# jackhwalters/DCS-Net

Measured on AMD Instinct MI355X. Metric: STFT frames/sec (train fwd+bwd+Adam), higher is better.
Workload: dtype f32

## Files before the change

dcs-net_amd/csrc/attention.hip:

```cpp
#include "conv_common.h"
#include "cbn_geom.h"

namespace {

constexpr int kThreads = 256;
#ifndef DCS_ATT_APP_IT
#define DCS_ATT_APP_IT 2
#endif
#ifndef DCS_ATT_GRID_CAP
#define DCS_ATT_GRID_CAP 8192
#endif
constexpr int kMaxChunks = DCS_ATT_MAX_CHUNKS;

inline bool att_geom(int C, int* G) { return att::geom(C, G); }
inline int ca_chunks(long HW, int G) { return att::ca_chunks(HW, G); }

__device__ __forceinline__ void ca_pool_kernel_body(const act_t* __restrict__ x, double* __restrict__ part,
                                                            long HW, int C, int G, int bx, int by, int gx) {
    __shared__ double red[kThreads * 4];
    const int t = threadIdx.x, g = t % G, r0 = t / G, rpi = kThreads / G;
    const int b = by;
    const ActIn4<act_t> x4 = act_in4(x) + (long)b * HW * G;
    float s0 = 0.f, s1 = 0.f, s2 = 0.f, s3 = 0.f;
    for (long r = (long)bx * rpi + r0; r < HW; r += (long)gx * rpi) {
// ... 75 lines not shown
    const int t = threadIdx.x, g = t % G, r0 = t / G, rpi = kThreads / G;
    const int b = by;
    const ActIn4<act_t> x4 = act_in4(x) + (long)b * HW * G;
    float4 a = make_float4(1.f, 0.f, 1.f, 0.f);
    if (ca) a = reinterpret_cast<const float4*>(ca)[(long)b * G + g];
    const float invC = 1.f / (float)C;
    const long iters = (HW + (long)gx * rpi - 1) / ((long)gx * rpi);
    for (long k = 0; k < iters; ++k) {
        const long r = (k * gx + bx) * rpi + r0;
        const bool ok = r < HW;
        float4 v = make_float4(0.f, 0.f, 0.f, 0.f);
        if (ok) v = x4[r * G + g];
        const float z0r = a.x * v.x - a.y * v.y, z0i = a.x * v.y + a.y * v.x;
        const float z1r = a.z * v.z - a.w * v.w, z1i = a.z * v.w + a.w * v.z;
        const float sr = group_sum(z0r + z1r, G), si = group_sum(z0i + z1i, G);
        const float mr = group_max(fmaxf(z0r, z1r), G), mi = group_max(fmaxf(z0i, z1i), G);
        if (ok && g == 0) pooled[(long)b * HW + r] = make_float4(sr * invC, si * invC, mr, mi);
    }
}

template <bool DROP>
__device__ __forceinline__ void attention_apply_kernel_body(const act_t* __restrict__ x,
                                                                    const float* __restrict__ ca,
                                                                    const float2* __restrict__ sa, act_t* __restrict__ y,
                                                                    long HW, int C, int G, float drop_p, uint64_t seed, const uint64_t* __restrict__ seed_dev, int bx, int by, int gx) {
    if (seed_dev) seed += seed_dev[0];
    const int t = threadIdx.x, g = t % G, r0 = t / G, rpi = kThreads / G;
    const int b = by;
    const long base = (long)b * HW * G;
    const ActIn4<act_t> x4 = act_in4(x) + base;
    const ActOut4<act_t> y4 = act_out4(y) + base;
    float4 a = make_float4(1.f, 0.f, 1.f, 0.f);
    if (ca) a = reinterpret_cast<const float4*>(ca)[(long)b * G + g];
    const float inv_keep = DROP ? 1.f / (1.f - drop_p) : 1.f;
    for (long r = (long)bx * rpi + r0; r < HW; r += (long)gx * rpi) {
        const float4 v = x4[r * G + g];
        float2 s = make_float2(1.f, 0.f);
        if (sa) s = sa[(long)b * HW + r];
        const float z0r = fmaf(a.x, v.x, -(a.y * v.y)), z0i = fmaf(a.x, v.y, a.y * v.x);
        const float z1r = fmaf(a.z, v.z, -(a.w * v.w)), z1i = fmaf(a.z, v.w, a.w * v.z);
        float4 o;
        o.x = fmaf(s.x, z0r, -(s.y * z0i)); o.y = fmaf(s.x, z0i, s.y * z0r);
        o.z = fmaf(s.x, z1r, -(s.y * z1i)); o.w = fmaf(s.x, z1i, s.y * z1r);
        if (DROP) {
            const uint64_t e = (uint64_t)(base + r * G + g) * 4;
            o.x *= dcs_keep_scale(seed, e, drop_p, inv_keep);
            o.y *= dcs_keep_scale(seed, e + 1, drop_p, inv_keep);
            o.z *= dcs_keep_scale(seed, e + 2, drop_p, inv_keep);
            o.w *= dcs_keep_scale(seed, e + 3, drop_p, inv_keep);
        }
        y4[r * G + g] = o;
    }
}

constexpr int kMaxBatch = 8;
template <class P> struct Tbl { P p[kMaxBatch]; int x0[kMaxBatch + 1]; };
template <class P> __device__ __forceinline__ int tbl_find(const Tbl<P>& t, int bx) {
    int z = 0;
#pragma unroll
    for (int k = 1; k < kMaxBatch; ++k) z += bx >= t.x0[k] ? 1 : 0;
    return z;
}

struct CaPoolP { const act_t* x; double* part; long HW; int C, G, nx; };
struct CaFcP { const double* part; int nchunks; const float2* w1; const float2* w2; float2* ca; float2* pooled; float2* hidden;
               long HW; int C, Ch; };
struct SpPoolP { const act_t* x; const float* ca; float4* pooled; long HW; int C, G, nx; };
struct ApplyP { const act_t* x; const float* ca; const float2* sa; act_t* y; long HW; int C, G, nx; };

__global__ __launch_bounds__(kThreads) void ca_pool_kernel(CaPoolP p) {
    ca_pool_kernel_body(p.x, p.part, p.HW, p.C, p.G, blockIdx.x, blockIdx.y, gridDim.x);
}
__global__ __launch_bounds__(kThreads) void ca_pool_multi_kernel(Tbl<CaPoolP> t) {
    const int z = tbl_find(t, blockIdx.x);
    const CaPoolP& p = t.p[z];
    ca_pool_kernel_body(p.x, p.part, p.HW, p.C, p.G, blockIdx.x - t.x0[z], blockIdx.y, p.nx);
}
__global__ __launch_bounds__(kThreads) void ca_fc_kernel(CaFcP p) {
    ca_fc_kernel_body(p.part, p.nchunks, p.w1, p.w2, p.ca, p.pooled, p.hidden, p.HW, p.C, p.Ch, blockIdx.x, 0, 0);
}
__global__ __launch_bounds__(kThreads) void ca_fc_multi_kernel(Tbl<CaFcP> t) {
    const CaFcP& p = t.p[blockIdx.z];
    ca_fc_kernel_body(p.part, p.nchunks, p.w1, p.w2, p.ca, p.pooled, p.hidden, p.HW, p.C, p.Ch, blockIdx.x, 0, 0);
}
__global__ __launch_bounds__(kThreads) void spatial_pool_kernel(SpPoolP p) {
    spatial_pool_kernel_body(p.x, p.ca, p.pooled, p.HW, p.C, p.G, blockIdx.x, blockIdx.y, gridDim.x);
}
__global__ __launch_bounds__(kThreads) void spatial_pool_multi_kernel(Tbl<SpPoolP> t) {
    const int z = tbl_find(t, blockIdx.x);
    const SpPoolP& p = t.p[z];
    spatial_pool_kernel_body(p.x, p.ca, p.pooled, p.HW, p.C, p.G, blockIdx.x - t.x0[z], blockIdx.y, p.nx);
}
template <bool DROP>
__global__ __launch_bounds__(kThreads) void attention_apply_kernel(ApplyP p, float drop_p, uint64_t seed, const uint64_t* seed_dev) {
    attention_apply_kernel_body<DROP>(p.x, p.ca, p.sa, p.y, p.HW, p.C, p.G, drop_p, seed, seed_dev, blockIdx.x, blockIdx.y, gridDim.x);
}
__global__ __launch_bounds__(kThreads) void attention_apply_multi_kernel(Tbl<ApplyP> t) {
    const int z = tbl_find(t, blockIdx.x);
    const ApplyP& p = t.p[z];
    attention_apply_kernel_body<false>(p.x, p.ca, p.sa, p.y, p.HW, p.C, p.G, 0.f, 0, nullptr, blockIdx.x - t.x0[z], blockIdx.y, p.nx);
}

#ifndef DCS_ACT_BF16
__global__ __launch_bounds__(kThreads) void dropout_kernel(const float* __restrict__ x, float* __restrict__ y, long n,
                                                            float drop_p, uint64_t seed, const uint64_t* __restrict__ seed_dev) {
    if (seed_dev) seed += seed_dev[0];
    const float inv_keep = 1.f / (1.f - drop_p);
    for (long i = (long)blockIdx.x * kThreads + threadIdx.x; i < n; i += (long)gridDim.x * kThreads)
        y[i] = x[i] * (drop_p > 0.f ? dcs_keep_scale(seed, (uint64_t)i, drop_p, inv_keep) : 1.f);
}
#endif

inline int stream_grid(long HW, int G, int B) {
    const int rpi = kThreads / G;
    long it = (HW + rpi - 1) / rpi;
    long nb = it <= DCS_ATT_SMALL_IT ? (it + DCS_ATT_APP_IT - 1) / DCS_ATT_APP_IT : (it + 3) / 4;
    long cap = (it <= DCS_ATT_SMALL_IT ? DCS_ATT_GRID_CAP : 2048) / (B > 0 ? B : 1);
    if (cap < 1) cap = 1;
    return (int)(nb < 1 ? 1 : (nb > cap ? cap : nb));
}

}

#ifndef DCS_ACT_BF16
extern "C" long dcs_ca_workspace_bytes(int B, long HW, int C) {
    int G;
    if (B <= 0 || HW <= 0 || !att_geom(C, &G)) return -1;
    return (long)B * ca_chunks(HW, G) * C * 2 * (long)sizeof(double);
}
#endif

extern "C" int DCS_SYM(dcs_channel_attention_fwd)(const act_t* x, const float* w1, const float* w2, float* ca_out,
                                         float* pooled_out, float* hidden_out, void* workspace, long workspace_bytes,
                                         int B, long HW, int C, int Ch, dcs_stream_t stream) {
    int G;
    if (!x || !w1 || !w2 || !ca_out || !pooled_out || !hidden_out || !workspace) return DCS_ERR_BADARG;
    if (B <= 0 || B > 65535 || HW <= 0 || !att_geom(C, &G) || Ch <= 0 || Ch > 64) return DCS_ERR_BADARG;
    const int nch = ca_chunks(HW, G);
    if (workspace_bytes < (long)B * nch * C * 2 * (long)sizeof(double)) return DCS_ERR_WORKSPACE;
    hipStream_t s = dcs_stream(stream);
    const CaPoolP pp{x, (double*)workspace, HW, C, G, nch};
    DCS_LAUNCH(ca_pool_kernel, dim3(nch, B), dim3(kThreads), 0, s, pp);
    DCS_CHECK_LAUNCH();
    const CaFcP fp{(const double*)workspace, nch, (const float2*)w1, (const float2*)w2, (float2*)ca_out, (float2*)pooled_out,
                   (float2*)hidden_out, HW, C, Ch};
    DCS_LAUNCH(ca_fc_kernel, dim3(B), dim3(kThreads), 0, s, fp);
    DCS_CHECK_LAUNCH();
    return DCS_OK;
}

#ifndef DCS_ACT_BF16
extern "C" int dcs_ca_pool_chunks(long HW, int C) {
    int G;
    if (HW <= 0 || !att_geom(C, &G)) return -1;
    return ca_chunks(HW, G);
}

extern "C" int dcs_channel_attention_fc_fwd(const void* part, const float* w1, const float* w2, float* ca_out,
                                            float* pooled_out, float* hidden_out, int B, long HW, int C, int Ch,
                                            dcs_stream_t stream) {
    int G;
    if (!part || !w1 || !w2 || !ca_out || !pooled_out || !hidden_out) return DCS_ERR_BADARG;
    if (B <= 0 || B > 65535 || HW <= 0 || !att_geom(C, &G) || Ch <= 0 || Ch > 64) return DCS_ERR_BADARG;
    const CaFcP fp{(const double*)part, ca_chunks(HW, G), (const float2*)w1, (const float2*)w2, (float2*)ca_out,
                   (float2*)pooled_out, (float2*)hidden_out, HW, C, Ch};
    DCS_LAUNCH(ca_fc_kernel, dim3(B), dim3(kThreads), 0, dcs_stream(stream), fp);
    DCS_CHECK_LAUNCH();
    return DCS_OK;
}
#endif

extern "C" int DCS_SYM(dcs_spatial_pool_fwd)(const act_t* x, const float* ca, float* pooled, int B, long HW, int C,
                                    dcs_stream_t stream) {
    int G;
    if (!x || !pooled || B <= 0 || B > 65535 || HW <= 0 || !att_geom(C, &G)) return DCS_ERR_BADARG;
    const int nx = stream_grid(HW, G, B);
    const SpPoolP sp{x, ca, (float4*)pooled, HW, C, G, nx};
    DCS_LAUNCH(spatial_pool_kernel, dim3(nx, B), dim3(kThreads), 0, dcs_stream(stream), sp);
    DCS_CHECK_LAUNCH();
    return DCS_OK;
}

extern "C" int DCS_SYM(dcs_attention_apply_fwd)(const act_t* x, const float* ca, const float* sa, act_t* y, int B, long HW,
                                       int C, float drop_p, unsigned long long seed, const unsigned long long* seed_dev, dcs_stream_t stream) {
    int G;
    if (!x || !y || B <= 0 || B > 65535 || HW <= 0 || !att_geom(C, &G)) return DCS_ERR_BADARG;
    if (!(drop_p >= 0.f && drop_p < 1.f)) return DCS_ERR_BADARG;
    const int nx = stream_grid(HW, G, B);
    dim3 grid(nx, B);
    const ApplyP ap{x, ca, (const float2*)sa, y, HW, C, G, nx};
    if (drop_p > 0.f)
        DCS_LAUNCH(attention_apply_kernel<true>, grid, dim3(kThreads), 0, dcs_stream(stream), ap, drop_p,
                           (uint64_t)seed, (const uint64_t*)seed_dev);
    else
        DCS_LAUNCH(attention_apply_kernel<false>, grid, dim3(kThreads), 0, dcs_stream(stream), ap, drop_p,
                           (uint64_t)seed, (const uint64_t*)seed_dev);
    DCS_CHECK_LAUNCH();
    return DCS_OK;
}

static long fwd_batched_workspace_bytes(int n, const dcs_attention_item* items, int B) {
    if (n < 1 || n > kMaxBatch || !items || B <= 0) return -1;
    long total = 0;
    for (int i = 0; i < n; ++i) {
        int G;
        if (!att_geom(items[i].C, &G)) return -1;
        const long b = (long)B * ca_chunks((long)items[i].H * items[i].W, G) * items[i].C * 2 * (long)sizeof(double);
        total += (b + 255) / 256 * 256;
    }
    return total;
}

#ifndef DCS_ACT_BF16
extern "C" long dcs_attention_fwd_batched_workspace_bytes(int n, const dcs_attention_item* items, int B) {
    return fwd_batched_workspace_bytes(n, items, B);
}
#endif

extern "C" int DCS_SYM(dcs_attention_fwd_batched)(int n, const dcs_attention_item* items, void* workspace, long workspace_bytes, int B,
                                         dcs_stream_t stream) {
    if (n < 1 || n > kMaxBatch || !items || !workspace || B <= 0 || B > 65535) return DCS_ERR_BADARG;
    if (workspace_bytes < fwd_batched_workspace_bytes(n, items, B)) return DCS_ERR_WORKSPACE;
    Tbl<CaPoolP> tp; Tbl<CaFcP> tf; Tbl<SpPoolP> ts; Tbl<ApplyP> ta;
    conv::Args ca_[kMaxBatch];
    int nx_pool = 1, nx_stream = 1;
    char* ws = (char*)workspace;
    for (int i = 0; i < n; ++i) {
        const dcs_attention_item& it = items[i];
        int G;
        if (!it.x || !it.w1 || !it.w2 || !it.wsa || !it.sa_bias || !it.ca || !it.pooled || !it.hidden || !it.sp || !it.sa ||
            !it.y || it.H <= 0 || it.W <= 0 || it.Ch <= 0 || it.Ch > 64 || !att_geom(it.C, &G))
            return DCS_ERR_BADARG;
        const long HW = (long)it.H * it.W;
        const int nch = ca_chunks(HW, G), nxs = stream_grid(HW, G, B);
        tp.p[i] = CaPoolP{(const act_t*)it.x, (double*)ws, HW, it.C, G, nch};
        tf.p[i] = CaFcP{(const double*)ws, nch, (const float2*)it.w1, (const float2*)it.w2, (float2*)it.ca, (float2*)it.pooled,
                        (float2*)it.hidden, HW, it.C, it.Ch};
        ts.p[i] = SpPoolP{(const act_t*)it.x, it.ca, (float4*)it.sp, HW, it.C, G, nxs};
        ta.p[i] = ApplyP{(const act_t*)it.x, it.ca, (const float2*)it.sa, (act_t*)it.y, HW, it.C, G, nxs};
        ws += ((long)B * nch * it.C * 2 * (long)sizeof(double) + 255) / 256 * 256;
        nx_pool = nch > nx_pool ? nch : nx_pool;
        nx_stream = nxs > nx_stream ? nxs : nx_stream;
        conv::Args& a = ca_[i];
        a = conv::Args{};
        a.x1 = (const act2_t*)it.sp;     a.x2 = nullptr; a.wp = (const float2*)it.wsa; a.bias = (const float2*)it.sa_bias;
        a.y = (act2_t*)it.sa;
        a.B = B; a.Hin = it.H; a.Win = it.W; a.C1 = 2; a.C2 = 0; a.up_f = 1; a.up_t = 1; a.zero_ins = 0; a.Cout = 1;
        a.kh = 7; a.kw = 7; a.sf = 1; a.st = 1; a.pad_f = 3; a.pad_t = 3; a.act = DCS_ACT_SIGMOID;
        a.Hv = it.H; a.Wv = it.W; a.Hout = it.H; a.Wout = it.W;
    }
    hipStream_t s = dcs_stream(stream);
    {
        int ap = 0, as_ = 0;
        for (int k = 0; k <= kMaxBatch; ++k) {
            tp.x0[k] = k < n ? ap : 0x7fffffff; ts.x0[k] = ta.x0[k] = k < n ? as_ : 0x7fffffff;
            if (k < n) { ap += tp.p[k].nx; as_ += ts.p[k].nx; }
        }
        tp.x0[n] = ap; ts.x0[n] = ta.x0[n] = as_;
        nx_pool = ap; nx_stream = as_;
    }
    DCS_LAUNCH(ca_pool_multi_kernel, dim3(nx_pool, B, 1), dim3(kThreads), 0, s, tp);
    DCS_CHECK_LAUNCH();
    DCS_LAUNCH(ca_fc_multi_kernel, dim3(B, 1, n), dim3(kThreads), 0, s, tf);
    DCS_CHECK_LAUNCH();
    DCS_LAUNCH(spatial_pool_multi_kernel, dim3(nx_stream, B, 1), dim3(kThreads), 0, s, ts);
    DCS_CHECK_LAUNCH();
    const int rc = dcs_conv_direct_multi(ca_, n, s);
    if (rc != DCS_OK) return rc;
    DCS_LAUNCH(attention_apply_multi_kernel, dim3(nx_stream, B, 1), dim3(kThreads), 0, s, ta);
    DCS_CHECK_LAUNCH();
    return DCS_OK;
}

#ifndef DCS_ACT_BF16
extern "C" int dcs_dropout_fwd(const float* x, float* y, long n, float drop_p, unsigned long long seed,
                               const unsigned long long* seed_dev, dcs_stream_t stream) {
    if (!x || !y || n <= 0 || !(drop_p >= 0.f && drop_p < 1.f)) return DCS_ERR_BADARG;
    long nb = (n + kThreads * 4 - 1) / (kThreads * 4);
    const int grid = (int)(nb < 1 ? 1 : (nb > 2048 ? 2048 : nb));
    DCS_LAUNCH(dropout_kernel, dim3(grid), dim3(kThreads), 0, dcs_stream(stream), x, y, n, drop_p,
                       (uint64_t)seed, (const uint64_t*)seed_dev);
    DCS_CHECK_LAUNCH();
    return DCS_OK;
}
#endif
```

dcs-net_amd/csrc/cbn.hip:

```cpp
#include "dcs_common.h"
#include "cbn_geom.h"

namespace {

constexpr int kThreads = 256;
constexpr int kMaxBlocks = 512;

struct CbnGeom {
    int vec_per_row;
    int rows_per_iter;
    int nblocks;
};

inline bool cbn_geom(long P, int C, CbnGeom* g) {
    if (P <= 0 || C <= 0) return false;
    if (C == 1) {
        long nvec = P / 2;
        long it = (nvec + kThreads - 1) / kThreads;
        long nb = (it + DCS_CBN_RED_IT - 1) / DCS_CBN_RED_IT;
        g->vec_per_row = 0;
        g->rows_per_iter = 0;
        g->nblocks = (int)(nb < 1 ? 1 : (nb > kMaxBlocks ? kMaxBlocks : nb));
        return true;
    }
// ... 149 lines not shown
    const float Rrr = (Cii + s) * ist, Rii = (Crr + s) * ist, Rri = -Cri * ist;
    const float W0 = w_[0], W1 = w_[1], W2 = w_[2], b0 = b_[0], b1 = b_[1];
    const float a0 = W0 * Rrr + W2 * Rri, a1 = W0 * Rri + W2 * Rii;
    const float a2 = W2 * Rrr + W1 * Rri, a3 = W2 * Rri + W1 * Rii;
    float* st = stats_out + 8 * c;
    st[0] = mr; st[1] = mi; st[2] = Rrr; st[3] = Rii; st[4] = Rri; st[5] = Crr; st[6] = Cii; st[7] = Cri;
    float* co = coef_out + 6 * c;
    co[0] = a0; co[1] = a1; co[2] = a2; co[3] = a3;
    co[4] = b0 - a0 * mr - a1 * mi;
    co[5] = b1 - a2 * mr - a3 * mi;
}

#ifndef DCS_ACT_BF16
__global__ void rbn_finalize_kernel(const float* __restrict__ x, const double* __restrict__ part, int nblocks,
                                    const float* __restrict__ weight, const float* __restrict__ bias,
                                    float* __restrict__ running_mean, float* __restrict__ running_var,
                                    float* __restrict__ stats_out, float* __restrict__ coef_out, long P, int C, int merge,
                                    float eps, float momentum, int use_batch_stats) {
    const int c = blockIdx.x, lane = threadIdx.x;
    float mr, mi, vr, vi;
    if (use_batch_stats) {
        double S[5] = {0, 0, 0, 0, 0};
        for (int b0 = lane; b0 < nblocks; b0 += 64 * 8) {
            double v[8][5];
#pragma unroll
            for (int k = 0; k < 8; ++k) {
                const int b = b0 + 64 * k < nblocks ? b0 + 64 * k : nblocks - 1;
#pragma unroll
                for (int i = 0; i < 5; ++i) v[k][i] = part[((long)b * C + c) * 5 + i];
            }
#pragma unroll
            for (int k = 0; k < 8; ++k)
#pragma unroll
                for (int i = 0; i < 5; ++i) S[i] += b0 + 64 * k < nblocks ? v[k][i] : 0.0;
        }
#pragma unroll
        for (int i = 0; i < 5; ++i) S[i] = dcs_wave_sum_d(S[i]);
        if (lane != 0) return;
        const double n = (double)P;
        const double kr = (double)x[2 * c], ki = (double)x[2 * c + 1];
        double m_r = kr + S[0] / n, m_i = ki + S[1] / n;
        double v_r = S[2] / n - (S[0] / n) * (S[0] / n), v_i = S[3] / n - (S[1] / n) * (S[1] / n);
        double cnt = n;
        if (merge) {
            const double m = 0.5 * (m_r + m_i);
            const double v = 0.5 * (v_r + (m_r - m) * (m_r - m) + v_i + (m_i - m) * (m_i - m));
            m_r = m_i = m; v_r = v_i = v; cnt = 2 * n;
        }
        mr = (float)m_r; mi = (float)m_i; vr = (float)v_r; vi = (float)v_i;
        if (momentum >= 0.f && running_mean != nullptr) {
            const float f = momentum, unb = cnt > 1 ? (float)(cnt / (cnt - 1.0)) : 1.f;
            if (merge) {
                running_mean[0] = f * mr + (1.f - f) * running_mean[0];
                running_var[0] = f * vr * unb + (1.f - f) * running_var[0];
            } else {
                running_mean[2 * c] = f * mr + (1.f - f) * running_mean[2 * c];
                running_mean[2 * c + 1] = f * mi + (1.f - f) * running_mean[2 * c + 1];
                running_var[2 * c] = f * vr * unb + (1.f - f) * running_var[2 * c];
                running_var[2 * c + 1] = f * vi * unb + (1.f - f) * running_var[2 * c + 1];
            }
        }
    } else {
        if (lane != 0) return;
        mr = running_mean[merge ? 0 : 2 * c]; mi = running_mean[merge ? 0 : 2 * c + 1];
        vr = running_var[merge ? 0 : 2 * c]; vi = running_var[merge ? 0 : 2 * c + 1];
    }
    const float isr = 1.0f / sqrtf(vr + eps), isi = 1.0f / sqrtf(vi + eps);
    float w0 = 1.f, w1 = 1.f, b0 = 0.f, b1 = 0.f;
    if (weight != nullptr) {
        w0 = weight[merge ? 0 : 2 * c]; w1 = weight[merge ? 0 : 2 * c + 1];
        b0 = bias[merge ? 0 : 2 * c]; b1 = bias[merge ? 0 : 2 * c + 1];
    }
    const float a0 = w0 * isr, a3 = w1 * isi;
    float* st = stats_out + 8 * c;
    st[0] = mr; st[1] = mi; st[2] = isr; st[3] = isi; st[4] = 0.f; st[5] = vr + eps; st[6] = vi + eps; st[7] = 0.f;
    float* co = coef_out + 6 * c;
    co[0] = a0; co[1] = 0.f; co[2] = 0.f; co[3] = a3;
    co[4] = b0 - a0 * mr;
    co[5] = b1 - a3 * mi;
}

#endif

template <int ACT>
__device__ __forceinline__ float act_fn(float v) {
    if (ACT == DCS_ACT_RELU) return v > 0.f ? v : 0.f;
    if (ACT == DCS_ACT_LRELU) return v > 0.f ? v : 0.01f * v;
    return v;
}

template <int ACT, bool DROP>
__global__ __launch_bounds__(kThreads) void cbn_apply_kernel(const act_t* __restrict__ x, act_t* __restrict__ y,
                                                              const float* __restrict__ coef, long P, int C, int G,
                                                              int rows_per_iter, float drop_p, uint64_t seed, const uint64_t* __restrict__ seed_dev) {
    if (seed_dev) seed += seed_dev[0];
    const float inv_keep = DROP ? 1.f / (1.f - drop_p) : 1.f;
    const int t = threadIdx.x;
    const ActIn4<act_t> x4 = act_in4(x);
    const ActOut4<act_t> y4 = act_out4(y);
    if (C == 1) {
        const float a0 = coef[0], a1 = coef[1], a2 = coef[2], a3 = coef[3], c0 = coef[4], c1 = coef[5];
        const long nvec = P / 2;
        for (long i = (long)blockIdx.x * kThreads + t; i < nvec; i += (long)gridDim.x * kThreads) {
            float4 v = x4[i], o;
            o.x = act_fn<ACT>(fmaf(a0, v.x, fmaf(a1, v.y, c0)));
            o.y = act_fn<ACT>(fmaf(a2, v.x, fmaf(a3, v.y, c1)));
            o.z = act_fn<ACT>(fmaf(a0, v.z, fmaf(a1, v.w, c0)));
            o.w = act_fn<ACT>(fmaf(a2, v.z, fmaf(a3, v.w, c1)));
            if (DROP) {
                const uint64_t e = (uint64_t)i * 4;
                o.x *= dcs_keep_scale(seed, e, drop_p, inv_keep);
                o.y *= dcs_keep_scale(seed, e + 1, drop_p, inv_keep);
                o.z *= dcs_keep_scale(seed, e + 2, drop_p, inv_keep);
                o.w *= dcs_keep_scale(seed, e + 3, drop_p, inv_keep);
            }
            y4[i] = o;
        }
        if ((P & 1) && blockIdx.x == 0 && t == 0) {
            const float xr = dcs_ld1(x + 2 * (P - 1)), xi = dcs_ld1(x + 2 * (P - 1) + 1);
            float yr = act_fn<ACT>(fmaf(a0, xr, fmaf(a1, xi, c0)));
            float yi = act_fn<ACT>(fmaf(a2, xr, fmaf(a3, xi, c1)));
            if (DROP) {
                yr *= dcs_keep_scale(seed, (uint64_t)2 * (P - 1), drop_p, inv_keep);
                yi *= dcs_keep_scale(seed, (uint64_t)2 * (P - 1) + 1, drop_p, inv_keep);
            }
            dcs_st1(y + 2 * (P - 1), yr);
            dcs_st1(y + 2 * (P - 1) + 1, yi);
        }
        return;
    }
    const int g = t % G, r0 = t / G;
    const float* ca = coef + 12 * g;
    const float a0 = ca[0], a1 = ca[1], a2 = ca[2], a3 = ca[3], c0 = ca[4], c1 = ca[5];
    const float e0 = ca[6], e1 = ca[7], e2 = ca[8], e3 = ca[9], f0 = ca[10], f1 = ca[11];
    for (long r = (long)blockIdx.x * rows_per_iter + r0; r < P; r += (long)gridDim.x * rows_per_iter) {
        float4 v = x4[r * G + g], o;
        o.x = act_fn<ACT>(fmaf(a0, v.x, fmaf(a1, v.y, c0)));
        o.y = act_fn<ACT>(fmaf(a2, v.x, fmaf(a3, v.y, c1)));
        o.z = act_fn<ACT>(fmaf(e0, v.z, fmaf(e1, v.w, f0)));
        o.w = act_fn<ACT>(fmaf(e2, v.z, fmaf(e3, v.w, f1)));
        if (DROP) {
            const uint64_t e = (uint64_t)(r * G + g) * 4;
            o.x *= dcs_keep_scale(seed, e, drop_p, inv_keep);
            o.y *= dcs_keep_scale(seed, e + 1, drop_p, inv_keep);
            o.z *= dcs_keep_scale(seed, e + 2, drop_p, inv_keep);
            o.w *= dcs_keep_scale(seed, e + 3, drop_p, inv_keep);
        }
        y4[r * G + g] = o;
    }
}

__device__ __forceinline__ float stored(float v) { return DCS_ACT_IS_BF16 ? dcs_bf16_to_f32(dcs_f32_to_bf16(v)) : v; }

template <int ACT>
__global__ __launch_bounds__(kThreads) void cbn_apply_pool_kernel(const act_t* __restrict__ x, act_t* __restrict__ y,
                                                                   const float* __restrict__ coef, double* __restrict__ part,
                                                                   long HW, int C, int G) {
    __shared__ double red[kThreads * 4];
    const int t = threadIdx.x, g = t % G, r0 = t / G, rpi = kThreads / G;
    const int b = blockIdx.y, bx = blockIdx.x, gx = gridDim.x;
    const ActIn4<act_t> x4 = act_in4(x) + (long)b * HW * G;
    const ActOut4<act_t> y4 = act_out4(y) + (long)b * HW * G;
    const float* ca = coef + 12 * g;
    const float a0 = ca[0], a1 = ca[1], a2 = ca[2], a3 = ca[3], c0 = ca[4], c1 = ca[5];
    const float e0 = ca[6], e1 = ca[7], e2 = ca[8], e3 = ca[9], f0 = ca[10], f1 = ca[11];
    float s0 = 0.f, s1 = 0.f, s2 = 0.f, s3 = 0.f;
    for (long r = (long)bx * rpi + r0; r < HW; r += (long)gx * rpi) {
        const float4 v = x4[r * G + g];
        float4 o;
        o.x = act_fn<ACT>(fmaf(a0, v.x, fmaf(a1, v.y, c0)));
        o.y = act_fn<ACT>(fmaf(a2, v.x, fmaf(a3, v.y, c1)));
        o.z = act_fn<ACT>(fmaf(e0, v.z, fmaf(e1, v.w, f0)));
        o.w = act_fn<ACT>(fmaf(e2, v.z, fmaf(e3, v.w, f1)));
        y4[r * G + g] = o;
        s0 += stored(o.x); s1 += stored(o.y); s2 += stored(o.z); s3 += stored(o.w);
    }
    red[t * 4 + 0] = s0; red[t * 4 + 1] = s1; red[t * 4 + 2] = s2; red[t * 4 + 3] = s3;
    __syncthreads();
    for (int o = t; o < G * 4; o += kThreads) {
        const int gg = o / 4, i = o % 4;
        double a = 0;
        for (int r = 0; r < rpi; ++r) a += red[(r * G + gg) * 4 + i];
        part[(((long)b * gx + bx) * C + 2 * gg) * 2 + i] = a;
    }
}

}

#ifndef DCS_ACT_BF16
extern "C" long dcs_cbn_workspace_bytes(long P, int C) {
    CbnGeom g;
    if (!cbn_geom(P, C, &g)) return -1;
    return (long)g.nblocks * C * 5 * (long)sizeof(double);
}
#endif

static int cbn_fwd_impl(const act_t* x, act_t* y, const float* weight, const float* bias, float* running_mean,
                        float* running_covar, float* stats_out, float* coef_out, void* workspace,
                        long workspace_bytes, long P, int C, float eps, float momentum, int use_batch_stats,
                        int act, float drop_p, unsigned long long seed, const unsigned long long* seed_dev, dcs_stream_t stream,
                        const float* slab_part, int slab_rows, int slab_stride, const float* slab_pivot) {
    CbnGeom g;
    if (!x || !y || !stats_out || !coef_out || !cbn_geom(P, C, &g)) return DCS_ERR_BADARG;
    if ((weight == nullptr) != (bias == nullptr)) return DCS_ERR_BADARG;
    if (use_batch_stats < 0 || use_batch_stats > 3) return DCS_ERR_BADARG;
    if (use_batch_stats == 3 && (!slab_part || !slab_pivot || slab_rows < 1 || slab_stride < slab_rows)) return DCS_ERR_BADARG;
    if (use_batch_stats == 0 && (!running_mean || !running_covar)) return DCS_ERR_BADARG;
    if (act != DCS_ACT_NONE && act != DCS_ACT_RELU && act != DCS_ACT_LRELU) return DCS_ERR_BADARG;
    if (!(drop_p >= 0.f && drop_p < 1.f)) return DCS_ERR_BADARG;
    hipStream_t s = dcs_stream(stream);
    if (use_batch_stats == 1) {
        if (!workspace || workspace_bytes < (long)g.nblocks * C * 5 * (long)sizeof(double)) return DCS_ERR_WORKSPACE;
        DCS_LAUNCH(cbn_stats_kernel, dim3(g.nblocks), dim3(kThreads), 0, s, x, (double*)workspace, P, C,
                           g.vec_per_row, g.rows_per_iter);
        DCS_CHECK_LAUNCH();
    }
    if (use_batch_stats == 3) {
        DCS_LAUNCH((cbn_finalize_kernel<float, float>), dim3(C), dim3(256), 0, s, slab_pivot, slab_part, slab_rows, slab_stride, weight, bias,
                   running_mean, running_covar, stats_out, coef_out, P, C, eps, momentum, 1);
        DCS_CHECK_LAUNCH();
    } else if (use_batch_stats != 2) {
        DCS_LAUNCH((cbn_finalize_kernel<double, act_t>), dim3(C), dim3(256), 0, s, x, (const double*)workspace,
                           g.nblocks, 0, weight, bias, running_mean, running_covar, stats_out, coef_out, P, C, eps, momentum,
                           use_batch_stats);
        DCS_CHECK_LAUNCH();
    }
    long iters = (C == 1) ? (P / 2 + kThreads - 1) / kThreads : (P + g.rows_per_iter - 1) / g.rows_per_iter;
    long nb = (iters + DCS_CBN_APP_IT - 1) / DCS_CBN_APP_IT;
    int grid = (int)(nb < 1 ? 1 : (nb > 2048 ? 2048 : nb));
#define DCS_CBN_APPLY(A, D)                                                                                   \
    DCS_LAUNCH((cbn_apply_kernel<A, D>), dim3(grid), dim3(kThreads), 0, s, x, y, coef_out, P, C,         \
                       g.vec_per_row, g.rows_per_iter, drop_p, (uint64_t)seed, (const uint64_t*)seed_dev)
    const bool drop = drop_p > 0.f;
    if (act == DCS_ACT_RELU) { if (drop) DCS_CBN_APPLY(DCS_ACT_RELU, true); else DCS_CBN_APPLY(DCS_ACT_RELU, false); }
    else if (act == DCS_ACT_LRELU) { if (drop) DCS_CBN_APPLY(DCS_ACT_LRELU, true); else DCS_CBN_APPLY(DCS_ACT_LRELU, false); }
    else { if (drop) DCS_CBN_APPLY(DCS_ACT_NONE, true); else DCS_CBN_APPLY(DCS_ACT_NONE, false); }
#undef DCS_CBN_APPLY
    DCS_CHECK_LAUNCH();
    return DCS_OK;
}

extern "C" int DCS_SYM(dcs_cbn_fwd)(const act_t* x, act_t* y, const float* weight, const float* bias, float* running_mean,
                           float* running_covar, float* stats_out, float* coef_out, void* workspace,
                           long workspace_bytes, long P, int C, float eps, float momentum, int use_batch_stats,
                           int act, float drop_p, unsigned long long seed, const unsigned long long* seed_dev, dcs_stream_t stream) {
    if (use_batch_stats == 3) return DCS_ERR_BADARG;
    return cbn_fwd_impl(x, y, weight, bias, running_mean, running_covar, stats_out, coef_out, workspace, workspace_bytes, P, C,
                        eps, momentum, use_batch_stats, act, drop_p, seed, seed_dev, stream, nullptr, 0, 0, nullptr);
}

extern "C" int DCS_SYM(dcs_cbn_fwd_slabs)(const act_t* x, act_t* y, const float* weight, const float* bias, float* running_mean,
                                 float* running_covar, float* stats_out, float* coef_out, const float* part, int rows,
                                 int stride, const float* pivot, long P, int C, float eps, float momentum, int act, float drop_p,
                                 unsigned long long seed, const unsigned long long* seed_dev, dcs_stream_t stream) {
    return cbn_fwd_impl(x, y, weight, bias, running_mean, running_covar, stats_out, coef_out, nullptr, 0, P, C, eps, momentum,
                        3, act, drop_p, seed, seed_dev, stream, part, rows, stride, pivot);
}

extern "C" int DCS_SYM(dcs_cbn_fwd_slabs_pool)(const act_t* x, act_t* y, const float* weight, const float* bias,
                                               float* running_mean, float* running_covar, float* stats_out, float* coef_out,
                                               const float* part, int rows, int stride, const float* pivot, void* pool_part,
                                               long pool_bytes, int B, long HW, int C, float eps, float momentum, int act,
                                               dcs_stream_t stream) {
    int G;
    if (!x || !y || !stats_out || !coef_out || !part || !pivot || !pool_part || B <= 0 || B > 65535 || HW <= 0 ||
        !att::geom(C, &G) || rows < 1 || stride < rows)
        return DCS_ERR_BADARG;
    if ((weight == nullptr) != (bias == nullptr)) return DCS_ERR_BADARG;
    if (act != DCS_ACT_NONE && act != DCS_ACT_RELU && act != DCS_ACT_LRELU) return DCS_ERR_BADARG;
    const int nch = att::ca_chunks(HW, G);
    if (pool_bytes < (long)B * nch * C * 2 * (long)sizeof(double)) return DCS_ERR_WORKSPACE;
    hipStream_t s = dcs_stream(stream);
    const long P = (long)B * HW;
    DCS_LAUNCH((cbn_finalize_kernel<float, float>), dim3(C), dim3(256), 0, s, pivot, part, rows, stride, weight, bias,
               running_mean, running_covar, stats_out, coef_out, P, C, eps, momentum, 1);
    DCS_CHECK_LAUNCH();
#define DCS_CBN_AP(A) DCS_LAUNCH((cbn_apply_pool_kernel<A>), dim3(nch, B), dim3(kThreads), 0, s, x, y, (const float*)coef_out, \
                                 (double*)pool_part, HW, C, G)
    if (act == DCS_ACT_RELU) DCS_CBN_AP(DCS_ACT_RELU);
    else if (act == DCS_ACT_LRELU) DCS_CBN_AP(DCS_ACT_LRELU);
    else DCS_CBN_AP(DCS_ACT_NONE);
#undef DCS_CBN_AP
    DCS_CHECK_LAUNCH();
    return DCS_OK;
}

#ifndef DCS_ACT_BF16
extern "C" int dcs_rbn_fwd(const float* x, float* y, const float* weight, const float* bias, float* running_mean,
                           float* running_var, float* stats_out, float* coef_out, void* workspace, long workspace_bytes,
                           long P, int Cr, float eps, float momentum, int use_batch_stats, int act, dcs_stream_t stream) {
    const int merge = Cr == 1;
    if (!x || !y || !stats_out || !coef_out || Cr < 1 || (!merge && (Cr & 1)) || (merge && (P & 1))) return DCS_ERR_BADARG;
    const int C = merge ? 1 : Cr / 2;
    const long Pc = merge ? P / 2 : P;
    CbnGeom g;
    if (!cbn_geom(Pc, C, &g)) return DCS_ERR_BADARG;
    if ((weight == nullptr) != (bias == nullptr) || use_batch_stats < 0 || use_batch_stats > 1) return DCS_ERR_BADARG;
    if (use_batch_stats == 0 && (!running_mean || !running_var)) return DCS_ERR_BADARG;
    if (act != DCS_ACT_NONE && act != DCS_ACT_RELU && act != DCS_ACT_LRELU) return DCS_ERR_BADARG;
    hipStream_t s = dcs_stream(stream);
    if (use_batch_stats) {
        if (!workspace || workspace_bytes < (long)g.nblocks * C * 5 * (long)sizeof(double)) return DCS_ERR_WORKSPACE;
        DCS_LAUNCH(cbn_stats_kernel, dim3(g.nblocks), dim3(kThreads), 0, s, x, (double*)workspace, Pc, C, g.vec_per_row,
                   g.rows_per_iter);
        DCS_CHECK_LAUNCH();
    }
    DCS_LAUNCH(rbn_finalize_kernel, dim3(C), dim3(64), 0, s, x, (const double*)workspace, g.nblocks, weight, bias,
               running_mean, running_var, stats_out, coef_out, Pc, C, merge, eps, momentum, use_batch_stats);
    DCS_CHECK_LAUNCH();
    long iters = (C == 1) ? (Pc / 2 + kThreads - 1) / kThreads : (Pc + g.rows_per_iter - 1) / g.rows_per_iter;
    long nb = (iters + DCS_CBN_APP_IT - 1) / DCS_CBN_APP_IT;
    const int grid = (int)(nb < 1 ? 1 : (nb > 2048 ? 2048 : nb));
#define DCS_RBN_APPLY(A)                                                                                        \
    DCS_LAUNCH((cbn_apply_kernel<A, false>), dim3(grid), dim3(kThreads), 0, s, x, y, coef_out, Pc, C, g.vec_per_row, \
               g.rows_per_iter, 0.f, (uint64_t)0, (const uint64_t*)nullptr)
    if (act == DCS_ACT_RELU) DCS_RBN_APPLY(DCS_ACT_RELU);
    else if (act == DCS_ACT_LRELU) DCS_RBN_APPLY(DCS_ACT_LRELU);
    else DCS_RBN_APPLY(DCS_ACT_NONE);
#undef DCS_RBN_APPLY
    DCS_CHECK_LAUNCH();
    return DCS_OK;
}
#endif
```

dcs-net_amd/csrc/cbn_geom.h:

```cpp
#pragma once
#ifndef DCS_CBN_RED_IT
#define DCS_CBN_RED_IT 8
#endif
#ifndef DCS_CBN_APP_IT
#define DCS_CBN_APP_IT 4
#endif

namespace cbn {

constexpr int kThreads = 256;
constexpr int kMaxBlocks = 512;

struct Geom {
    int vec_per_row;
    int rows_per_iter;
    int nblocks;
};

inline bool geom(long P, int C, Geom* g) {
    if (P <= 0 || C <= 0) return false;
    long it;
    if (C == 1) {
        g->vec_per_row = 0;
        g->rows_per_iter = 0;
        it = (P / 2 + kThreads - 1) / kThreads;
    } else {
        if (C & 1) return false;
        const int G = C / 2;
        if (G > kThreads || (kThreads % G) != 0) return false;
        g->vec_per_row = G;
        g->rows_per_iter = kThreads / G;
        it = (P + g->rows_per_iter - 1) / g->rows_per_iter;
    }
    const long nb = (it + DCS_CBN_RED_IT - 1) / DCS_CBN_RED_IT;
    g->nblocks = (int)(nb < 1 ? 1 : (nb > kMaxBlocks ? kMaxBlocks : nb));
    return true;
}

inline int stream_grid(long P, int C, const Geom& g) {
    const long iters = (C == 1) ? (P / 2 + kThreads - 1) / kThreads : (P + g.rows_per_iter - 1) / g.rows_per_iter;
    const long nb = (iters + DCS_CBN_APP_IT - 1) / DCS_CBN_APP_IT;
    return (int)(nb < 1 ? 1 : (nb > 2048 ? 2048 : nb));
}

}

#ifndef DCS_ATT_RED_IT
#define DCS_ATT_RED_IT 2
#endif
#ifndef DCS_ATT_SMALL_IT
#define DCS_ATT_SMALL_IT 256
#endif
#ifndef DCS_ATT_MAX_CHUNKS
#define DCS_ATT_MAX_CHUNKS 256
#endif
namespace att {
inline bool geom(int C, int* G) {
    if (C < 2 || (C & 1)) return false;
    const int g = C / 2;
    if (g > 64 || (g & (g - 1)) != 0) return false;
    *G = g;
    return true;
}
inline int ca_chunks(long HW, int G) {
    const int rows_per_iter = 256 / G;
    const long it = (HW + rows_per_iter - 1) / rows_per_iter;
    long nb = it <= DCS_ATT_SMALL_IT ? (it + DCS_ATT_RED_IT - 1) / DCS_ATT_RED_IT : (it + 7) / 8;
    if (it > DCS_ATT_SMALL_IT && nb > 64) nb = 64;
    return (int)(nb < 1 ? 1 : (nb > DCS_ATT_MAX_CHUNKS ? DCS_ATT_MAX_CHUNKS : nb));
}
}
```

dcs-net_amd/dcsnet/_lib.py:

```python
import ctypes
import os

_HERE = os.path.dirname(os.path.abspath(__file__))
LIB_PATH = os.environ.get('DCS_LIB_PATH') or os.path.join(os.path.dirname(_HERE), 'lib', 'libdcsnet_hip.so')

ACT_NONE, ACT_RELU, ACT_LRELU, ACT_SIGMOID = 0, 1, 2, 3

_P = ctypes.c_void_p
_I = ctypes.c_int
_L = ctypes.c_long
_F = ctypes.c_float
_U64 = ctypes.c_ulonglong



class AttentionItem(ctypes.Structure):
    _fields_ = [(n, _P) for n in ('x', 'w1', 'w2', 'wsa', 'sa_bias', 'ca', 'pooled', 'hidden', 'sp', 'sa', 'y', 'g_out',
                                  'wsa_bwd', 'g_pre', 'g_sp', 'g_x', 'g_fc0_r', 'g_fc0_i', 'g_fc2_r', 'g_fc2_i')] + \
               [(n, _I) for n in ('H', 'W', 'C', 'Ch')] + [('g_pooled', _P)]


SIGNATURES = {
    'dcs_abi_version': (_I, []),
    'dcs_error_string': (ctypes.c_char_p, [_I]),
    'dcs_pack_conv_weight': (_I, [_P, _P, _P, _P, _P, _P, _I, _I, _I, _I, _I, _I, _I, _P]),
    'dcs_cconv2d_fwd_workspace_bytes': (_L, [_I] * 14),
    'dcs_cconv2d_fwd': (_I, [_P, _P, _P, _P, _P, _P, _L] + [_I] * 15 + [_P]),
    'dcs_cconv2d_fwd_affine': (_I, [_P, _P, _P, _P, _P, _P, _P, _L] + [_I] * 15 + [_P]),
    'dcs_cconv2d_fwd_stats_rows': (_I, [_I] * 14),
    'dcs_cconv2d_fwd_stats': (_I, [_P] * 6 + [_I, _P, _P, _L] + [_I] * 14 + [_P]),
    'dcs_rconv2d_fwd_workspace_bytes': (_L, [_I] * 14),
    'dcs_rconv2d_fwd': (_I, [_P, _P, _P, _P, _P, _P, _L] + [_I] * 15 + [_P]),
    'dcs_rconv2d_bwd_data_workspace_bytes': (_L, [_I] * 11),
    'dcs_rconv2d_bwd_data': (_I, [_P, _P, _P, _P, _L] + [_I] * 11 + [_P]),
    'dcs_rbn_fwd': (_I, [_P] * 9 + [_L, _L, _I, _F, _F, _I, _I, _P]),
    'dcs_rbn_bwd': (_I, [_P] * 8 + [_L, _L, _I, _I, _I, _P]),
    'dcs_packed_weight_floats': (_L, [_I] * 6),
    'dcs_packed_weight_bwd_floats': (_L, [_I] * 10),
    'dcs_pack_conv_weight_bwd': (_I, [_P, _P] + [_I] * 10 + [_P]),
    'dcs_cconv2d_bwd_data_workspace_bytes': (_L, [_I] * 14),
    'dcs_cconv2d_bwd_data': (_I, [_P] * 5 + [_L] + [_I] * 14 + [_P]),
    'dcs_upsample_cat_bwd': (_I, [_P, _P, _P] + [_I] * 7 + [_P]),
    'dcs_cconv2d_bwd_weight_workspace_bytes': (_L, [_I] * 14),
    'dcs_cconv2d_bwd_weight': (_I, [_P] * 8 + [_L] + [_I] * 15 + [_P]),
    'dcs_cbn_workspace_bytes': (_L, [_L, _I]),
    'dcs_cbn_fwd': (_I, [_P] * 9 + [_L, _L, _I, _F, _F, _I, _I, _F, _U64, _P, _P]),
    'dcs_cbn_fwd_slabs': (_I, [_P] * 9 + [_I, _I, _P, _L, _I, _F, _F, _I, _F, _U64, _P, _P]),
    'dcs_ca_pool_chunks': (_I, [_L, _I]),
    'dcs_cbn_fwd_slabs_pool': (_I, [_P] * 9 + [_I, _I, _P, _P, _L, _I, _L, _I, _F, _F, _I, _P]),
    'dcs_channel_attention_fc_fwd': (_I, [_P] * 6 + [_I, _L, _I, _I, _P]),
    'dcs_cbn_bwd_workspace_bytes': (_L, [_L, _I]),
    'dcs_cbn_bwd': (_I, [_P] * 9 + [_L, _L, _I, _I, _I, _F, _U64, _P, _P]),
    'dcs_cbn_bwd_add': (_I, [_P] * 9 + [_L, _L, _I, _I, _I, _F, _U64, _P, _P, _F, _L, _P, _P]),
    'dcs_ca_workspace_bytes': (_L, [_I, _L, _I]),
    'dcs_channel_attention_fwd': (_I, [_P] * 7 + [_L, _I, _L, _I, _I, _P]),
    'dcs_spatial_pool_fwd': (_I, [_P, _P, _P, _I, _L, _I, _P]),
    'dcs_attention_apply_fwd': (_I, [_P, _P, _P, _P, _I, _L, _I, _F, _U64, _P, _P]),
    'dcs_rattention_workspace_bytes': (_L, [_I, _L, _I]),
    'dcs_rattention_fwd': (_I, [_P] * 8 + [_L] + [_I] * 6 + [_P]),
    'dcs_rattention_train_workspace_bytes': (_L, [_I, _L, _I, _I]),
    'dcs_rattention_pool_fwd': (_I, [_P] * 8 + [_L] + [_I] * 5 + [_P]),
    'dcs_rattention_apply_fwd': (_I, [_P] * 4 + [_I] * 4 + [_P]),
    'dcs_rattention_apply_bwd': (_I, [_P] * 8 + [_L] + [_I] * 4 + [_P]),
    'dcs_rattention_pool_bwd': (_I, [_P] * 11 + [_I] + [_P, _L] + [_I] * 5 + [_P]),
    'dcs_attention_bwd_sa': (_I, [_P] * 5 + [_I, _L, _I, _F, _U64, _P, _P]),
    'dcs_attention_bwd_workspace_bytes': (_L, [_I, _L, _I, _I]),
    'dcs_attention_bwd_x': (_I, [_P] * 16 + [_L, _I, _L, _I, _I, _F, _U64, _P, _P]),
    'dcs_attention_bwd_fc_weights': (_I, [_P, _L, _P, _P, _P, _P, _P, _P, _I, _L, _I, _I, _P]),
    'dcs_attention_fwd_batched_workspace_bytes': (_L, [_I, _P, _I]),
    'dcs_attention_fwd_batched': (_I, [_I, _P, _P, _L, _I, _P]),
    'dcs_attention_bwd_batched_workspace_bytes': (_L, [_I, _P, _I]),
    'dcs_attention_bwd_batched': (_I, [_I, _P, _P, _L, _I, _P]),
    'dcs_lstm_layer_fwd': (_I, [_P] * 6 + [_I, _I, _I, _I, _L, _L, _L, _P]),
    'dcs_lstm_layer_fwd_bias': (_I, [_P, _P, _P, _P, _P, _P, _P, _P, _I, _I, _I, _I, _L, _L, _L, _P]),
    'dcs_lstm_layer_bwd': (_I, [_P] * 6 + [_I] * 4 + [_P]),
    'dcs_dropout_fwd': (_I, [_P, _P, _L, _F, _U64, _P, _P]),
    'dcs_complex_act_fwd': (_I, [_P, _P, _L, _I, _P]),
    'dcs_complex_upsample_fwd': (_I, [_P, _P, _I, _I, _I, _I, _I, _I, _P]),
    'dcs_tapsum_fwd': (_I, [_P, _P, _P, _P] + [_I] * 10 + [_P]),
    'dcs_cconv_up2_single_fwd': (_I, [_P] * 6 + [_I] * 6 + [_P]),
    'dcs_cconv_up2_single_bwd_data': (_I, [_P] * 4 + [_I] * 6 + [_P]),
    'dcs_cconv_up2_single_bwd_weight_workspace_bytes': (_L, []),
    'dcs_cconv_up2_single_bwd_weight': (_I, [_P] * 7 + [_I, _P, _L] + [_I] * 5 + [_P]),
    'dcs_tapsum_bwd_workspace_bytes': (_L, []),
    'dcs_tapsum_bwd': (_I, [_P, _P, _P, _P, _P, _L] + [_I] * 10 + [_P]),
    'dcs_bound_crm_fwd': (_I, [_P, _P, _L, _F, _P]),
    'dcs_bound_mask_apply_fwd': (_I, [_P, _P, _P, _P, _P, _L, _F, _P]),
    'dcs_bound_mask_apply_bwd': (_I, [_P] * 6 + [_L, _F, _P]),
    'dcs_bound2_mask_apply_fwd': (_I, [_P] * 6 + [_L, _F, _F, _U64, _P, _P]),
    'dcs_bound2_mask_apply_bwd': (_I, [_P] * 7 + [_L, _F, _F, _U64, _P, _P]),
    'dcs_bound2_apply_polar_frames_fwd': (_I, [_P] * 4 + [_I] * 4 + [_F, _F, _U64, _P, _P]),
    'dcs_bound2_apply_polar_frames_bwd': (_I, [_P] * 5 + [_I] * 4 + [_F, _I, _F, _U64, _P, _P]),
    'dcs_complex_abs_f32': (_I, [_P, _P, _L, _P]),
    'dcs_rmask_apply_polar_frames_fwd': (_I, [_P] * 4 + [_I] * 4 + [_F, _I, _P]),
    'dcs_rmask_apply_polar_frames_bwd': (_I, [_P] * 5 + [_I] * 4 + [_F, _I, _I, _P]),
    'dcs_irfft512_frames': (_I, [_P, _P, _L, _P]),
    'dcs_rfft512_frames': (_I, [_P, _P, _L, _P]),
    'dcs_rfft512_ola_frames': (_I, [_P, _P, _P, _P, _I, _I, _I, _F, _P]),
    'dcs_irfft512_ola_frames': (_I, [_P, _P, _P, _P, _I, _I, _I, _F, _P]),
    'dcs_polar_frames_fwd': (_I, [_P, _P, _I, _I, _I, _I, _F, _P]),
    'dcs_polar_frames_bwd': (_I, [_P, _P, _P, _I, _I, _I, _I, _F, _I, _P]),
    'dcs_istft_envelope': (_I, [_P, _P, _I, _I, _I, _P]),
    'dcs_istft_ola_fwd': (_I, [_P, _P, _P, _P, _I, _I, _I, _I, _F, _P]),
    'dcs_istft_ola_bwd': (_I, [_P, _P, _P, _P, _I, _I, _I, _I, _F, _P]),
    'dcs_stft_frames_fwd': (_I, [_P, _P, _P, _P, _I, _I, _I, _I, _I, _P]),
    'dcs_stft_bins_fwd': (_I, [_P, _P, _I, _I, _I, _F, _P]),
    'dcs_sisnr_fwd': (_I, [_P, _P, _P, _P, _I, _I, _F, _P]),
    'dcs_sisnr_bwd': (_I, [_P, _P, _P, _P, _F, _P, _I, _I, _P]),
    'dcs_sisnr_losses_fwd': (_I, [_P, _P, _P, _I, _F, _P]),
    'dcs_lstm_whh_grad': (_I, [_P, _P, _P, _I, _I, _I, _P]),
    'dcs_atb_chunks': (_I, [_P, _P, _P, _L, _L, _L, _L, _I, _I, _I, _I, _I, _I, _I, _I, _P]),
    'dcs_chunk_sum_acc': (_I, [_P, _P, _L, _L, _I, _I, _I, _L, _P]),
    'dcs_atb_chunks_strided': (_I, [_P, _P, _P, _L, _L, _L, _L, _I, _I, _I, _I, _I, _I, _I, _I, _I, _P]),
    'dcs_gemm_f32': (_I, [_P, _P, _P] + [_I] * 8 + [_L, _L, _I, _L, _L, _L, _I, _I, _P]),
    'dcs_lstm_combine_fwd': (_I, [_P, _P, _L, _P]),
    'dcs_lstm_combine_bwd': (_I, [_P, _P, _L, _P]),
    'dcs_lstm_param_grads': (_I, [_P, _P, _P, _P, _P, _I, _I, _I, _P]),
    'dcs_lstm_param_grads_ih': (_I, [_P, _P, _P, _P, _P, _I, _I, _I, _P, _P, _I, _L, _I, _P]),
    'dcs_sisnr_losses_guard_fwd': (_I, [_P, _P, _P, _I, _F, _P, _P]),
    'dcs_sisnr_pair_bwd': (_I, [_P, _P, _P, _P, _P, _P, _F, _P, _I, _I, _P]),
    'dcs_crm_fwd': (_I, [_P, _P, _P, _L, _F, _P]),
    'dcs_adam_amsgrad_step': (_I, [_P] * 6 + [_F, _F, _L, _P, _F, _F, _F, _F, _I, _P, _P, _P]),
    'dcs_adam_amsgrad_step_sumsq': (_I, [_P] * 6 + [_I, _F, _F, _L, _P, _F, _F, _F, _F, _I, _P, _P, _P]),
    'dcs_swa_average_f32': (_I, [_P, _P, _L, _L, _P]),
    'dcs_grad_sumsq_parts': (_I, [_P, _L, _P, _I, _P, _P, _P, _P, _I, _P]),
    'dcs_step_guard': (_I, [_P, _P, _P]),
    'dcs_stream_hold': (_I, [_P, _I, _P]),
    'dcs_kernel_timer_begin': (_I, [_I]),
    'dcs_kernel_timer_end': (_I, []),
    'dcs_kernel_timer_read': (_I, [_I, _P]),
    'dcs_step_advance': (_I, [_P, _P, _P, _P]),
    'dcs_step_advance_counters': (_I, [_P, _P, _P, _P, _I, _P]),
    'dcs_pack_tap_rows': (_I, [_P, _P, _P, _P, _I, _I, _I, _I, _P]),
    'dcs_tap_rows_wgrad_scatter': (_I, [_P, _P, _P, _P, _I, _I, _I, _I, _P]),
    'dcs_set_conv_precision': (_I, [_I]),
    'dcs_get_conv_precision': (_I, []),
    'dcs_wgrad_defer_begin': (_I, []),
    'dcs_wgrad_defer_suspend': (_I, [_I]),
    'dcs_wgrad_defer_flush': (_I, [_P]),
    'dcs_pack_plan_begin': (_I, []),
    'dcs_pack_plan_end': (_I, [_P]),
    'dcs_pack_plan_jobs': (_I, [_P, _P, _P]),
    'dcs_pack_plan_run': (_I, [_P, _P]),
    'dcs_pack_plan_destroy': (_I, [_P]),
    'dcs_resample_poly_f32': (_I, [_P, _P, _I, _L, _P, _I, _I, _I, _P]),
    'dcs_stoi_workspace_bytes': (_L, [_I, _L]),
    'dcs_stoi_f32': (_I, [_P, _P, _I, _L, _P, _P, _P, _P, _P, _L, _P]),
    'dcs_resample_poly_ragged_f32': (_I, [_P, _P, _I, _L, _P, _P, _L, _P, _I, _I, _I, _P]),
    'dcs_stoi_ragged_workspace_bytes': (_L, [_I, _L]),
    'dcs_stoi_ragged_f32': (_I, [_P, _P, _P, _I, _L, _L, _P, _P, _P, _P, _P, _L, _P]),
    'dcs_sisnr_ragged_f32': (_I, [_P, _P, _P, _I, _L, _P, _P]),
    'dcs_resample_sinc_f32':(_I, [_P, _P, _P, _P, _I, _L, _P, _I, _I, _I, _P]),
    'dcs_audio_stft_batch_f32': (_I, [_P, _P, _P, _I, _P, _P, _I, _P, _I, _I, _I, _F, _P, _P, _P, _P]),
    'dcs_audio_stft_segments_f32': (_I, [_P, _P, _I, _P, _P, _I, _P, _I, _I, _I, _I, _F, _P, _P]),
    'dcs_segments_stitch_f32': (_I, [_P, _L, _P, _P, _I, _L, _I, _I, _I, _P, _P, _P]),
}

_lib = None


class DcsHipError(RuntimeError):
    pass


for _n in ('dcs_cconv2d_fwd', 'dcs_cconv2d_fwd_affine', 'dcs_cconv2d_fwd_stats', 'dcs_cconv2d_bwd_data', 'dcs_cconv2d_bwd_weight',
           'dcs_cconv_up2_single_fwd', 'dcs_cconv_up2_single_bwd_data', 'dcs_cconv_up2_single_bwd_weight', 'dcs_tapsum_bwd', 'dcs_cbn_fwd', 'dcs_cbn_fwd_slabs', 'dcs_cbn_fwd_slabs_pool', 'dcs_cbn_bwd', 'dcs_cbn_bwd_add',
           'dcs_channel_attention_fwd', 'dcs_spatial_pool_fwd', 'dcs_attention_apply_fwd', 'dcs_attention_fwd_batched',
           'dcs_attention_bwd_sa', 'dcs_attention_bwd_x', 'dcs_attention_bwd_batched'):
    SIGNATURES[_n + '_h'] = SIGNATURES[_n]


def load():
    global _lib
    if _lib is not None:
        return _lib
    import torch
    if not os.path.exists(LIB_PATH):
        raise DcsHipError(f'{LIB_PATH} not found: build it with `python dcs-net_amd/build.py` '
                          '(there is no CPU or eager fallback)')
    lib = ctypes.CDLL(LIB_PATH)
    for name, (res, args) in SIGNATURES.items():
        try:
            fn = getattr(lib, name)
        except AttributeError as e:
            raise DcsHipError(f'{LIB_PATH} does not export {name}; rebuild it') from e
        fn.restype = res
        fn.argtypes = args
    _lib = lib
    return lib


def check(code, what):
    if code != 0:
        msg = load().dcs_error_string(code).decode()
        raise DcsHipError(f'{what}: {msg} (code {code})')


def ptr(t):
    return None if t is None else t.data_ptr()


def cur_stream():
    import torch
    return torch.cuda.current_stream().cuda_stream
```

dcs-net_amd/dcsnet/functional.py:

```python
import os
import weakref

import torch

from . import _derived
from . import ops
from .ops import ACT_NONE, ACT_RELU, ACT_LRELU, ACT_SIGMOID, to_nhwc, from_nhwc
from ._lib import DcsHipError

_PACKED = _derived.Derived(capacity=512)


def bump_param_generation():
    _derived.bump_generation()
    ops.pack_plan_invalidate()


def note_state_update():
    _derived.bump_generation()


state_generation = _derived.generation


# ... 19 lines not shown
            if e is not None and e[0][0]() is w_r and e[0][1]() is w_i and e[2] == (
                    w_r._version, w_i._version, None if b_r is None else b_r._version,
                    None if b_i is None else b_i._version):
                return e[1]

    def make():
        d = lambda t: None if t is None else t.detach()
        wr, wi = d(w_r), d(w_i)
        if wr.dim() == 2:
            wr, wi = wr.view(*wr.shape, 1, 1), wi.view(*wi.shape, 1, 1)
        if tap_rows:
            packed = ops.pack_tap_rows(wr, wi, int(tap_rows))
        else:
            packed = ops.pack_conv_weight(wr, wi, d(b_r), d(b_i), transposed, tuple(up))
        if plan is not None and plan.recording:
            wref = lambda t: None if t is None else weakref.ref(t)
            plan.fwd[pkey] = [(wref(w_r), wref(w_i), wref(b_r), wref(b_i)), packed, None]
        return packed
    return _PACKED.get(w_r, (bool(transposed), tuple(up), int(tap_rows)), (w_r, w_i, b_r, b_i), make, ops.conv_precision())


ATTENTION_BATCH_MAX = ops.ATTENTION_BATCH_MAX

FLUSH_AT_NEXT_FORK = False
WGRAD_SIDE = None
sink_hits = 0


def _sink(p):
    if p is None or not p.requires_grad:
        return None
    s = getattr(p, '_dcs_grad_sink', None)
    if s is None or p.grad is None or p.grad.data_ptr() != s.data_ptr():
        return None
    global sink_hits
    sink_hits += 1
    return s


DEFER_FC = os.environ.get('DCS_DEFER_FC', '1') != '0'
PENDING_SIDE = []


def _run_pending_side():
    while PENDING_SIDE:
        job = PENDING_SIDE.pop(0)
        ops.attention_bwd_fc_weights(job)
        if ops.WGRAD_DEFER is not None:
            ops.WGRAD_DEFER.append(job)


class _CConv2dFn(torch.autograd.Function):

    @staticmethod
    def forward(ctx, x1, x2, w_r, w_i, b_r, b_i, transposed, ksize, stride, pad, up, act, holder=None):
        wp, bias = packed_weight(w_r, w_i, b_r, b_i, transposed, up)
        if holder is not None:
            y, holder['stat'] = ops.cconv2d_stats(x1, x2, wp, bias, ksize, stride, pad, up)
        else:
            y = ops.cconv2d(x1, x2, wp, bias, ksize, stride, pad, up, act)
        ctx.geom = (transposed, tuple(ksize), tuple(stride), tuple(pad), tuple(up), act, tuple(w_r.shape),
                    b_r is not None)
        ctx.sinks = (_sink(w_r), _sink(w_i), _sink(b_r), _sink(b_i))
        ctx.save_for_backward(x1, x2, wp, y if act == ACT_SIGMOID else None)
        return y

    @staticmethod
    def backward(ctx, gy):
        x1, x2, wp, y = ctx.saved_tensors
        transposed, ksize, stride, pad, up, act, w_shape, has_bias = ctx.geom
        gy = gy.contiguous()
        if act == ACT_SIGMOID:
            gy = gy * y * (1.0 - y)
        elif act != ACT_NONE:
            raise DcsHipError('cconv2d backward: only ACT_NONE / ACT_SIGMOID epilogues are differentiable here')
        gx1 = gx2 = gw_r = gw_i = gb_r = gb_i = None
        need = ctx.needs_input_grad
        want_w = need[2] or need[3] or need[4] or need[5]
        side = None
        if (want_w and WGRAD_SIDE is not None and ops.WGRAD_DEFER is not None and gy.is_cuda and
                ctx.sinks[0] is not None and ctx.sinks[1] is not None and (not has_bias or (ctx.sinks[2] is not None and ctx.sinks[3] is not None))):
            side = WGRAD_SIDE
            side.wait_stream(torch.cuda.current_stream())
        if need[0] or need[1]:
            C1 = x1.shape[3]
            Cin = C1 + (x2.shape[3] if x2 is not None else 0)
            gx1, gx2 = ops.cconv2d_bwd_data(gy, ops.pack_conv_weight_bwd(wp, ksize, stride, pad, up),
                                            (x1.shape[1], x1.shape[2], Cin), ksize, stride, pad, up, C1)
        if want_w:
            if side is not None:
                with torch.cuda.stream(side):
                    _run_pending_side()
                    g = ops.cconv2d_bwd_weight(x1, x2, gy, w_shape, has_bias, ksize, stride, pad, up, transposed, ctx.sinks,
                                               immediate=True)
                    global FLUSH_AT_NEXT_FORK
                    if FLUSH_AT_NEXT_FORK:
                        FLUSH_AT_NEXT_FORK = False
                        ops.wgrad_defer_flush(partial=True)
            else:
                g = ops.cconv2d_bwd_weight(x1, x2, gy, w_shape, has_bias, ksize, stride, pad, up, transposed, ctx.sinks)
            gw_r, gw_i, gb_r, gb_i = (None if sk is not None else t for t, sk in zip(g, ctx.sinks))
        return gx1, gx2, gw_r, gw_i, gb_r, gb_i, None, None, None, None, None, None, None


def cconv2d(x1, x2, w_r, w_i, b_r, b_i, transposed, ksize, stride, pad, up=(1, 1), act=ACT_NONE):
    return _CConv2dFn.apply(x1, x2, w_r, w_i, b_r, b_i, transposed, tuple(ksize), tuple(stride), tuple(pad),
                            tuple(up), act)


def cconv2d_with_stats(x1, x2, w_r, w_i, b_r, b_i, transposed, ksize, stride, pad, up=(1, 1)):
    holder = {}
    y = _CConv2dFn.apply(x1, x2, w_r, w_i, b_r, b_i, transposed, tuple(ksize), tuple(stride), tuple(pad), tuple(up),
                         ACT_NONE, holder)
    return y, holder.get('stat')


def cconv2d_cbn_eval(x1, x2, w_r, w_i, b_r, b_i, transposed, ksize, stride, pad, up, coef, act):
    wp, bias = packed_weight(w_r, w_i, b_r, b_i, transposed, tuple(up))
    return ops.cconv2d(x1, x2, wp, bias, tuple(ksize), tuple(stride), tuple(pad), tuple(up), act, coef=coef)


class _CbnFn(torch.autograd.Function):

    @staticmethod
    def forward(ctx, x, weight, bias, running_mean, running_covar, eps, momentum, use_batch_stats, act, drop_p, seed, stat=None):
        y, stats, coef = ops.cbn(x, weight, bias, running_mean, running_covar, eps, momentum, use_batch_stats,
                                 act, drop_p, seed, stat=stat)
        ctx.cfg = (bool(use_batch_stats), act, float(drop_p), int(seed), weight is not None)
        ctx.sinks = (_sink(weight), _sink(bias))
        ctx.save_for_backward(x, weight, stats, coef)
        return y

    @staticmethod
    def backward(ctx, g_out):
        x, weight, stats, coef = ctx.saved_tensors
        use_batch, act, drop_p, seed, affine = ctx.cfg
        g_x, g_w, g_b = ops.cbn_bwd(x, g_out.contiguous(), weight, stats, coef, use_batch, act, drop_p, seed, affine,
                                    ctx.sinks, need_gx=ctx.needs_input_grad[0])
        g_w = None if ctx.sinks[0] is not None else g_w
        g_b = None if ctx.sinks[1] is not None else g_b
        return g_x, g_w, g_b, None, None, None, None, None, None, None, None, None


def cbn(x, weight, bias, running_mean, running_covar, eps, momentum, use_batch_stats, act=ACT_NONE,
        drop_p=0.0, seed=0, stat=None):
    return _CbnFn.apply(x, weight, bias, running_mean, running_covar, eps, momentum, use_batch_stats, act,
                        drop_p, seed, stat)


class _CbnTwoFn(torch.autograd.Function):

    @staticmethod
    def forward(ctx, x, weight, bias, running_mean, running_covar, eps, momentum, use_batch_stats, act, drop_p, seed, stat=None):
        y, stats, coef = ops.cbn(x, weight, bias, running_mean, running_covar, eps, momentum, use_batch_stats,
                                 act, drop_p, seed, stat=stat)
        ctx.cfg = (bool(use_batch_stats), act, float(drop_p), int(seed), weight is not None)
        ctx.sinks = (_sink(weight), _sink(bias))
        ctx.save_for_backward(x, weight, stats, coef)
        ctx.set_materialize_grads(False)
        y2 = torch.empty(0, dtype=y.dtype, device=y.device).set_(y.untyped_storage(), y.storage_offset(), y.shape, y.stride())
        return y, y2

    @staticmethod
    def backward(ctx, g_a, g_b):
        x, weight, stats, coef = ctx.saved_tensors
        use_batch, act, drop_p, seed, affine = ctx.cfg
        if g_a is None and g_b is None:
            return (None,) * 12
        if g_a is None:
            g_a, g_b = g_b, None
        g_add = None
        for g_ in (g_a, g_b):
            if g_ is not None and _POOL_ADD:
                hit = _POOL_ADD.pop(g_.data_ptr(), None)
                if hit is not None:
                    if g_add is not None:
                        raise DcsHipError('cbn_two backward: two split pool terms for one stage output')
                    g_add = hit
        g_x, g_w, g_b_ = ops.cbn_bwd(x, g_a.contiguous(), weight, stats, coef, use_batch, act, drop_p, seed, affine,
                                     ctx.sinks, g_add=g_add, g_out2=None if g_b is None else g_b.contiguous())
        g_w = None if ctx.sinks[0] is not None else g_w
        g_b_ = None if ctx.sinks[1] is not None else g_b_
        return g_x, g_w, g_b_, None, None, None, None, None, None, None, None, None


def cbn_two(x, weight, bias, running_mean, running_covar, eps, momentum, use_batch_stats, act=ACT_NONE,
            drop_p=0.0, seed=0, stat=None):
    y, y2 = _CbnTwoFn.apply(x, weight, bias, running_mean, running_covar, eps, momentum, use_batch_stats, act,
                            drop_p, seed, stat)
    y2._dcs_adds_pool_term = True
    return y, y2


def channel_attention(x, fc0_r, fc0_i, fc2_r, fc2_i):
    w1, _ = packed_weight(fc0_r, fc0_i, None, None, False)
    w2, _ = packed_weight(fc2_r, fc2_i, None, None, False)
    ca, _, _ = ops.channel_attention(x, w1, w2)
    return ca


def spatial_attention(x, ca, conv_r, conv_i, ksize):
    pooled = ops.spatial_pool(x, ca)
    wp, bias = packed_weight(conv_r, conv_i, None, None, False)
    k = (ksize, ksize)
    return ops.cconv2d(pooled, None, wp, bias, k, (1, 1), (ksize // 2, ksize // 2), (1, 1), ACT_SIGMOID)


def attention_apply(x, ca, sa, drop_p=0.0, seed=0):
    return ops.attention_apply(x, ca, sa, drop_p, seed)


class _AttentionFn(torch.autograd.Function):

    @staticmethod
    def forward(ctx, x, fc0_r, fc0_i, fc2_r, fc2_i, c1_r, c1_i, ksize, drop_p, seed):
        w1, _ = packed_weight(fc0_r, fc0_i, None, None, False)
        w2, _ = packed_weight(fc2_r, fc2_i, None, None, False)
        wsa, zero_bias = packed_weight(c1_r, c1_i, None, None, False)
        ca, pooled, hidden = ops.channel_attention(x, w1, w2)
        sp = ops.spatial_pool(x, ca)
        sa = ops.cconv2d(sp, None, wsa, zero_bias, (ksize, ksize), (1, 1), (ksize // 2, ksize // 2), (1, 1),
                         ACT_SIGMOID)
        out = ops.attention_apply(x, ca, sa, drop_p, seed)
        ctx.cfg = (ksize, float(drop_p), int(seed))
        ctx.sinks = tuple(_sink(t) for t in (fc0_r, fc0_i, fc2_r, fc2_i, c1_r, c1_i))
        ctx.save_for_backward(x, ca, sa, sp, pooled, hidden, w1, w2, wsa)
        return out

    @staticmethod
    def backward(ctx, g_out):
        x, ca, sa, sp, pooled, hidden, w1, w2, wsa = ctx.saved_tensors
        ksize, drop_p, seed = ctx.cfg
        g = ops.attention_bwd(x, g_out.contiguous(), ca, sa, sp, pooled, hidden, w1, w2, wsa, ksize, drop_p, seed,
                              ctx.sinks)
        gw = tuple(None if sk is not None else t for t, sk in zip(g[1:], ctx.sinks))
        return (g[0], *gw, None, None, None)


def attention_block(x, fc0_r, fc0_i, fc2_r, fc2_i, c1_r, c1_i, ksize, drop_p=0.0, seed=0):
    return _AttentionFn.apply(x, fc0_r, fc0_i, fc2_r, fc2_i, c1_r, c1_i, ksize, drop_p, seed)


class _CbnAttentionFn(torch.autograd.Function):

    @staticmethod
    def forward(ctx, x, weight, bias, running_mean, running_covar, eps, momentum, use_batch_stats, act,
                fc0_r, fc0_i, fc2_r, fc2_i, c1_r, c1_i, ksize, drop_p, seed, stat=None):
        w1, _ = packed_weight(fc0_r, fc0_i, None, None, False)
        w2, _ = packed_weight(fc2_r, fc2_i, None, None, False)
        wsa, zero_bias = packed_weight(c1_r, c1_i, None, None, False)
        if stat is not None and use_batch_stats and weight is not None and ops.FUSE_APPLY_POOL:
            a, stats, coef, ca, pooled, hidden = ops.cbn_channel_attention(x, weight, bias, running_mean, running_covar, eps,
                                                                           momentum, act, stat, w1, w2)
        else:
            a, stats, coef = ops.cbn(x, weight, bias, running_mean, running_covar, eps, momentum, use_batch_stats, act, 0.0, 0,
                                     stat=stat)
            ca, pooled, hidden = ops.channel_attention(a, w1, w2)
        sp = ops.spatial_pool(a, ca)
        sa = ops.cconv2d(sp, None, wsa, zero_bias, (ksize, ksize), (1, 1), (ksize // 2, ksize // 2), (1, 1), ACT_SIGMOID)
        out = ops.attention_apply(a, ca, sa, drop_p, seed)
        ctx.cfg = (bool(use_batch_stats), act, weight is not None, ksize, float(drop_p), int(seed))
        ctx.sinks = tuple(_sink(t) for t in (weight, bias, fc0_r, fc0_i, fc2_r, fc2_i, c1_r, c1_i))
        ctx.save_for_backward(x, weight, stats, coef, a, ca, sa, sp, pooled, hidden, w1, w2, wsa)
        return out

    @staticmethod
    def backward(ctx, g_out):
        x, weight, stats, coef, a, ca, sa, sp, pooled, hidden, w1, w2, wsa = ctx.saved_tensors
        use_batch, act, affine, ksize, drop_p, seed = ctx.cfg
        sk = ctx.sinks
        defer = DEFER_FC and WGRAD_SIDE is not None and ops.WGRAD_DEFER is not None and all(s_ is not None for s_ in sk[2:6])
        g = ops.attention_bwd(a, g_out.contiguous(), ca, sa, sp, pooled, hidden, w1, w2, wsa, ksize, drop_p, seed, sk[2:],
                              split_pool=True, defer_fc=defer)
        if defer:
            PENDING_SIDE.append(g[8])
        g_x, g_w, g_b = ops.cbn_bwd(x, g[0], weight, stats, coef, use_batch, act, 0.0, 0, affine, sk[:2], g_add=g[7])
        full = (g_w, g_b, *g[1:7])
        gp = tuple(None if s_ is not None else t for t, s_ in zip(full, sk))
        return (g_x, gp[0], gp[1], None, None, None, None, None, None, *gp[2:], None, None, None, None)


def cbn_attention(x, weight, bias, running_mean, running_covar, eps, momentum, use_batch_stats, act,
                  fc0_r, fc0_i, fc2_r, fc2_i, c1_r, c1_i, ksize, drop_p=0.0, seed=0, stat=None):
    return _CbnAttentionFn.apply(x, weight, bias, running_mean, running_covar, eps, momentum, use_batch_stats, act,
                                 fc0_r, fc0_i, fc2_r, fc2_i, c1_r, c1_i, ksize, drop_p, seed, stat)


class _AttentionBlocksFn(torch.autograd.Function):

    @staticmethod
    def forward(ctx, n, ksize, split, *args):
        xs, params = args[:n], [args[n + 6 * i:n + 6 * i + 6] for i in range(n)]
        ctx.split = tuple(split)
        w1s, w2s, wsas, biases = [], [], [], []
        for fc0_r, fc0_i, fc2_r, fc2_i, c1_r, c1_i in params:
            w1s.append(packed_weight(fc0_r, fc0_i, None, None, False)[0])
            w2s.append(packed_weight(fc2_r, fc2_i, None, None, False)[0])
            wsa, zero_bias = packed_weight(c1_r, c1_i, None, None, False)
            wsas.append(wsa)
            biases.append(zero_bias)
        outs = ops.attention_blocks_fwd(xs, w1s, w2s, wsas, biases)
        ctx.n, ctx.ksize = n, ksize
        ctx.sinks = [tuple(_sink(t) for t in pr) for pr in params]
        ctx.shapes = [(tuple(pr[0].shape), tuple(pr[2].shape)) for pr in params]
        saved = []
        for x, o, w1, w2, wsa in zip(xs, outs, w1s, w2s, wsas):
            saved += [x, o['ca'], o['sa'], o['sp'], o['pooled'], o['hidden'], w1, w2, wsa]
        ctx.save_for_backward(*saved)
        return tuple(o['y'] for o in outs)

    @staticmethod
    def backward(ctx, *g_outs):
        n, ksize = ctx.n, ctx.ksize
        t = ctx.saved_tensors
        k, pad = (ksize, ksize), (ksize // 2, ksize // 2)
        saved, gs, wbs, fcs, sps = [], [], [], [], []
        for i in range(n):
            x, ca, sa, sp, pooled, hidden, w1, w2, wsa = t[9 * i:9 * i + 9]
            saved.append(dict(x=x, ca=ca, sa=sa, pooled=pooled, hidden=hidden, w1=w1, w2=w2))
            sps.append(sp)
            g = g_outs[i]
            gs.append(torch.zeros_like(x) if g is None else g.contiguous())
            wbs.append(ops.pack_conv_weight_bwd(wsa, k, (1, 1), pad))
            sk, (s0, s2) = ctx.sinks[i], ctx.shapes[i]
            new = lambda shape: torch.empty(shape, dtype=torch.float32, device=x.device)
            fcs.append(tuple(sk[j] if sk[j] is not None else new(s0 if j < 2 else s2) for j in range(4)))
        split = tuple(sp_ and ctx.needs_input_grad[3 + i] for i, sp_ in enumerate(ctx.split))
        res = ops.attention_blocks_bwd(saved, gs, wbs, fcs, split)
        if any(split):
            _POOL_ADD.clear()
            for (g_x, _, g_pooled), sp_ in zip(res, split):
                if sp_:
                    _POOL_ADD[g_x.data_ptr()] = g_pooled
            torch.autograd.Variable._execution_engine.queue_callback(_pool_add_consumed)
        grads_x, grads_p = [], []
        for i in range(n):
            g_x, g_pre, _ = res[i]
            sk = ctx.sinks[i]
            g_c1r, g_c1i, _, _ = ops.cconv2d_bwd_weight(sps[i], None, g_pre, (1, 2, ksize, ksize), False, k, (1, 1), pad,
                                                        outs=(sk[4], sk[5], None, None))
            full = (*fcs[i], g_c1r, g_c1i)
            grads_x.append(g_x)
            grads_p += [None if s_ is not None else g_ for g_, s_ in zip(full, sk)]
        global FLUSH_AT_NEXT_FORK
        if WGRAD_SIDE is not None and ops.WGRAD_DEFER is not None:
            ops.WGRAD_DEFER.append((sps, [r[1] for r in res]))
            FLUSH_AT_NEXT_FORK = True
        return (None, None, None, *grads_x, *grads_p)


SPLIT_SKIP_POOL = os.environ.get('DCS_SPLIT_SKIP_POOL', '1') != '0'
_POOL_ADD = {}


def _pool_add_consumed():
    if _POOL_ADD:
        _POOL_ADD.clear()
        raise DcsHipError('attention_blocks backward: a split average-pool term was not consumed by a cbn_two backward')


def attention_blocks(xs, params, ksize):
    flat = [p for pr in params for p in pr]
    split = tuple(bool(SPLIT_SKIP_POOL and getattr(x, '_dcs_adds_pool_term', False) and torch.is_grad_enabled() and x.requires_grad)
                  for x in xs)
    return _AttentionBlocksFn.apply(len(xs), ksize, split, *xs, *flat)



def _as_real(z):
    if z.dtype != torch.complex64:
        raise DcsHipError(f'expected complex64, got {z.dtype}')
    return torch.view_as_real(z.contiguous() if not _dense(z) else z)


def _dense(z):
    return z.is_contiguous() or (z.dim() == 4 and z.is_contiguous(memory_format=torch.channels_last))


def _elementwise(z, act):
    if z.dim() == 4 and z.is_contiguous(memory_format=torch.channels_last) and not z.is_contiguous():
        x = to_nhwc(z)
        return from_nhwc(ops.complex_act(x, act))
    x = torch.view_as_real(z.contiguous())
    return torch.view_as_complex(ops.complex_act(x, act))


def complex_relu(z):
    return _elementwise(z, ACT_RELU)


def complex_lrelu(z):
    return _elementwise(z, ACT_LRELU)


def complex_sigmoid(z):
    return _elementwise(z, ACT_SIGMOID)


def complex_upsample(z, scale_factor):
    sf = (scale_factor, scale_factor) if isinstance(scale_factor, (int, float)) else tuple(scale_factor)
    up = (int(sf[0]), int(sf[1]))
    if up != tuple(sf) or min(up) < 1:
        raise DcsHipError(f'complex_upsample: integer scale factors only, got {scale_factor}')
    return from_nhwc(ops.complex_upsample(to_nhwc(z), up))


def complex_linear(z, w_r, w_i, b_r, b_i):
    in_f = z.shape[-1]
    lead = z.shape[:-1]
    x = torch.view_as_real(z.reshape(-1, in_f).contiguous())
    N = x.shape[0]
    W = 16 if N % 16 == 0 else 1
    x = x.view(1, N // W, W, in_f, 2)
    y = cconv2d(x, None, w_r, w_i, b_r, b_i, False, (1, 1), (1, 1), (0, 0))
    return torch.view_as_complex(y.view(N, -1, 2)).view(*lead, -1)


class _LstmRecFn(torch.autograd.Function):

    @staticmethod
    def forward(ctx, gx, w_hh):
        n_sets, seqs, S, _, G4 = gx.shape
        need = gx.requires_grad or w_hh.requires_grad
        out, gates, c = ops.lstm_layer(gx, w_hh, n_sets, seqs, S, (seqs * S * 2 * G4, S * 2 * G4, 2 * G4), need)
        ctx.dims = (n_sets, seqs, S)
        if need:
            ctx.save_for_backward(out, gates, c, w_hh)
        return out

    @staticmethod
    def backward(ctx, g_out):
        out, gates, c, w_hh = ctx.saved_tensors
        n_sets, seqs, S = ctx.dims
        H = w_hh.shape[-1]
        g_pre = ops.lstm_layer_bwd(g_out.contiguous(), gates, c, w_hh, n_sets, seqs, S)
        g_pre5 = g_pre.view(n_sets, seqs, S, 2, 4 * H)
        g_whh = None
        if ctx.needs_input_grad[1]:
            o = out.view(n_sets, seqs, S, 2, H)
            h_prev = torch.zeros_like(o)
            h_prev[:, :, 1:, 0] = o[:, :, :-1, 0]
            h_prev[:, :, :-1, 1] = o[:, :, 1:, 1]
            g_whh = torch.einsum('sntdj,sntdk->sdjk', g_pre5, h_prev)
        return g_pre5, g_whh


def _project(inp, w_ih, shared, per_set=False, train=True):
    G8, K = w_ih.shape[1], w_ih.shape[2]
    M = inp.shape[-2]
    if not (ops.gemm_ok(M, G8, K, 2, train) and inp.is_contiguous() and w_ih.is_contiguous()):
        if shared and not per_set:
            return torch.mm(inp, w_ih.reshape(2 * G8, -1).t())
        return torch.matmul(inp, w_ih.transpose(1, 2))
    if shared and not per_set:
        gx = torch.empty((M, 2 * G8), dtype=torch.float32, device=inp.device)
        return ops.gemm_f32(inp, w_ih, gx, M, 2 * G8, K, K, K, 2 * G8, True)
    gx = torch.empty((2, M, G8), dtype=torch.float32, device=inp.device)
    return ops.gemm_f32(inp, w_ih, gx, M, G8, K, K, K, G8, True, nbatch=2, a_batch=0 if shared else M * K, b_batch=G8 * K,
                        c_batch=M * G8)


def _project_bwd(g_gx, w_ih, shared):
    G8, K = w_ih.shape[1], w_ih.shape[2]
    M = g_gx.shape[1]
    if not (ops.gemm_ok(M, K, G8, 2, True) and g_gx.is_contiguous() and w_ih.is_contiguous()):
        if shared:
            g_inp = torch.mm(g_gx[0], w_ih[0])
            return g_inp.addmm_(g_gx[1], w_ih[1])
        return torch.bmm(g_gx, w_ih)
    if shared:
        g_inp = torch.empty((M, K), dtype=torch.float32, device=g_gx.device)
        return ops.gemm_f32(g_gx, w_ih, g_inp, M, K, G8, G8, K, K, False, nseg=2, a_seg=M * G8, b_seg=G8 * K)
    g_inp = torch.empty((2, M, K), dtype=torch.float32, device=g_gx.device)
    return ops.gemm_f32(g_gx, w_ih, g_inp, M, K, G8, G8, K, K, False, nbatch=2, a_batch=M * G8, b_batch=G8 * K, c_batch=M * K)


class _ProjectFn(torch.autograd.Function):

    @staticmethod
    def forward(ctx, inp, w_ih):
        ctx.save_for_backward(inp, w_ih)
        return _project(inp, w_ih, shared=inp.dim() == 2, per_set=True)

    @staticmethod
    def backward(ctx, g):
        inp, w_ih = ctx.saved_tensors
        g = g.contiguous()
        g_inp = _project_bwd(g, w_ih, shared=inp.dim() == 2) if ctx.needs_input_grad[0] else None
        g_w = torch.matmul(g.transpose(1, 2), inp) if ctx.needs_input_grad[1] else None
        return g_inp, g_w


class _LstmLayerFn(torch.autograd.Function):

    @staticmethod
    def forward(ctx, inp, anchor, st, B2, S):
        w_ih, w_hh = st['weight_ih'][0], st['weight_hh'][0]
        need = inp.requires_grad or anchor.requires_grad
        ctx.planes = 0
        if inp.is_complex():
            zr = torch.view_as_real(inp)
            G8, K = w_ih.shape[1], w_ih.shape[2]
            ctx.planes = R0 = zr.shape[0] * zr.shape[1]
            gx = torch.empty((2 * R0, 2 * G8), dtype=torch.float32, device=inp.device)
            ops.gemm_f32(zr, w_ih, gx, 2 * R0, 2 * G8, K, K, K, 2 * G8, True, a_planes=R0)
            inp = zr
            G4 = G8 // 2
            strides = (G8, S * 2 * G8, 2 * G8)
        elif inp.dim() == 2:
            G8 = w_ih.shape[1]
            gx = _project(inp, w_ih, shared=True)
            G4 = G8 // 2
            strides = (G8, S * 2 * G8, 2 * G8)
        else:
            gx = _project(inp, w_ih, shared=False)
            G4 = gx.shape[-1] // 2
            strides = (B2 * S * 2 * G4, S * 2 * G4, 2 * G4)
        out, gates, c, hprev = ops.lstm_layer(gx, w_hh, 2, B2, S, strides, need, True,
# ... 608 lines not shown
```

dcs-net_amd/dcsnet/ops.py:

```python
import os as _os
import torch

from . import _lib
from ._lib import ACT_NONE, ACT_RELU, ACT_LRELU, ACT_SIGMOID, check, ptr, cur_stream


def _chk(t, name, dims=None, act=False):
    if t is None:
        return
    if not t.is_cuda:
        raise _lib.DcsHipError(f'{name}: expected a CUDA (HIP) tensor; the HIP path has no CPU fallback')
    if t.dtype != torch.float32 and not (act and t.dtype == torch.bfloat16):
        raise _lib.DcsHipError(f'{name}: expected float32{" or bfloat16" if act else ""}, got {t.dtype}')
    if not t.is_contiguous():
        raise _lib.DcsHipError(f'{name}: expected a contiguous tensor')
    if dims is not None and t.dim() != dims:
        raise _lib.DcsHipError(f'{name}: expected {dims} dims, got shape {tuple(t.shape)}')


def _sym(name, *acts):
    dts = {t.dtype for t in acts if t is not None}
    if len(dts) > 1:
        raise _lib.DcsHipError(f'{name}: activation tensors of different dtypes {sorted(str(d) for d in dts)}')
    bf = dts == {torch.bfloat16}
# ... 86 lines not shown
def pack_plan_run(plan):
    global PLAN
    PLAN = plan
    check(_lib.load().dcs_pack_plan_run(plan.handle, cur_stream()), 'dcs_pack_plan_run')
    _plan_snapshot(plan)
    plan.valid = True


def pack_plan_invalidate():
    if PLAN is not None:
        PLAN.valid = False


def pack_plan_drop():
    global PLAN
    PLAN = None



def _workspace(nbytes, device):
    key = (device.index, cur_stream())
    buf = _workspaces.get(key)
    if buf is None or buf.numel() < nbytes:
        if buf is not None:
            _retired.append(buf)
        buf = torch.empty(max(int(nbytes), 1 << 20), dtype=torch.uint8, device=device)
        _workspaces[key] = buf
    return buf


def pack_conv_weight(w_r, w_i, b_r=None, b_i=None, transposed=False, up=(1, 1)):
    for n, t in (('w_r', w_r), ('w_i', w_i), ('b_r', b_r), ('b_i', b_i)):
        _chk(t, n)
    if transposed:
        Cin, Cout, kh, kw = w_r.shape
    else:
        Cout, Cin, kh, kw = w_r.shape
    lib = _lib.load()
    buf = torch.empty(lib.dcs_packed_weight_floats(Cout, Cin, kh, kw, up[0], up[1]), dtype=torch.float32,
                      device=w_r.device)
    wp = buf[:kh * kw * Cin * Cout * 2].view(kh * kw, Cin, Cout, 2)
    bias = torch.empty((Cout, 2), dtype=torch.float32, device=w_r.device)
    check(lib.dcs_pack_conv_weight(ptr(w_r), ptr(w_i), ptr(b_r), ptr(b_i), ptr(wp), ptr(bias),
                                   Cout, Cin, kh, kw, int(bool(transposed)), up[0], up[1], cur_stream()),
          'dcs_pack_conv_weight')
    return wp, bias


def pack_tap_rows(w_r, w_i, ct):
    _chk(w_r, 'w_r', 4)
    _chk(w_i, 'w_i', 4)
    Cin, one, kh, kw = w_r.shape
    if one != 1 or ct < kh * kw:
        raise _lib.DcsHipError(f'pack_tap_rows: expected [Cin,1,kh,kw] and ct >= kh*kw, got {tuple(w_r.shape)}, ct={ct}')
    lib = _lib.load()
    buf = torch.empty(lib.dcs_packed_weight_floats(ct, Cin, 1, 1, 1, 1), dtype=torch.float32, device=w_r.device)
    wp = buf[:Cin * ct * 2].view(1, Cin, ct, 2)
    bias = torch.empty((ct, 2), dtype=torch.float32, device=w_r.device)
    check(lib.dcs_pack_tap_rows(ptr(w_r), ptr(w_i), ptr(wp), ptr(bias), Cin, kh, kw, ct, cur_stream()), 'dcs_pack_tap_rows')
    return wp, bias


def tap_rows_scatter(gt_r, gt_i, w_shape, outs=None):
    Cin, _, kh, kw = w_shape
    acc = outs is not None and outs[0] is not None and outs[1] is not None
    g_r = outs[0] if acc else torch.empty(w_shape, dtype=torch.float32, device=gt_r.device)
    g_i = outs[1] if acc else torch.empty(w_shape, dtype=torch.float32, device=gt_r.device)
    check(_lib.load().dcs_tap_rows_wgrad_scatter(ptr(gt_r), ptr(gt_i), ptr(g_r), ptr(g_i), Cin, kh, kw, int(acc),
                                                 cur_stream()), 'dcs_tap_rows_wgrad_scatter')
    return g_r, g_i


def cconv2d(x1, x2, wp, bias, ksize, stride=(1, 1), pad=(0, 0), up=(1, 1), act=ACT_NONE, coef=None):
    _chk(x1, 'x1', 5, act=True)
    _chk(x2, 'x2', 5, act=True)
    _chk(wp, 'wp', 4)
    _chk(bias, 'bias', 2)
    B, Hin, Win, C1, _ = x1.shape
    C2 = 0
    if x2 is not None:
        if x2.shape[:3] != x1.shape[:3]:
            raise _lib.DcsHipError(f'cconv2d: x1 {tuple(x1.shape)} and x2 {tuple(x2.shape)} differ in B/H/W')
        C2 = x2.shape[3]
    kh, kw = ksize
    if wp.shape[0] != kh * kw or wp.shape[1] != C1 + C2:
        raise _lib.DcsHipError(f'cconv2d: packed weight {tuple(wp.shape)} does not match k={ksize}, Cin={C1 + C2}')
    Cout = wp.shape[2]
    Hout = (Hin * up[0] + 2 * pad[0] - kh) // stride[0] + 1
    Wout = (Win * up[1] + 2 * pad[1] - kw) // stride[1] + 1
    y = torch.empty((B, Hout, Wout, Cout, 2), dtype=x1.dtype, device=x1.device)
    lib = _lib.load()
    nbytes = lib.dcs_cconv2d_fwd_workspace_bytes(B, Hin, Win, C1, C2, up[0], up[1], Cout, kh, kw, stride[0], stride[1],
                                                 pad[0], pad[1])
    ws = _workspace(nbytes, x1.device) if nbytes > 0 else None
    nbytes = max(nbytes, 0)
    ev = (CONV_TIMER.begin(8.0 * B * Hout * Wout * Cout * (C1 + C2) * kh * kw, 'enc_fwd' if max(stride) > 1 else None,
                           executed=_fold_fraction(C1, C1 + C2, Cout, ksize, stride, pad, up),
                           emulated=_emulated(C1 + C2, Cout, kh * kw if tuple(up) == (1, 1) else 0) and (C1 % 2 == 0 or C1 + C2 == 1),
                           nbytes=_conv_bytes(x1, B * Hin * Win * (C1 + C2), B * Hout * Wout * Cout, kh * kw * (C1 + C2) * Cout))
          if CONV_TIMER is not None else None)
    if coef is not None:
        _chk(coef, 'coef', 2)
        if tuple(coef.shape) != (Cout, 6):
            raise _lib.DcsHipError(f'cconv2d: coef {tuple(coef.shape)} does not match Cout={Cout}')
    check(_sym('dcs_cconv2d_fwd_affine', x1, x2)(ptr(x1), ptr(x2), ptr(wp), ptr(bias), ptr(coef), ptr(y), ptr(ws), nbytes, B, Hin, Win,
                                     C1, C2, up[0], up[1], Cout, kh, kw, stride[0], stride[1], pad[0], pad[1], act,
                                     cur_stream()), 'dcs_cconv2d_fwd_affine')
    if ev is not None:
        CONV_TIMER.end(ev)
    return y


def cconv2d_stats(x1, x2, wp, bias, ksize, stride=(1, 1), pad=(0, 0), up=(1, 1)):
    import ctypes
    _chk(x1, 'x1', 5, act=True)
    _chk(x2, 'x2', 5, act=True)
    _chk(wp, 'wp', 4)
    _chk(bias, 'bias', 2)
    B, Hin, Win, C1, _ = x1.shape
    C2 = 0 if x2 is None else x2.shape[3]
    kh, kw = ksize
    Cout = wp.shape[2]
    lib = _lib.load()
    geo = (B, Hin, Win, C1, C2, up[0], up[1], Cout, kh, kw, stride[0], stride[1], pad[0], pad[1])
    rows = lib.dcs_cconv2d_fwd_stats_rows(*geo) if STATS_EPILOGUE else 0
    if rows < 1:
        return cconv2d(x1, x2, wp, bias, ksize, stride, pad, up, ACT_NONE), None
    if x2 is not None and x2.shape[:3] != x1.shape[:3]:
        raise _lib.DcsHipError(f'cconv2d: x1 {tuple(x1.shape)} and x2 {tuple(x2.shape)} differ in B/H/W')
    if wp.shape[0] != kh * kw or wp.shape[1] != C1 + C2:
        raise _lib.DcsHipError(f'cconv2d: packed weight {tuple(wp.shape)} does not match k={ksize}, Cin={C1 + C2}')
    Hout = (Hin * up[0] + 2 * pad[0] - kh) // stride[0] + 1
    Wout = (Win * up[1] + 2 * pad[1] - kw) // stride[1] + 1
    y = torch.empty((B, Hout, Wout, Cout, 2), dtype=x1.dtype, device=x1.device)
    part = torch.empty((Cout, 5, rows), dtype=torch.float32, device=x1.device)
    nbytes = max(lib.dcs_cconv2d_fwd_workspace_bytes(*geo), 0)
    ws = _workspace(nbytes, x1.device) if nbytes > 0 else None
    ev = (CONV_TIMER.begin(8.0 * B * Hout * Wout * Cout * (C1 + C2) * kh * kw, 'enc_fwd' if max(stride) > 1 else None,
                           executed=_fold_fraction(C1, C1 + C2, Cout, ksize, stride, pad, up),
                           emulated=_emulated(C1 + C2, Cout, kh * kw if tuple(up) == (1, 1) else 0) and (C1 % 2 == 0 or C1 + C2 == 1),
                           nbytes=_conv_bytes(x1, B * Hin * Win * (C1 + C2), B * Hout * Wout * Cout, kh * kw * (C1 + C2) * Cout))
          if CONV_TIMER is not None else None)
    used = ctypes.c_int(0)
    check(_sym('dcs_cconv2d_fwd_stats', x1, x2)(ptr(x1), ptr(x2), ptr(wp), ptr(bias), ptr(y), ptr(part), rows, ctypes.byref(used), ptr(ws),
                                    nbytes, *geo, cur_stream()), 'dcs_cconv2d_fwd_stats')
    if ev is not None:
        CONV_TIMER.end(ev)
    return y, (part, used.value, bias)


import os as _os
FUSE_APPLY_POOL = _os.environ.get('DCS_FUSE_APPLY_POOL', '1') != '0'
STATS_EPILOGUE = _os.environ.get('DCS_STATS_EPILOGUE', '1') != '0'


def _conv_bytes(act, n_in, n_out, n_w):
    e = 4.0 if act.dtype == torch.bfloat16 else 8.0
    w = 4.0 if conv_precision() == 'bf16' else 8.0
    return e * (n_in + n_out) + w * n_w


def _emulated(k_channels, n_channels, taps=0):
    if conv_precision() == 'bf16x6' and k_channels == 1 and n_channels == 8 and taps == 49:
        return True
    return (conv_precision() == 'bf16x6' and n_channels % 8 == 0 and
            (k_channels % 16 == 0 or (k_channels == 8 and taps in (49, 16) and n_channels != 8)))


def _wgrad_emulated(C1, Cin, Cout, ksize):
    import os
    if conv_precision() != 'bf16x6' or os.environ.get('DCS_WGRAD_X6', '1') == '0':
        return False
    if Cin % 8 or Cout % 8 or C1 % 2 or ksize[0] != ksize[1]:
        return False
    return ksize[0] in (1, 3, 5) or (ksize[0] == 7 and 16 <= Cout < 32)


def _fold_fraction(C1, Cin, Cout, ksize, stride, pad, up):
    if (tuple(ksize) == (3, 3) and tuple(stride) == (1, 1) and tuple(pad) == (1, 1) and tuple(up) in ((2, 1), (1, 2), (2, 2))
            and Cin % 8 == 0 and Cout % 8 == 0 and C1 % 2 == 0):
        return (2 if up[0] == 2 else 3) * (2 if up[1] == 2 else 3) / 9.0
    return 1.0


def pack_conv_weight_bwd(wp, ksize, stride=(1, 1), pad=(0, 0), up=(1, 1)):
    _chk(wp, 'wp', 4)
    taps, Cin, Cout, _ = wp.shape
    kh, kw = ksize
    plan = PLAN
    key = (wp.data_ptr(), tuple(ksize), tuple(stride), tuple(pad), tuple(up))
    if plan is not None and plan.valid and not plan.recording:
        hit = plan.bwd.get(key)
        if hit is not None:
            return hit
    lib = _lib.load()
    geo = (Cout, Cin, kh, kw, stride[0], stride[1], pad[0], pad[1], up[0], up[1])
    buf = torch.empty(lib.dcs_packed_weight_bwd_floats(*geo), dtype=torch.float32, device=wp.device)
    wpb = buf[:taps * Cin * Cout * 2].view(taps, Cout, Cin, 2)
    check(lib.dcs_pack_conv_weight_bwd(ptr(wp), ptr(wpb), *geo, cur_stream()), 'dcs_pack_conv_weight_bwd')
    if plan is not None and plan.recording:
        plan.bwd[key] = wpb
        plan.keep.append((wp, buf))
    return wpb


def cconv2d_bwd_data(gy, wp_bwd, in_shape, ksize, stride, pad, up=(1, 1), C1=None):
    _chk(gy, 'gy', 5, act=True)
    _chk(wp_bwd, 'wp_bwd', 4)
    B, Hout, Wout, Cout, _ = gy.shape
    Hin, Win, Cin = in_shape
    C1 = Cin if C1 is None else C1
    C2 = Cin - C1
    gx1 = torch.empty((B, Hin, Win, C1, 2), dtype=gy.dtype, device=gy.device)
    gx2 = torch.empty((B, Hin, Win, C2, 2), dtype=gy.dtype, device=gy.device) if C2 else None
    lib = _lib.load()
    geo = (B, Hin, Win, C1, C2, up[0], up[1], Cout, ksize[0], ksize[1], stride[0], stride[1], pad[0], pad[1])
    nbytes = lib.dcs_cconv2d_bwd_data_workspace_bytes(*geo)
    if nbytes < 0:
        raise _lib.DcsHipError(f'cconv2d_bwd_data: unsupported geometry {geo}')
    ws = _workspace(nbytes, gy.device) if nbytes else None
    ev = (CONV_TIMER.begin(8.0 * B * Hout * Wout * Cout * Cin * ksize[0] * ksize[1],
                           executed=_fold_fraction(C1, Cin, Cout, ksize, stride, pad, up), emulated=_emulated(Cout, Cin),
                           nbytes=_conv_bytes(gy, B * Hout * Wout * Cout, B * Hin * Win * Cin, ksize[0] * ksize[1] * Cin * Cout))
          if CONV_TIMER is not None else None)
    check(_sym('dcs_cconv2d_bwd_data', gy)(ptr(gy), ptr(wp_bwd), ptr(gx1), ptr(gx2), ptr(ws), ws.numel() if ws is not None else 0,
                                   *geo, cur_stream()), 'dcs_cconv2d_bwd_data')
    if ev is not None:
        CONV_TIMER.end(ev)
    return gx1, gx2


def cconv2d_bwd_weight(x1, x2, gy, w_shape, has_bias, ksize, stride, pad, up=(1, 1), transposed=False, outs=None, immediate=False):
    _chk(x1, 'x1', 5, act=True)
    _chk(x2, 'x2', 5, act=True)
    _chk(gy, 'gy', 5, act=True)
    B, Hin, Win, C1, _ = x1.shape
    C2 = 0 if x2 is None else x2.shape[3]
    Cout = gy.shape[3]
    dev = gy.device
    o = outs or (None, None, None, None)
    gw_r = o[0] if o[0] is not None else torch.empty(w_shape, dtype=torch.float32, device=dev)
    gw_i = o[1] if o[1] is not None else torch.empty(w_shape, dtype=torch.float32, device=dev)
    gb_r = (o[2] if o[2] is not None else torch.empty(Cout, dtype=torch.float32, device=dev)) if has_bias else None
    gb_i = (o[3] if o[3] is not None else torch.empty(Cout, dtype=torch.float32, device=dev)) if has_bias else None
    for n, t in (('gw_r', gw_r), ('gw_i', gw_i), ('gb_r', gb_r), ('gb_i', gb_i)):
        _chk(t, n)
    lib = _lib.load()
    geo = (B, Hin, Win, C1, C2, up[0], up[1], Cout, ksize[0], ksize[1], stride[0], stride[1], pad[0], pad[1])
    nbytes = lib.dcs_cconv2d_bwd_weight_workspace_bytes(*geo)
    if nbytes < 0:
        raise _lib.DcsHipError(f'cconv2d_bwd_weight: unsupported geometry {geo}')
    scope = WGRAD_DEFER
    all_out = outs is not None and o[0] is not None and o[1] is not None and (not has_bias or (o[2] is not None and o[3] is not None))
    if scope is not None and all_out:
        ws = torch.empty(max(nbytes, 16), dtype=torch.uint8, device=dev)
        scope.append((ws, x1, x2, gy))
    else:
        ws = _workspace(nbytes, dev)
    suspend = scope is not None and (not all_out or immediate)
    if suspend:
        lib.dcs_wgrad_defer_suspend(1)
    ev = None
    if CONV_TIMER is not None:
        ev = CONV_TIMER.begin(8.0 * B * gy.shape[1] * gy.shape[2] * Cout * (C1 + C2) * ksize[0] * ksize[1],
                              executed=_fold_fraction(C1, C1 + C2, Cout, ksize, stride, pad, up),
                              emulated=_wgrad_emulated(C1, C1 + C2, Cout, ksize),
                              nbytes=(_conv_bytes(x1, B * Hin * Win * (C1 + C2) + B * gy.shape[1] * gy.shape[2] * Cout, 0, 0) +
                                      8.0 * ksize[0] * ksize[1] * (C1 + C2) * Cout))
    try:
        check(_sym('dcs_cconv2d_bwd_weight', x1, x2, gy)(ptr(x1), ptr(x2), ptr(gy), ptr(gw_r), ptr(gw_i), ptr(gb_r), ptr(gb_i), ptr(ws),
                                         ws.numel(), *geo, int(bool(transposed)), cur_stream()), 'dcs_cconv2d_bwd_weight')
    finally:
        if suspend:
            lib.dcs_wgrad_defer_suspend(0)
    if ev is not None:
        CONV_TIMER.end(ev)
    return gw_r, gw_i, gb_r, gb_i


WGRAD_DEFER = None


def wgrad_defer_begin():
    global WGRAD_DEFER
    check(_lib.load().dcs_wgrad_defer_begin(), 'dcs_wgrad_defer_begin')
    WGRAD_DEFER = []


def wgrad_defer_flush(partial=False):
    global WGRAD_DEFER
    ev = CONV_TIMER.begin(0.0) if CONV_TIMER is not None else None
    try:
        check(_lib.load().dcs_wgrad_defer_flush(cur_stream()), 'dcs_wgrad_defer_flush')
    finally:
        if not partial:
            WGRAD_DEFER = None
    if partial:
        check(_lib.load().dcs_wgrad_defer_begin(), 'dcs_wgrad_defer_begin')
    if ev is not None:
        CONV_TIMER.end(ev)



def cbn(x, weight, bias, running_mean, running_covar, eps=1e-5, momentum=0.1, use_batch_stats=True,
        act=ACT_NONE, drop_p=0.0, seed=0, out=None, coef_cached=None, stat=None):
    _chk(x, 'x', 5, act=True)
    for n, t in (('weight', weight), ('bias', bias), ('running_mean', running_mean), ('running_covar', running_covar)):
        _chk(t, n)
    B, H, W, C, _ = x.shape
    P = B * H * W
    y = torch.empty_like(x) if out is None else out
    lib = _lib.load()
    if stat is not None and use_batch_stats:
        part, rows, pivot = stat
        _chk(part, 'stat part', 3)
        _chk(pivot, 'stat pivot', 2)
        if part.shape[2] < rows or tuple(part.shape[:2]) != (C, 5) or tuple(pivot.shape) != (C, 2):
            raise _lib.DcsHipError(f'cbn: statistics slabs {tuple(part.shape)} / pivot {tuple(pivot.shape)} do not match C={C}')
        stats = torch.empty((C, 8), dtype=torch.float32, device=x.device)
        coef = torch.empty((C, 6), dtype=torch.float32, device=x.device)
        check(_sym('dcs_cbn_fwd_slabs', x, y)(ptr(x), ptr(y), ptr(weight), ptr(bias), ptr(running_mean), ptr(running_covar), ptr(stats),
                                    ptr(coef), ptr(part), int(rows), int(part.shape[2]), ptr(pivot), P, C, eps,
                                    -1.0 if momentum is None else momentum, act, float(drop_p), int(seed), ptr(SEED_STATE),
                                    cur_stream()), 'dcs_cbn_fwd_slabs')
        return y, stats, coef
    nbytes = lib.dcs_cbn_workspace_bytes(P, C)
    if nbytes < 0:
        raise _lib.DcsHipError(f'cbn: unsupported channel count C={C}')
    ws = _workspace(nbytes, x.device)
    mode = int(bool(use_batch_stats))
    if coef_cached is not None:
        if mode != 0:
            raise _lib.DcsHipError('cbn: cached coefficients are an eval-mode feature')
        stats, coef = coef_cached
        mode = 2
    else:
        stats = torch.empty((C, 8), dtype=torch.float32, device=x.device)
        coef = torch.empty((C, 6), dtype=torch.float32, device=x.device)
    check(_sym('dcs_cbn_fwd', x, y)(ptr(x), ptr(y), ptr(weight), ptr(bias), ptr(running_mean), ptr(running_covar),
                          ptr(stats), ptr(coef), ptr(ws), ws.numel(), P, C, eps,
                          -1.0 if momentum is None else momentum, mode, act,
                          float(drop_p), int(seed), ptr(SEED_STATE), cur_stream()), 'dcs_cbn_fwd')
    return y, stats, coef


def cbn_channel_attention(x, weight, bias, running_mean, running_covar, eps, momentum, act, stat, w1, w2):
    _chk(x, 'x', 5, act=True)
    for n, t in (('weight', weight), ('bias', bias), ('running_mean', running_mean), ('running_covar', running_covar),
                 ('w1', w1), ('w2', w2)):
        _chk(t, n)
    part, rows, pivot = stat
    B, H, W, C, _ = x.shape
    HW = H * W
    Ch = w1.shape[-2]
    lib = _lib.load()
    nch = lib.dcs_ca_pool_chunks(HW, C)
    if nch < 1 or part.shape[2] < rows or tuple(part.shape[:2]) != (C, 5) or tuple(pivot.shape) != (C, 2):
        raise _lib.DcsHipError(f'cbn_channel_attention: unsupported C={C} or mismatching statistics slabs {tuple(part.shape)}')
    dev = x.device
    a = torch.empty_like(x)
    new = lambda *sh: torch.empty(sh, dtype=torch.float32, device=dev)
    stats, coef, ca, pooled, hidden = new(C, 8), new(C, 6), new(B, C, 2), new(B, C, 2), new(B, Ch, 2)
    nbytes = B * nch * C * 2 * 8
    ws = _workspace(nbytes, dev)
    check(_sym('dcs_cbn_fwd_slabs_pool', x, a)(ptr(x), ptr(a), ptr(weight), ptr(bias), ptr(running_mean), ptr(running_covar),
                                              ptr(stats), ptr(coef), ptr(part), int(rows), int(part.shape[2]), ptr(pivot),
                                              ptr(ws), ws.numel(), B, HW, C, eps, -1.0 if momentum is None else momentum, act,
                                              cur_stream()), 'dcs_cbn_fwd_slabs_pool')
    check(lib.dcs_channel_attention_fc_fwd(ptr(ws), ptr(w1), ptr(w2), ptr(ca), ptr(pooled), ptr(hidden), B, HW, C, Ch,
                                           cur_stream()), 'dcs_channel_attention_fc_fwd')
    return a, stats, coef, ca, pooled, hidden


def cbn_bwd(x, g_out, weight, stats, coef, use_batch_stats, act, drop_p=0.0, seed=0, affine=True, outs=None,
            g_add=None, g_out2=None, need_gx=True):
    _chk(x, 'x', 5, act=True)
    _chk(g_out, 'g_out', 5, act=True)
    _chk(g_out2, 'g_out2', 5, act=True)
    if g_out2 is not None and g_out2.shape != g_out.shape:
        raise _lib.DcsHipError(f'cbn_bwd: g_out {tuple(g_out.shape)} vs g_out2 {tuple(g_out2.shape)}')
    B, H, W, C, _ = x.shape
    P = B * H * W
    g_x = torch.empty_like(x) if need_gx else None
    o = outs or (None, None)
    g_w = (o[0] if o[0] is not None else torch.empty((C, 3), dtype=torch.float32, device=x.device)) if affine else None
    g_b = (o[1] if o[1] is not None else torch.empty((C, 2), dtype=torch.float32, device=x.device)) if affine else None
    lib = _lib.load()
    nbytes = lib.dcs_cbn_bwd_workspace_bytes(P, C)
    if nbytes < 0:
        raise _lib.DcsHipError(f'cbn_bwd: unsupported channel count C={C}')
    ws = _workspace(nbytes, x.device)
    if g_add is not None:
        _chk(g_add, 'g_add', 3)
    check(_sym('dcs_cbn_bwd_add', x, g_out, g_out2)(ptr(x), ptr(g_out), ptr(g_x), ptr(weight), ptr(stats), ptr(coef), ptr(g_w), ptr(g_b),
                              ptr(ws), ws.numel(), P, C, int(bool(use_batch_stats)), act, float(drop_p), int(seed),
                              ptr(SEED_STATE), ptr(g_add), 1.0 / (H * W), H * W, ptr(g_out2), cur_stream()), 'dcs_cbn_bwd_add')
    return g_x, g_w, g_b


def channel_attention(x, w1, w2):
    _chk(x, 'x', 5, act=True)
    _chk(w1, 'w1')
    _chk(w2, 'w2')
    B, H, W, C, _ = x.shape
    Ch = w1.shape[-2]
    ca = torch.empty((B, C, 2), dtype=torch.float32, device=x.device)
    pooled = torch.empty((B, C, 2), dtype=torch.float32, device=x.device)
    hidden = torch.empty((B, Ch, 2), dtype=torch.float32, device=x.device)
    lib = _lib.load()
    nbytes = lib.dcs_ca_workspace_bytes(B, H * W, C)
    if nbytes < 0:
        raise _lib.DcsHipError(f'channel_attention: unsupported channel count C={C}')
    ws = _workspace(nbytes, x.device)
    check(_sym('dcs_channel_attention_fwd', x)(ptr(x), ptr(w1), ptr(w2), ptr(ca), ptr(pooled), ptr(hidden), ptr(ws),
                                        ws.numel(), B, H * W, C, Ch, cur_stream()), 'dcs_channel_attention_fwd')
    return ca, pooled, hidden


def spatial_pool(x, ca=None):
    _chk(x, 'x', 5, act=True)
    _chk(ca, 'ca', 3)
    B, H, W, C, _ = x.shape
    pooled = torch.empty((B, H, W, 2, 2), dtype=torch.float32, device=x.device)
    check(_sym('dcs_spatial_pool_fwd', x)(ptr(x), ptr(ca), ptr(pooled), B, H * W, C, cur_stream()),
          'dcs_spatial_pool_fwd')
    return pooled


def attention_apply(x, ca=None, sa=None, drop_p=0.0, seed=0, out=None):
    _chk(x, 'x', 5, act=True)
    _chk(ca, 'ca', 3)
    _chk(sa, 'sa')
    B, H, W, C, _ = x.shape
    y = torch.empty_like(x) if out is None else out
    check(_sym('dcs_attention_apply_fwd', x, y)(ptr(x), ptr(ca), ptr(sa), ptr(y), B, H * W, C, float(drop_p),
                                              int(seed), ptr(SEED_STATE), cur_stream()), 'dcs_attention_apply_fwd')
    return y


def attention_bwd(x, g_out, ca, sa, sp, pooled, hidden, w1, w2, wsa, ksize, drop_p=0.0, seed=0, outs=None,
                  split_pool=False, defer_fc=False):
    _chk(x, 'x', 5, act=True)
    _chk(g_out, 'g_out', 5, act=True)
    B, H, W, C, _ = x.shape
    HW = H * W
    Ch = hidden.shape[1]
    dev = x.device
    lib = _lib.load()
    g_pre = torch.empty((B, H, W, 1, 2), dtype=torch.float32, device=dev)
    check(_sym('dcs_attention_bwd_sa', x, g_out)(ptr(x), ptr(g_out), ptr(ca), ptr(sa), ptr(g_pre), B, HW, C, float(drop_p),
                                   int(seed), ptr(SEED_STATE), cur_stream()), 'dcs_attention_bwd_sa')
    k, pad = (ksize, ksize), (ksize // 2, ksize // 2)
    g_sp, _ = cconv2d_bwd_data(g_pre, pack_conv_weight_bwd(wsa, k, (1, 1), pad), (H, W, 2), k, (1, 1), pad)
    o = outs or (None,) * 6
    g_c1r, g_c1i, _, _ = cconv2d_bwd_weight(sp, None, g_pre, (1, 2, ksize, ksize), False, k, (1, 1), pad,
                                            outs=(o[4], o[5], None, None))
    g_x = torch.empty_like(x)
    new = lambda shape: torch.empty(shape, dtype=torch.float32, device=dev)
    g0r = o[0] if o[0] is not None else new((Ch, C, 1, 1))
    g0i = o[1] if o[1] is not None else new((Ch, C, 1, 1))
    g2r = o[2] if o[2] is not None else new((C, Ch, 1, 1))
    g2i = o[3] if o[3] is not None else new((C, Ch, 1, 1))
    nbytes = lib.dcs_attention_bwd_workspace_bytes(B, HW, C, Ch)
    if nbytes < 0:
        raise _lib.DcsHipError(f'attention_bwd: unsupported channel count C={C}')
    defer_fc = bool(defer_fc and split_pool)
    ws = torch.empty(nbytes, dtype=torch.uint8, device=dev) if defer_fc else _workspace(nbytes, dev)
    g_pooled = new((B, C, 2)) if split_pool else None
    fcp = (None,) * 4 if defer_fc else (g0r, g0i, g2r, g2i)
    check(_sym('dcs_attention_bwd_x', x, g_out)(ptr(x), ptr(g_out), ptr(ca), ptr(sa), ptr(g_sp), ptr(pooled), ptr(hidden), ptr(w1),
                                  ptr(w2), ptr(g_x), ptr(fcp[0]), ptr(fcp[1]), ptr(fcp[2]), ptr(fcp[3]), ptr(g_pooled), ptr(ws),
                                  ws.numel(), B, HW, C, Ch, float(drop_p), int(seed), ptr(SEED_STATE), cur_stream()),
          'dcs_attention_bwd_x')
    if defer_fc:
        return g_x, g0r, g0i, g2r, g2i, g_c1r, g_c1i, g_pooled, (ws, pooled, hidden, g0r, g0i, g2r, g2i, B, HW, C, Ch)
    if split_pool:
        return g_x, g0r, g0i, g2r, g2i, g_c1r, g_c1i, g_pooled
    return g_x, g0r, g0i, g2r, g2i, g_c1r, g_c1i


def attention_bwd_fc_weights(job):
    ws, pooled, hidden, g0r, g0i, g2r, g2i, B, HW, C, Ch = job
    check(_lib.load().dcs_attention_bwd_fc_weights(ptr(ws), ws.numel(), ptr(pooled), ptr(hidden), ptr(g0r), ptr(g0i), ptr(g2r),
                                                   ptr(g2i), B, HW, C, Ch, cur_stream()), 'dcs_attention_bwd_fc_weights')


ATTENTION_BATCH_MAX = 8


def _attention_items(blocks):
    items = (_lib.AttentionItem * len(blocks))()
    for it, blk in zip(items, blocks):
        for k, v in blk.items():
            setattr(it, k, v if isinstance(v, int) else ptr(v))
    return items


def attention_blocks_fwd(xs, w1s, w2s, wsas, biases):
    lib = _lib.load()
    B, dev = xs[0].shape[0], xs[0].device
    new = lambda *shape: torch.empty(shape, dtype=torch.float32, device=dev)
    blocks, outs = [], []
    for x, w1, w2, wsa, bias in zip(xs, w1s, w2s, wsas, biases):
        _chk(x, 'x', 5, act=True)
        _, H, W, C, _ = x.shape
        Ch = w1.shape[-2]
        o = dict(y=torch.empty_like(x), ca=new(B, C, 2), pooled=new(B, C, 2), hidden=new(B, Ch, 2), sp=new(B, H, W, 2, 2),
                 sa=new(B, H, W, 1, 2))
        blocks.append(dict(x=x, w1=w1, w2=w2, wsa=wsa, sa_bias=bias, H=H, W=W, C=C, Ch=Ch, **o))
        outs.append(o)
    items = _attention_items(blocks)
    n = len(blocks)
    nbytes = lib.dcs_attention_fwd_batched_workspace_bytes(n, items, B)
    if nbytes < 0:
        raise _lib.DcsHipError('attention_blocks_fwd: unsupported block geometry')
    ws = _workspace(nbytes, dev)
    check(_sym('dcs_attention_fwd_batched', *xs)(n, items, ptr(ws), ws.numel(), B, cur_stream()), 'dcs_attention_fwd_batched')
    return outs


def attention_blocks_bwd(saved, g_outs, wsa_bwds, fc_outs, split_pool=None):
    lib = _lib.load()
    B, dev = g_outs[0].shape[0], g_outs[0].device
    blocks, res = [], []
    split_pool = split_pool or (False,) * len(saved)
    for (sv, g, wb, fo), split in zip(zip(saved, g_outs, wsa_bwds, fc_outs), split_pool):
        _chk(g, 'g_out', 5, act=True)
        x = sv['x']
        _, H, W, C, _ = x.shape
        g_pre = torch.empty((B, H, W, 1, 2), dtype=torch.float32, device=dev)
        g_sp = torch.empty((B, H, W, 2, 2), dtype=torch.float32, device=dev)
        g_x = torch.empty_like(x)
        g_pooled = torch.empty((B, C, 2), dtype=torch.float32, device=dev) if split else None
        blocks.append(dict(x=x, w1=sv['w1'], w2=sv['w2'], ca=sv['ca'], pooled=sv['pooled'], hidden=sv['hidden'], sa=sv['sa'],
                           g_out=g, wsa_bwd=wb, g_pre=g_pre, g_sp=g_sp, g_x=g_x, g_fc0_r=fo[0], g_fc0_i=fo[1], g_fc2_r=fo[2],
                           g_fc2_i=fo[3], H=H, W=W, C=C, Ch=sv['hidden'].shape[1], **({'g_pooled': g_pooled} if split else {})))
        res.append((g_x, g_pre, g_pooled))
    items = _attention_items(blocks)
    n = len(blocks)
    nbytes = lib.dcs_attention_bwd_batched_workspace_bytes(n, items, B)
    if nbytes < 0:
        raise _lib.DcsHipError('attention_blocks_bwd: unsupported block geometry')
    ws = _workspace(nbytes, dev)
    check(_sym('dcs_attention_bwd_batched', *g_outs, *[sv['x'] for sv in saved])(n, items, ptr(ws), ws.numel(), B, cur_stream()), 'dcs_attention_bwd_batched')
    return res


def lstm_layer(gx, w_hh, n_sets, seqs_per_set, S, strides, save=False, save_hprev=False, bias=None):
    _chk(gx, 'gx')
    _chk(w_hh, 'w_hh', 4)
    H = w_hh.shape[-1]
    NS = n_sets * seqs_per_set
    out = torch.empty((NS, S, 2 * H), dtype=torch.float32, device=gx.device)
    gates = torch.empty((NS, S, 2, 4 * H), dtype=torch.float32, device=gx.device) if save else None
    c = torch.empty((NS, S, 2, H), dtype=torch.float32, device=gx.device) if save else None
    hprev = torch.empty((NS, S, 2, H), dtype=torch.float32, device=gx.device) if save and save_hprev else None
    ba, bb = (None, None) if bias is None else bias
    _chk(ba, 'bias_a')
    _chk(bb, 'bias_b')
    check(_lib.load().dcs_lstm_layer_fwd_bias(ptr(gx), ptr(w_hh), ptr(ba), ptr(bb), ptr(out), ptr(gates), ptr(c), ptr(hprev),
                                              n_sets, seqs_per_set, S, H, strides[0], strides[1], strides[2], cur_stream()),
          'dcs_lstm_layer_fwd_bias')
    return (out, gates, c, hprev) if save_hprev else (out, gates, c)


def lstm_layer_bwd(g_out, gates, c, w_hh, n_sets, seqs_per_set, S, bias_part=False):
    _chk(g_out, 'g_out', 3)
    _chk(gates, 'gates', 4)
    _chk(c, 'c', 4)
    _chk(w_hh, 'w_hh', 4)
    g_pre = torch.empty_like(gates)
    part = torch.empty((gates.shape[0], 2, gates.shape[-1]), dtype=torch.float32, device=gates.device) if bias_part else None
    check(_lib.load().dcs_lstm_layer_bwd(ptr(g_out), ptr(gates), ptr(c), ptr(w_hh), ptr(g_pre), ptr(part), n_sets,
                                         seqs_per_set, S, w_hh.shape[-1], cur_stream()), 'dcs_lstm_layer_bwd')
    return (g_pre, part) if bias_part else g_pre


def dropout(x, drop_p, seed, out=None):
    _chk(x, 'x')
    y = torch.empty_like(x) if out is None else out
    check(_lib.load().dcs_dropout_fwd(ptr(x), ptr(y), x.numel(), float(drop_p), int(seed), ptr(SEED_STATE), cur_stream()),
          'dcs_dropout_fwd')
    return y


def complex_act(x, act, out=None):
    _chk(x, 'x')
    y = torch.empty_like(x) if out is None else out
    check(_lib.load().dcs_complex_act_fwd(ptr(x), ptr(y), x.numel(), act, cur_stream()), 'dcs_complex_act_fwd')
    return y


def complex_upsample(x, up):
    _chk(x, 'x', 5)
    B, H, W, C, _ = x.shape
    y = torch.empty((B, H * up[0], W * up[1], C, 2), dtype=torch.float32, device=x.device)
    check(_lib.load().dcs_complex_upsample_fwd(ptr(x), ptr(y), B, H, W, C, up[0], up[1], cur_stream()),
          'dcs_complex_upsample_fwd')
    return y


def tapsum(z, ksize, up, pad, backward=False, grad=None, bias=None, bias_grad=None, out_dtype=torch.float32):
    lib = _lib.load()
    if not backward:
        _chk(z, 'z', 5)
        B, Hs, Ws, CT, _ = z.shape
        y = torch.empty((B, Hs * up[0], Ws * up[1], 1, 2), dtype=torch.float32, device=z.device)
        b_r, b_i = bias if bias is not None else (None, None)
        check(lib.dcs_tapsum_fwd(ptr(z), ptr(y), ptr(b_r), ptr(b_i), B, Hs, Ws, CT, ksize[0], ksize[1], up[0], up[1],
                                 pad[0], pad[1], cur_stream()), 'dcs_tapsum_fwd')
        return y
    _chk(grad, 'grad', 5)
    B, Hs, Ws, CT, _ = z
    gz = torch.empty((B, Hs, Ws, CT, 2), dtype=out_dtype, device=grad.device)
    gb_r, gb_i = bias_grad if bias_grad is not None else (None, None)
    ws = _workspace(lib.dcs_tapsum_bwd_workspace_bytes(), grad.device) if gb_r is not None else None
    check(_sym('dcs_tapsum_bwd', gz)(ptr(grad), ptr(gz), ptr(gb_r), ptr(gb_i), ptr(ws), 0 if ws is None else ws.numel(), B, Hs, Ws, CT,
                             ksize[0], ksize[1], up[0], up[1], pad[0], pad[1], cur_stream()), 'dcs_tapsum_bwd')
    return gz


def cconv_up2_single(x1, x2, wt, b_r, b_i):
    _chk(x1, 'x1', 5, act=True)
    _chk(x2, 'x2', 5, act=True)
    _chk(wt, 'wt', 4)
    B, Hs, Ws, C1, _ = x1.shape
    C2 = 0 if x2 is None else x2.shape[3]
    y = torch.empty((B, 2 * Hs, 2 * Ws, 1, 2), dtype=torch.float32, device=x1.device)
    check(_sym('dcs_cconv_up2_single_fwd', x1, x2)(ptr(x1), ptr(x2), ptr(wt), ptr(b_r), ptr(b_i), ptr(y), B, Hs, Ws, C1, C2,
                                               wt.shape[2], cur_stream()), 'dcs_cconv_up2_single_fwd')
    return y


def cconv_up2_single_bwd_data(gy, wt, C1, C2, out_dtype=torch.float32):
    _chk(gy, 'gy', 5)
    _chk(wt, 'wt', 4)
    B, Ho, Wo = gy.shape[:3]
    Hs, Ws = Ho // 2, Wo // 2
    gx1 = torch.empty((B, Hs, Ws, C1, 2), dtype=out_dtype, device=gy.device)
    gx2 = torch.empty((B, Hs, Ws, C2, 2), dtype=out_dtype, device=gy.device) if C2 else None
    ev = (CONV_TIMER.begin(8.0 * B * Hs * Ws * 16 * (C1 + C2), emulated=True,
                           nbytes=gy.numel() * 4.0 + B * Hs * Ws * (C1 + C2) * 2.0 * gx1.element_size())
          if CONV_TIMER is not None else None)
    check(_sym('dcs_cconv_up2_single_bwd_data', gx1, gx2)(ptr(gy), ptr(wt), ptr(gx1), ptr(gx2), B, Hs, Ws, C1, C2, wt.shape[2],
                                                          cur_stream()), 'dcs_cconv_up2_single_bwd_data')
    if ev is not None:
        CONV_TIMER.end(ev)
    return gx1, gx2


def cconv_up2_single_bwd_weight(gy, x1, x2, w_shape, outs=None, bias_outs=None):
    _chk(gy, 'gy', 5)
    _chk(x1, 'x1', 5, act=True)
    _chk(x2, 'x2', 5, act=True)
    B, Hs, Ws, C1, _ = x1.shape
    C2 = 0 if x2 is None else x2.shape[3]
    acc = outs is not None and outs[0] is not None and outs[1] is not None
    g_r = outs[0] if acc else torch.empty(w_shape, dtype=torch.float32, device=gy.device)
    g_i = outs[1] if acc else torch.empty(w_shape, dtype=torch.float32, device=gy.device)
    gb_r, gb_i = bias_outs if bias_outs is not None else (None, None)
    lib = _lib.load()
    ws = _workspace(lib.dcs_cconv_up2_single_bwd_weight_workspace_bytes(), gy.device)
    ev = (CONV_TIMER.begin(8.0 * B * Hs * Ws * 16 * (C1 + C2), emulated=True,
                           nbytes=gy.numel() * 4.0 + B * Hs * Ws * (C1 + C2) * 2.0 * x1.element_size())
          if CONV_TIMER is not None else None)
    check(_sym('dcs_cconv_up2_single_bwd_weight', x1, x2)(ptr(gy), ptr(x1), ptr(x2), ptr(g_r), ptr(g_i), ptr(gb_r), ptr(gb_i), int(acc),
                                                            ptr(ws), ws.numel(), B, Hs, Ws, C1, C2, cur_stream()),
          'dcs_cconv_up2_single_bwd_weight')
# ... 715 lines not shown
```

include/dcsnet_hip.h:

```cpp
#ifndef DCSNET_HIP_H
#define DCSNET_HIP_H

#ifdef __cplusplus
extern "C" {
#endif

typedef void* dcs_stream_t;

#define DCS_OK              0
#define DCS_ERR_BADARG     (-1)
#define DCS_ERR_LAUNCH     (-2)
#define DCS_ERR_WORKSPACE  (-3)

#define DCS_ACT_NONE   0
#define DCS_ACT_RELU   1
#define DCS_ACT_LRELU  2
#define DCS_ACT_SIGMOID 3

int         dcs_abi_version(void);
const char* dcs_error_string(int code);

long dcs_packed_weight_floats(int Cout, int Cin, int kh, int kw, int up_f, int up_t);
int dcs_pack_conv_weight(const float* w_r, const float* w_i, const float* b_r, const float* b_i,
                         float* wp, float* bias_out,
                         int Cout, int Cin, int kh, int kw, int transposed, int up_f, int up_t,
                         dcs_stream_t stream);

long dcs_cconv2d_fwd_workspace_bytes(int B, int Hin, int Win, int C1, int C2, int up_f, int up_t,
                                     int Cout, int kh, int kw, int sf, int st, int pad_f, int pad_t);
int dcs_cconv2d_fwd(const float* x1, const float* x2, const float* wp, const float* bias, float* y,
                    void* workspace, long workspace_bytes,
                    int B, int Hin, int Win, int C1, int C2, int up_f, int up_t,
                    int Cout, int kh, int kw, int sf, int st, int pad_f, int pad_t, int act,
                    dcs_stream_t stream);

int dcs_cconv2d_fwd_stats_rows(int B, int Hin, int Win, int C1, int C2, int up_f, int up_t,
                               int Cout, int kh, int kw, int sf, int st, int pad_f, int pad_t);
int dcs_cconv2d_fwd_stats(const float* x1, const float* x2, const float* wp, const float* bias, float* y,
                          float* stat, int stat_rows, int* rows_used, void* workspace, long workspace_bytes,
                          int B, int Hin, int Win, int C1, int C2, int up_f, int up_t,
                          int Cout, int kh, int kw, int sf, int st, int pad_f, int pad_t, dcs_stream_t stream);

int dcs_cconv2d_fwd_affine(const float* x1, const float* x2, const float* wp, const float* bias, const float* coef, float* y,
                           void* workspace, long workspace_bytes,
                           int B, int Hin, int Win, int C1, int C2, int up_f, int up_t,
                           int Cout, int kh, int kw, int sf, int st, int pad_f, int pad_t, int act,
                           dcs_stream_t stream);

long dcs_rconv2d_fwd_workspace_bytes(int B, int Hin, int Win, int C1r, int C2r, int up_f, int up_t, int Coutr,
                                     int kh, int kw, int sf, int st, int pad_f, int pad_t);
int dcs_rconv2d_fwd(const float* x1, const float* x2, const float* bm, const float* bias, float* y,
                    void* workspace, long workspace_bytes,
                    int B, int Hin, int Win, int C1r, int C2r, int up_f, int up_t,
                    int Coutr, int kh, int kw, int sf, int st, int pad_f, int pad_t, int act,
                    dcs_stream_t stream);
long dcs_rconv2d_bwd_data_workspace_bytes(int B, int Hv, int Wv, int Cinr, int Coutr, int kh, int kw, int sf, int st,
                                          int pad_f, int pad_t);
int dcs_rconv2d_bwd_data(const float* gy, const float* bm_bwd, float* gxv, void* workspace, long workspace_bytes,
                         int B, int Hv, int Wv, int Cinr, int Coutr, int kh, int kw, int sf, int st, int pad_f, int pad_t,
                         dcs_stream_t stream);

int dcs_rbn_fwd(const float* x, float* y, const float* weight, const float* bias, float* running_mean, float* running_var,
                float* stats_out, float* coef_out, void* workspace, long workspace_bytes, long P, int Cr, float eps,
                float momentum, int use_batch_stats, int act, dcs_stream_t stream);
int dcs_rbn_bwd(const float* x, const float* g_out, float* g_x, const float* stats, const float* coef, float* g_weight,
                float* g_bias, void* workspace, long workspace_bytes, long P, int Cr, int use_batch_stats, int act,
                dcs_stream_t stream);

long dcs_packed_weight_bwd_floats(int Cout, int Cin, int kh, int kw, int sf, int st, int pad_f, int pad_t,
                                  int up_f, int up_t);
int  dcs_pack_conv_weight_bwd(const float* wp, float* wp_bwd, int Cout, int Cin, int kh, int kw,
                              int sf, int st, int pad_f, int pad_t, int up_f, int up_t, dcs_stream_t stream);
long dcs_cconv2d_bwd_data_workspace_bytes(int B, int Hin, int Win, int C1, int C2, int up_f, int up_t,
                                          int Cout, int kh, int kw, int sf, int st, int pad_f, int pad_t);
int  dcs_cconv2d_bwd_data(const float* gy, const float* wp_bwd, float* gx1, float* gx2,
                          void* workspace, long workspace_bytes,
                          int B, int Hin, int Win, int C1, int C2, int up_f, int up_t,
                          int Cout, int kh, int kw, int sf, int st, int pad_f, int pad_t, dcs_stream_t stream);
int  dcs_upsample_cat_bwd(const float* gxv, float* gx1, float* gx2, int B, int Hin, int Win, int C1, int C2,
                          int up_f, int up_t, dcs_stream_t stream);
long dcs_cconv2d_bwd_weight_workspace_bytes(int B, int Hin, int Win, int C1, int C2, int up_f, int up_t,
                                            int Cout, int kh, int kw, int sf, int st, int pad_f, int pad_t);
int  dcs_cconv2d_bwd_weight(const float* x1, const float* x2, const float* gy,
                            float* gw_r, float* gw_i, float* gb_r, float* gb_i,
                            void* workspace, long workspace_bytes,
                            int B, int Hin, int Win, int C1, int C2, int up_f, int up_t,
                            int Cout, int kh, int kw, int sf, int st, int pad_f, int pad_t, int transposed,
                            dcs_stream_t stream);

long dcs_cbn_workspace_bytes(long P, int C);
int  dcs_cbn_fwd(const float* x, float* y, const float* weight, const float* bias,
                 float* running_mean, float* running_covar,
                 float* stats_out, float* coef_out, void* workspace, long workspace_bytes,
                 long P, int C, float eps, float momentum, int use_batch_stats, int act,
                 float drop_p, unsigned long long seed, const unsigned long long* seed_dev, dcs_stream_t stream);

int  dcs_cbn_fwd_slabs(const float* x, float* y, const float* weight, const float* bias,
                       float* running_mean, float* running_covar, float* stats_out, float* coef_out,
                       const float* part, int rows, int stride, const float* pivot,
                       long P, int C, float eps, float momentum, int act,
                       float drop_p, unsigned long long seed, const unsigned long long* seed_dev, dcs_stream_t stream);

int dcs_ca_pool_chunks(long HW, int C);
int dcs_cbn_fwd_slabs_pool(const float* x, float* y, const float* weight, const float* bias,
                           float* running_mean, float* running_covar, float* stats_out, float* coef_out,
                           const float* part, int rows, int stride, const float* pivot, void* pool_part, long pool_bytes,
                           int B, long HW, int C, float eps, float momentum, int act, dcs_stream_t stream);
int dcs_channel_attention_fc_fwd(const void* pool_part, const float* w1, const float* w2, float* ca_out, float* pooled_out,
                                 float* hidden_out, int B, long HW, int C, int Ch, dcs_stream_t stream);

long dcs_cbn_bwd_workspace_bytes(long P, int C);
int  dcs_cbn_bwd(const float* x, const float* g_out, float* g_x, const float* weight,
                 const float* stats, const float* coef, float* g_weight, float* g_bias,
                 void* workspace, long workspace_bytes, long P, int C, int use_batch_stats, int act,
                 float drop_p, unsigned long long seed, const unsigned long long* seed_dev, dcs_stream_t stream);
int  dcs_cbn_bwd_add(const float* x, const float* g_out, float* g_x, const float* weight, const float* stats,
                     const float* coef, float* g_weight, float* g_bias, void* workspace, long workspace_bytes,
                     long P, int C, int use_batch_stats, int act, float drop_p, unsigned long long seed,
                     const unsigned long long* seed_dev, const float* g_add, float add_scale, long HW,
                     const float* g_out2, dcs_stream_t stream);

long dcs_ca_workspace_bytes(int B, long HW, int C);
int  dcs_channel_attention_fwd(const float* x, const float* w1, const float* w2,
                               float* ca_out, float* pooled_out, float* hidden_out,
                               void* workspace, long workspace_bytes,
                               int B, long HW, int C, int Ch, dcs_stream_t stream);

int dcs_spatial_pool_fwd(const float* x, const float* ca, float* pooled,
                         int B, long HW, int C, dcs_stream_t stream);

int dcs_attention_apply_fwd(const float* x, const float* ca, const float* sa, float* y,
                            int B, long HW, int C, float drop_p, unsigned long long seed,
                            const unsigned long long* seed_dev, dcs_stream_t stream);

typedef struct {
    const float* x; const float* w1; const float* w2; const float* wsa; const float* sa_bias;
    float* ca; float* pooled; float* hidden; float* sp; float* sa; float* y;
    const float* g_out; const float* wsa_bwd; float* g_pre; float* g_sp; float* g_x;
    float* g_fc0_r; float* g_fc0_i; float* g_fc2_r; float* g_fc2_i;
    int H, W, C, Ch;
    float* g_pooled;
} dcs_attention_item;
long dcs_attention_fwd_batched_workspace_bytes(int n, const dcs_attention_item* items, int B);
int dcs_attention_fwd_batched(int n, const dcs_attention_item* items, void* workspace, long workspace_bytes, int B,
                              dcs_stream_t stream);
long dcs_attention_bwd_batched_workspace_bytes(int n, const dcs_attention_item* items, int B);
int dcs_attention_bwd_batched(int n, const dcs_attention_item* items, void* workspace, long workspace_bytes, int B,
                              dcs_stream_t stream);

long dcs_rattention_workspace_bytes(int B, long HW, int C);
int  dcs_rattention_fwd(const float* x, const float* w1, const float* w2, const float* wsa, const float* sa_bias,
                        float* ca_out, float* y, void* workspace, long workspace_bytes,
                        int B, int H, int W, int C, int Ch, int ksize, dcs_stream_t stream);

long dcs_rattention_train_workspace_bytes(int B, long HW, int C, int Ch);
int  dcs_rattention_pool_fwd(const float* x, const float* w1, const float* w2, float* ca_out, float* mx_out, float* hid_out,
                             float* pooled, void* workspace, long workspace_bytes, int B, int H, int W, int C, int Ch,
                             dcs_stream_t stream);
int  dcs_rattention_apply_fwd(const float* x, const float* ca, const float* sa, float* y, int B, int H, int W, int C,
                              dcs_stream_t stream);
int  dcs_rattention_apply_bwd(const float* gy, const float* x, const float* ca, const float* sa, float* gx, float* g_sa,
                              float* g_ca, void* workspace, long workspace_bytes, int B, int H, int W, int C,
                              dcs_stream_t stream);
int  dcs_rattention_pool_bwd(const float* g_pooled, const float* g_ca, const float* x, const float* ca, const float* mx,
                             const float* hid, const float* w1, const float* w2, float* gx, float* gw1, float* gw2,
                             int accumulate, void* workspace, long workspace_bytes, int B, int H, int W, int C, int Ch,
                             dcs_stream_t stream);

int  dcs_attention_bwd_sa(const float* x, const float* g_out, const float* ca, const float* sa, float* g_pre,
                          int B, long HW, int C, float drop_p, unsigned long long seed, const unsigned long long* seed_dev, dcs_stream_t stream);
long dcs_attention_bwd_workspace_bytes(int B, long HW, int C, int Ch);
int  dcs_attention_bwd_x(const float* x, const float* g_out, const float* ca, const float* sa, const float* g_sp,
                         const float* pooled, const float* hidden, const float* w1, const float* w2,
                         float* g_x, float* g_fc0_r, float* g_fc0_i, float* g_fc2_r, float* g_fc2_i, float* g_pooled,
                         void* workspace, long workspace_bytes, int B, long HW, int C, int Ch,
                         float drop_p, unsigned long long seed, const unsigned long long* seed_dev, dcs_stream_t stream);
int dcs_attention_bwd_fc_weights(const void* workspace, long workspace_bytes, const float* pooled, const float* hidden,
                                 float* g_fc0_r, float* g_fc0_i, float* g_fc2_r, float* g_fc2_i, int B, long HW, int C, int Ch,
                                 dcs_stream_t stream);

int dcs_lstm_layer_fwd(const float* gx, const float* w_hh, float* out, float* gates_save, float* c_save,
                       float* hprev_save, int n_sets, int seqs_per_set, int S, int H, long stride_set, long stride_n, long stride_t,
                       dcs_stream_t stream);

int dcs_lstm_layer_fwd_bias(const float* gx, const float* w_hh, const float* bias_a, const float* bias_b, float* out,
                            float* gates_save, float* c_save, float* hprev_save, int n_sets, int seqs_per_set, int S,
                            int Hdim, long stride_set, long stride_n, long stride_t, dcs_stream_t stream);
int dcs_lstm_layer_bwd(const float* g_out, const float* gates, const float* c_save, const float* w_hh,
                       float* g_pre, float* g_bias_part, int n_sets, int seqs_per_set, int S, int H, dcs_stream_t stream);

int dcs_lstm_whh_grad(const float* g_pre, const float* h_prev, float* part, int NT, int CK, int H, dcs_stream_t stream);
int dcs_atb_chunks(const float* A, const float* B, float* part, long a_lo, long a_hi, long b_lo, long b_hi, int nlo, int nhi,
                   int lda, int ldb, int M, int N, int R, int CK, dcs_stream_t stream);
int dcs_chunk_sum_acc(const float* part, float* out, long o_lo, long o_hi, int nlo, int nhi, int CK, long MN,
                      dcs_stream_t stream);
int dcs_atb_chunks_strided(const float* A, const float* B, float* part, long a_lo, long a_hi, long b_lo, long b_hi, int nlo,
                           int nhi, int lda, int ldb, int b_es, int M, int N, int R, int CK, dcs_stream_t stream);
int dcs_gemm_f32(const float* A, const float* B, float* C, int M, int N, int K, int lda, int ldb, int ldc, int b_transposed,
                 int nseg, long a_seg, long b_seg, int nbatch, long a_batch, long b_batch, long c_batch, int a_planes,
                 int c_planes, dcs_stream_t stream);
int dcs_lstm_combine_fwd(const float* o, float* out, long n, dcs_stream_t stream);
int dcs_lstm_combine_bwd(const float* g, float* g_o, long n, dcs_stream_t stream);
int dcs_lstm_param_grads(const float* part, const float* b_part, float* g_whh, float* g_bih, float* g_bhh, int CK,
                         int seqs_per_set, int H, dcs_stream_t stream);
int dcs_lstm_param_grads_ih(const float* part, const float* b_part, float* g_whh, float* g_bih, float* g_bhh, int CK,
                            int seqs_per_set, int H, const float* part_ih, float* g_wih, int CK_ih, long MN_ih, int nsets,
                            dcs_stream_t stream);

int dcs_dropout_fwd(const float* x, float* y, long n, float drop_p, unsigned long long seed,
                    const unsigned long long* seed_dev, dcs_stream_t stream);

int dcs_complex_act_fwd(const float* x, float* y, long n_floats, int act, dcs_stream_t stream);
int dcs_complex_upsample_fwd(const float* x, float* y, int B, int H, int W, int C, int up_f, int up_t,
                             dcs_stream_t stream);

int dcs_tapsum_fwd(const float* z, float* y, const float* b_r, const float* b_i, int B, int Hs, int Ws, int CT,
                   int kh, int kw, int up_f, int up_t, int pad_f, int pad_t, dcs_stream_t stream);
long dcs_tapsum_bwd_workspace_bytes(void);
int dcs_tapsum_bwd(const float* gy, float* gz, float* gb_r, float* gb_i, void* workspace, long workspace_bytes,
                   int B, int Hs, int Ws, int CT, int kh, int kw, int up_f, int up_t, int pad_f, int pad_t,
                   dcs_stream_t stream);

int dcs_cconv_up2_single_fwd(const float* x1, const float* x2, const float* wt, const float* b_r, const float* b_i,
                             float* y, int B, int Hs, int Ws, int C1, int C2, int ct, dcs_stream_t stream);

int dcs_cconv_up2_single_bwd_data(const float* gy, const float* wt, float* gx1, float* gx2, int B, int Hs, int Ws, int C1, int C2,
                                  int ct, dcs_stream_t stream);
long dcs_cconv_up2_single_bwd_weight_workspace_bytes(void);
int dcs_cconv_up2_single_bwd_weight(const float* gy, const float* x1, const float* x2, float* gw_r, float* gw_i, float* gb_r,
                                    float* gb_i, int accumulate, void* workspace, long workspace_bytes, int B, int Hs, int Ws,
                                    int C1, int C2, dcs_stream_t stream);

int dcs_bound_crm_fwd(const float* M_raw, float* M_out, long n, float eps, dcs_stream_t stream);

int dcs_bound_mask_apply_fwd(const float* Y, const float* M_in, float* M_out, float* N_hat, float* S_hat,
                             long n, float eps, dcs_stream_t stream);

int dcs_bound_mask_apply_bwd(const float* Y, const float* M_in, const float* g_M, const float* g_N,
                             const float* g_S, float* g_Min, long n, float eps, dcs_stream_t stream);

int dcs_bound2_mask_apply_fwd(const float* Y, const float* D_raw, float* M1_out, float* M_out, float* N_hat, float* S_hat,
                              long n, float eps, float drop_p, unsigned long long seed, const unsigned long long* seed_dev,
                              dcs_stream_t stream);
int dcs_bound2_mask_apply_bwd(const float* Y, const float* D_raw, const float* g_M1, const float* g_M, const float* g_N,
                              const float* g_S, float* g_D, long n, float eps, float drop_p, unsigned long long seed,
                              const unsigned long long* seed_dev, dcs_stream_t stream);

int dcs_bound2_apply_polar_frames_fwd(const float* Y, const float* D_raw, float* M_out, float* out, int B, int F, int Fp, int T,
                                      float eps, float drop_p, unsigned long long seed, const unsigned long long* seed_dev,
                                      dcs_stream_t stream);
int dcs_bound2_apply_polar_frames_bwd(const float* Y, const float* D_raw, const float* g_out, const float* g_M, float* g_D,
                                      int B, int F, int Fp, int T, float eps, int hermitian, float drop_p,
                                      unsigned long long seed, const unsigned long long* seed_dev, dcs_stream_t stream);

int dcs_complex_abs_f32(const float* Y, float* out, long n, dcs_stream_t stream);
int dcs_rmask_apply_polar_frames_fwd(const float* Y, const float* D, float* M_out, float* out, int B, int F, int Fp, int T,
                                     float eps, int pair, dcs_stream_t stream);
int dcs_rmask_apply_polar_frames_bwd(const float* Y, const float* D, const float* g_out, const float* g_M, float* g_D,
                                     int B, int F, int Fp, int T, float eps, int hermitian, int pair, dcs_stream_t stream);

int dcs_irfft512_frames(const float* X, float* y, long frames, dcs_stream_t stream);
int dcs_rfft512_frames(const float* g, float* G, long frames, dcs_stream_t stream);
int dcs_rfft512_ola_frames(const float* g_y, const float* window, const float* inv_env, float* G, int B, int T, int hop,
                           float scale, dcs_stream_t stream);
int dcs_irfft512_ola_frames(const float* X, const float* window, const float* inv_env, float* y, int B, int T, int hop,
                            float scale, dcs_stream_t stream);
int dcs_polar_frames_fwd(const float* z, float* out, int B, int F, int Fp, int T, float eps, dcs_stream_t stream);
int dcs_polar_frames_bwd(const float* z, const float* g_out, float* g_z, int B, int F, int Fp, int T, float eps,
                         int hermitian, dcs_stream_t stream);
int dcs_istft_envelope(const float* window, float* inv_env, int T, int n_fft, int hop, dcs_stream_t stream);
int dcs_istft_ola_fwd(const float* frames, const float* window, const float* inv_env, float* y, int B, int T,
                      int n_fft, int hop, float scale, dcs_stream_t stream);
int dcs_istft_ola_bwd(const float* g_y, const float* window, const float* inv_env, float* g_frames, int B, int T,
                      int n_fft, int hop, float scale, dcs_stream_t stream);

int dcs_sisnr_fwd(const float* clean, const float* est, float* snr, float* coef, int B, int L, float eps,
                  dcs_stream_t stream);
int dcs_sisnr_bwd(const float* clean, const float* est, const float* coef, const float* g, float scale, float* g_est,
                  int B, int L, dcs_stream_t stream);

int dcs_sisnr_losses_fwd(const float* snr_speech, const float* snr_noise, float* out3, int B, float alpha,
                         dcs_stream_t stream);
int dcs_sisnr_losses_guard_fwd(const float* snr_speech, const float* snr_noise, float* out3, int B, float alpha,
                               float* skip, dcs_stream_t stream);
int dcs_sisnr_pair_bwd(const float* target, const float* est, const float* coef, const float* g_noise,
                       const float* g_speech, const float* g_total, float alpha, float* g_est, int B, int L,
                       dcs_stream_t stream);

int dcs_stft_frames_fwd(const float* clean, const float* noisy, const float* window, float* frames, int B, int L, int T,
                        int n_fft, int hop, dcs_stream_t stream);
int dcs_stft_bins_fwd(const float* spec, float* out, int SB, int T, int F, float scale, dcs_stream_t stream);

int dcs_crm_fwd(const float* S, const float* Y, float* M, long n, float eps, dcs_stream_t stream);

int dcs_adam_amsgrad_step(float* p, const float* g, float* m, float* v, float* vmax,
                          const float* grad_norm, float max_norm, float grad_scale, long n,
                          const float* lr, float beta1, float beta2, float eps, float weight_decay, int step,
                          const int* step_dev, const float* skip, dcs_stream_t stream);
int dcs_grad_sumsq_parts(const float* g, long n, double* parts, int n_parts, const float* skip, int* step_dev, long long* seed_dev,
                         long long* counters, int n_counters, dcs_stream_t stream);
int dcs_adam_amsgrad_step_sumsq(float* p, const float* g, float* m, float* v, float* vmax, const double* sumsq_parts, int n_parts,
                                float max_norm, float grad_scale, long n, const float* lr, float beta1, float beta2, float eps,
                                float weight_decay, int step, const int* step_dev, const float* skip, dcs_stream_t stream);

int dcs_swa_average_f32(float* avg, const float* p, long n, long n_averaged, dcs_stream_t stream);

int dcs_step_guard(const float* loss, float* skip, dcs_stream_t stream);
int dcs_stream_hold(const int* host_flag, int timeout_ms, dcs_stream_t stream);
int dcs_kernel_timer_begin(int slot);
int dcs_kernel_timer_end(void);
int dcs_kernel_timer_read(int slot, float* ms);
int dcs_step_advance(const float* skip, int* step_dev, long long* seed_dev, dcs_stream_t stream);
int dcs_step_advance_counters(const float* skip, int* step_dev, long long* seed_dev, long long* counters, int n_counters,
                              dcs_stream_t stream);

int dcs_pack_tap_rows(const float* w_r, const float* w_i, float* wp, float* bias_out, int Cin, int kh, int kw, int ct,
                      dcs_stream_t stream);
int dcs_tap_rows_wgrad_scatter(const float* gt_r, const float* gt_i, float* gw_r, float* gw_i, int Cin, int kh, int kw,
                               int accumulate, dcs_stream_t stream);

int dcs_set_conv_precision(int mode);
int dcs_get_conv_precision(void);

int dcs_wgrad_defer_begin(void);
int dcs_wgrad_defer_suspend(int suspended);
int dcs_wgrad_defer_flush(dcs_stream_t stream);

int dcs_pack_plan_begin(void);
int dcs_pack_plan_end(void** plan_out);
int dcs_pack_plan_jobs(const void* plan, int* n_jobs, int* n_launches);
int dcs_pack_plan_run(const void* plan, dcs_stream_t stream);
int dcs_pack_plan_destroy(void* plan);

int dcs_resample_poly_f32(const float* x, float* y, int rows, long L, const float* h, int taps, int up, int down,
                          dcs_stream_t stream);
long dcs_stoi_workspace_bytes(int B, long L10);
int dcs_stoi_f32(const float* clean10, const float* est10, int B, long L10, const int* band_lo, const int* band_hi,
                 float* out_d, int* out_kept, void* workspace, long workspace_bytes, dcs_stream_t stream);

int dcs_resample_poly_ragged_f32(const float* x, const long* offsets, int n, long total, float* y, long* out_offsets,
                                 long out_capacity, const float* h, int taps, int up, int down, dcs_stream_t stream);
long dcs_stoi_ragged_workspace_bytes(int n, long total10);
int dcs_stoi_ragged_f32(const float* clean10, const float* est10, const long* offsets, int n, long total10, long longest10,
                        const int* band_lo, const int* band_hi, float* out_d, int* out_kept, void* workspace,
                        long workspace_bytes, dcs_stream_t stream);
int dcs_sisnr_ragged_f32(const float* clean, const float* est, const long* offsets, int n, long total, float* out,
                         dcs_stream_t stream);

int dcs_resample_sinc_f32(const float* x, const long* x_off, float* y, const long* y_off, int rows, long total_out,
                          const float* taps, int orig, int new_, int width, dcs_stream_t stream);
int dcs_audio_stft_batch_f32(const float* clean, const float* noisy, const long* offsets, int n_items, const int* item_index,
                             const int* item_start, int B, const float* window, int n_fft, int T, int hop, float scale,
                             float* out_noise, float* out_noisy, float* out_clean, dcs_stream_t stream);

int dcs_audio_stft_segments_f32(const float* noisy, const long* offsets, int n_items, const int* seg_item,
                                const int* seg_first_frame, int S, const float* window, int n_fft, int T, int overlap, int hop,
                                float scale, float* out, dcs_stream_t stream);
int dcs_segments_stitch_f32(const float* seg, long seg_rows, const int* seg_first, const long* offsets, int n_items,
                            long total_out, int T, int overlap, int hop, float* y, short* pcm, dcs_stream_t stream);

typedef unsigned short dcs_bf16_t;
int dcs_cconv2d_fwd_h(const dcs_bf16_t* x1, const dcs_bf16_t* x2, const float* wp, const float* bias, dcs_bf16_t* y,
                      void* workspace, long workspace_bytes,
                      int B, int Hin, int Win, int C1, int C2, int up_f, int up_t,
                      int Cout, int kh, int kw, int sf, int st, int pad_f, int pad_t, int act, dcs_stream_t stream);
int dcs_cconv2d_fwd_affine_h(const dcs_bf16_t* x1, const dcs_bf16_t* x2, const float* wp, const float* bias, const float* coef,
                             dcs_bf16_t* y, void* workspace, long workspace_bytes,
                             int B, int Hin, int Win, int C1, int C2, int up_f, int up_t,
                             int Cout, int kh, int kw, int sf, int st, int pad_f, int pad_t, int act, dcs_stream_t stream);
int dcs_cconv2d_fwd_stats_h(const dcs_bf16_t* x1, const dcs_bf16_t* x2, const float* wp, const float* bias, dcs_bf16_t* y,
                            float* stat, int stat_rows, int* rows_used, void* workspace, long workspace_bytes,
                            int B, int Hin, int Win, int C1, int C2, int up_f, int up_t,
                            int Cout, int kh, int kw, int sf, int st, int pad_f, int pad_t, dcs_stream_t stream);
int dcs_cconv2d_bwd_data_h(const dcs_bf16_t* gy, const float* wp_bwd, dcs_bf16_t* gx1, dcs_bf16_t* gx2,
                           void* workspace, long workspace_bytes,
                           int B, int Hin, int Win, int C1, int C2, int up_f, int up_t,
                           int Cout, int kh, int kw, int sf, int st, int pad_f, int pad_t, dcs_stream_t stream);
int dcs_cconv2d_bwd_weight_h(const dcs_bf16_t* x1, const dcs_bf16_t* x2, const dcs_bf16_t* gy,
                             float* gw_r, float* gw_i, float* gb_r, float* gb_i, void* workspace, long workspace_bytes,
                             int B, int Hin, int Win, int C1, int C2, int up_f, int up_t,
                             int Cout, int kh, int kw, int sf, int st, int pad_f, int pad_t, int transposed,
                             dcs_stream_t stream);
int dcs_cconv_up2_single_fwd_h(const dcs_bf16_t* x1, const dcs_bf16_t* x2, const float* wt, const float* b_r, const float* b_i,
                               float* y, int B, int Hs, int Ws, int C1, int C2, int ct, dcs_stream_t stream);
int dcs_cconv_up2_single_bwd_data_h(const float* gy, const float* wt, dcs_bf16_t* gx1, dcs_bf16_t* gx2, int B, int Hs, int Ws, int C1,
                                    int C2, int ct, dcs_stream_t stream);
int dcs_cconv_up2_single_bwd_weight_h(const float* gy, const dcs_bf16_t* x1, const dcs_bf16_t* x2, float* gw_r, float* gw_i,
                                      float* gb_r, float* gb_i, int accumulate, void* workspace, long workspace_bytes, int B, int Hs,
                                      int Ws, int C1, int C2, dcs_stream_t stream);
int dcs_tapsum_bwd_h(const float* gy, dcs_bf16_t* gz, float* gb_r, float* gb_i, void* workspace, long workspace_bytes,
                     int B, int Hs, int Ws, int CT, int kh, int kw, int up_f, int up_t, int pad_f, int pad_t,
                     dcs_stream_t stream);
int dcs_cbn_fwd_h(const dcs_bf16_t* x, dcs_bf16_t* y, const float* weight, const float* bias,
                  float* running_mean, float* running_covar, float* stats_out, float* coef_out,
                  void* workspace, long workspace_bytes, long P, int C, float eps, float momentum, int use_batch_stats,
                  int act, float drop_p, unsigned long long seed, const unsigned long long* seed_dev, dcs_stream_t stream);
int dcs_cbn_fwd_slabs_h(const dcs_bf16_t* x, dcs_bf16_t* y, const float* weight, const float* bias,
                        float* running_mean, float* running_covar, float* stats_out, float* coef_out,
                        const float* part, int rows, int stride, const float* pivot,
                        long P, int C, float eps, float momentum, int act,
                        float drop_p, unsigned long long seed, const unsigned long long* seed_dev, dcs_stream_t stream);
int dcs_cbn_fwd_slabs_pool_h(const dcs_bf16_t* x, dcs_bf16_t* y, const float* weight, const float* bias,
                             float* running_mean, float* running_covar, float* stats_out, float* coef_out,
                             const float* part, int rows, int stride, const float* pivot, void* pool_part, long pool_bytes,
                             int B, long HW, int C, float eps, float momentum, int act, dcs_stream_t stream);
int dcs_cbn_bwd_h(const dcs_bf16_t* x, const dcs_bf16_t* g_out, dcs_bf16_t* g_x, const float* weight,
                  const float* stats, const float* coef, float* g_weight, float* g_bias,
                  void* workspace, long workspace_bytes, long P, int C, int use_batch_stats, int act,
                  float drop_p, unsigned long long seed, const unsigned long long* seed_dev, dcs_stream_t stream);
int dcs_cbn_bwd_add_h(const dcs_bf16_t* x, const dcs_bf16_t* g_out, dcs_bf16_t* g_x, const float* weight, const float* stats,
                      const float* coef, float* g_weight, float* g_bias, void* workspace, long workspace_bytes,
                      long P, int C, int use_batch_stats, int act, float drop_p, unsigned long long seed,
                      const unsigned long long* seed_dev, const float* g_add, float add_scale, long HW,
                      const dcs_bf16_t* g_out2, dcs_stream_t stream);
int dcs_channel_attention_fwd_h(const dcs_bf16_t* x, const float* w1, const float* w2,
                                float* ca_out, float* pooled_out, float* hidden_out,
                                void* workspace, long workspace_bytes, int B, long HW, int C, int Ch, dcs_stream_t stream);
int dcs_spatial_pool_fwd_h(const dcs_bf16_t* x, const float* ca, float* pooled, int B, long HW, int C, dcs_stream_t stream);
int dcs_attention_apply_fwd_h(const dcs_bf16_t* x, const float* ca, const float* sa, dcs_bf16_t* y,
                              int B, long HW, int C, float drop_p, unsigned long long seed,
                              const unsigned long long* seed_dev, dcs_stream_t stream);
int dcs_attention_fwd_batched_h(int n, const dcs_attention_item* items, void* workspace, long workspace_bytes, int B,
                                dcs_stream_t stream);
int dcs_attention_bwd_sa_h(const dcs_bf16_t* x, const dcs_bf16_t* g_out, const float* ca, const float* sa, float* g_pre,
                           int B, long HW, int C, float drop_p, unsigned long long seed, const unsigned long long* seed_dev,
                           dcs_stream_t stream);
int dcs_attention_bwd_x_h(const dcs_bf16_t* x, const dcs_bf16_t* g_out, const float* ca, const float* sa, const float* g_sp,
                          const float* pooled, const float* hidden, const float* w1, const float* w2,
                          dcs_bf16_t* g_x, float* g_fc0_r, float* g_fc0_i, float* g_fc2_r, float* g_fc2_i, float* g_pooled,
                          void* workspace, long workspace_bytes, int B, long HW, int C, int Ch,
                          float drop_p, unsigned long long seed, const unsigned long long* seed_dev, dcs_stream_t stream);
int dcs_attention_bwd_batched_h(int n, const dcs_attention_item* items, void* workspace, long workspace_bytes, int B,
                                dcs_stream_t stream);

#ifdef __cplusplus
}
#endif
#endif
```

Baseline: 2.584 million.

## Fuse encoder CBN apply with channel-attention pooling and reuse slabs in attention forward

Adds a CBN forward variant that applies the normalisation, activation and dropout, then writes per-chunk channel-sum slabs as a by-product. These slabs are passed through autograd to the batched attention forward, which skips its own pooling pass for blocks that already have slabs. The aim is to remove one full read of the encoder activations and one kernel launch per attention block, at the cost of extra float64 slab storage and added plumbing through the autograd function.

```diff
diff --git a/dcs-net_amd/csrc/attention.hip b/dcs-net_amd/csrc/attention.hip
--- a/dcs-net_amd/csrc/attention.hip
+++ b/dcs-net_amd/csrc/attention.hip
@@ -251,7 +251,7 @@
 #ifndef DCS_ACT_BF16
 extern "C" int dcs_ca_pool_chunks(long HW, int C) {
     int G;
-    if (HW <= 0 || !att_geom(C, &G)) return -1;
+    if (HW <= 0 || !att::pool_geom(C, &G)) return -1;
     return ca_chunks(HW, G);
 }
 
@@ -298,12 +298,13 @@
     return DCS_OK;
 }
 
-static long fwd_batched_workspace_bytes(int n, const dcs_attention_item* items, int B) {
+static long fwd_batched_workspace_bytes(int n, const dcs_attention_item* items, int B, const void* const* pool_parts = nullptr) {
     if (n < 1 || n > kMaxBatch || !items || B <= 0) return -1;
     long total = 0;
     for (int i = 0; i < n; ++i) {
         int G;
         if (!att_geom(items[i].C, &G)) return -1;
+        if (pool_parts && pool_parts[i]) continue;
         const long b = (long)B * ca_chunks((long)items[i].H * items[i].W, G) * items[i].C * 2 * (long)sizeof(double);
         total += (b + 255) / 256 * 256;
     }
@@ -316,13 +317,15 @@
 }
 #endif
 
-extern "C" int DCS_SYM(dcs_attention_fwd_batched)(int n, const dcs_attention_item* items, void* workspace, long workspace_bytes, int B,
-                                         dcs_stream_t stream) {
-    if (n < 1 || n > kMaxBatch || !items || !workspace || B <= 0 || B > 65535) return DCS_ERR_BADARG;
-    if (workspace_bytes < fwd_batched_workspace_bytes(n, items, B)) return DCS_ERR_WORKSPACE;
+static int attention_fwd_batched_impl(int n, const dcs_attention_item* items, const void* const* pool_parts, void* workspace,
+                                      long workspace_bytes, int B, dcs_stream_t stream) {
+    if (n < 1 || n > kMaxBatch || !items || B <= 0 || B > 65535) return DCS_ERR_BADARG;
+    const long need = fwd_batched_workspace_bytes(n, items, B, pool_parts);
+    if (need < 0) return DCS_ERR_BADARG;
+    if (need > 0 && (!workspace || workspace_bytes < need)) return DCS_ERR_WORKSPACE;
     Tbl<CaPoolP> tp; Tbl<CaFcP> tf; Tbl<SpPoolP> ts; Tbl<ApplyP> ta;
     conv::Args ca_[kMaxBatch];
-    int nx_pool = 1, nx_stream = 1;
+    int nx_pool = 1, nx_stream = 1, npool = 0;
     char* ws = (char*)workspace;
     for (int i = 0; i < n; ++i) {
         const dcs_attention_item& it = items[i];
@@ -332,12 +335,16 @@
             return DCS_ERR_BADARG;
         const long HW = (long)it.H * it.W;
         const int nch = ca_chunks(HW, G), nxs = stream_grid(HW, G, B);
-        tp.p[i] = CaPoolP{(const act_t*)it.x, (double*)ws, HW, it.C, G, nch};
-        tf.p[i] = CaFcP{(const double*)ws, nch, (const float2*)it.w1, (const float2*)it.w2, (float2*)it.ca, (float2*)it.pooled,
+        const double* slabs = pool_parts ? (const double*)pool_parts[i] : nullptr;
+        if (!slabs) {
+            tp.p[npool++] = CaPoolP{(const act_t*)it.x, (double*)ws, HW, it.C, G, nch};
+            slabs = (const double*)ws;
+            ws += ((long)B * nch * it.C * 2 * (long)sizeof(double) + 255) / 256 * 256;
+        }
+        tf.p[i] = CaFcP{slabs, nch, (const float2*)it.w1, (const float2*)it.w2, (float2*)it.ca, (float2*)it.pooled,
                         (float2*)it.hidden, HW, it.C, it.Ch};
         ts.p[i] = SpPoolP{(const act_t*)it.x, it.ca, (float4*)it.sp, HW, it.C, G, nxs};
         ta.p[i] = ApplyP{(const act_t*)it.x, it.ca, (const float2*)it.sa, (act_t*)it.y, HW, it.C, G, nxs};
-        ws += ((long)B * nch * it.C * 2 * (long)sizeof(double) + 255) / 256 * 256;
         nx_pool = nch > nx_pool ? nch : nx_pool;
         nx_stream = nxs > nx_stream ? nxs : nx_stream;
         conv::Args& a = ca_[i];
@@ -352,14 +359,17 @@
     {
         int ap = 0, as_ = 0;
         for (int k = 0; k <= kMaxBatch; ++k) {
-            tp.x0[k] = k < n ? ap : 0x7fffffff; ts.x0[k] = ta.x0[k] = k < n ? as_ : 0x7fffffff;
-            if (k < n) { ap += tp.p[k].nx; as_ += ts.p[k].nx; }
-        }
-        tp.x0[n] = ap; ts.x0[n] = ta.x0[n] = as_;
+            tp.x0[k] = k < npool ? ap : 0x7fffffff; ts.x0[k] = ta.x0[k] = k < n ? as_ : 0x7fffffff;
+            if (k < npool) ap += tp.p[k].nx;
+            if (k < n) as_ += ts.p[k].nx;
+        }
+        tp.x0[npool] = ap; ts.x0[n] = ta.x0[n] = as_;
         nx_pool = ap; nx_stream = as_;
     }
-    DCS_LAUNCH(ca_pool_multi_kernel, dim3(nx_pool, B, 1), dim3(kThreads), 0, s, tp);
-    DCS_CHECK_LAUNCH();
+    if (npool > 0) {
+        DCS_LAUNCH(ca_pool_multi_kernel, dim3(nx_pool, B, 1), dim3(kThreads), 0, s, tp);
+        DCS_CHECK_LAUNCH();
+    }
     DCS_LAUNCH(ca_fc_multi_kernel, dim3(B, 1, n), dim3(kThreads), 0, s, tf);
     DCS_CHECK_LAUNCH();
     DCS_LAUNCH(spatial_pool_multi_kernel, dim3(nx_stream, B, 1), dim3(kThreads), 0, s, ts);
@@ -369,6 +379,17 @@
     DCS_LAUNCH(attention_apply_multi_kernel, dim3(nx_stream, B, 1), dim3(kThreads), 0, s, ta);
     DCS_CHECK_LAUNCH();
     return DCS_OK;
+}
+
+extern "C" int DCS_SYM(dcs_attention_fwd_batched)(int n, const dcs_attention_item* items, void* workspace, long workspace_bytes, int B,
+                                         dcs_stream_t stream) {
+    if (!workspace) return DCS_ERR_BADARG;
+    return attention_fwd_batched_impl(n, items, nullptr, workspace, workspace_bytes, B, stream);
+}
+
+extern "C" int DCS_SYM(dcs_attention_fwd_batched_pooled)(int n, const dcs_attention_item* items, const void* const* pool_parts,
+                                                         void* workspace, long workspace_bytes, int B, dcs_stream_t stream) {
+    return attention_fwd_batched_impl(n, items, pool_parts, workspace, workspace_bytes, B, stream);
 }
 
 #ifndef DCS_ACT_BF16
diff --git a/dcs-net_amd/csrc/cbn.hip b/dcs-net_amd/csrc/cbn.hip
--- a/dcs-net_amd/csrc/cbn.hip
+++ b/dcs-net_amd/csrc/cbn.hip
@@ -325,19 +325,23 @@
 
 __device__ __forceinline__ float stored(float v) { return DCS_ACT_IS_BF16 ? dcs_bf16_to_f32(dcs_f32_to_bf16(v)) : v; }
 
-template <int ACT>
+template <int ACT, bool DROP, typename ACC>
 __global__ __launch_bounds__(kThreads) void cbn_apply_pool_kernel(const act_t* __restrict__ x, act_t* __restrict__ y,
                                                                    const float* __restrict__ coef, double* __restrict__ part,
-                                                                   long HW, int C, int G) {
+                                                                   long HW, int C, int G, float drop_p, uint64_t seed,
+                                                                   const uint64_t* __restrict__ seed_dev) {
     __shared__ double red[kThreads * 4];
+    if (DROP && seed_dev) seed += seed_dev[0];
+    const float inv_keep = DROP ? 1.f / (1.f - drop_p) : 1.f;
     const int t = threadIdx.x, g = t % G, r0 = t / G, rpi = kThreads / G;
     const int b = blockIdx.y, bx = blockIdx.x, gx = gridDim.x;
-    const ActIn4<act_t> x4 = act_in4(x) + (long)b * HW * G;
-    const ActOut4<act_t> y4 = act_out4(y) + (long)b * HW * G;
+    const long base = (long)b * HW * G;
+    const ActIn4<act_t> x4 = act_in4(x) + base;
+    const ActOut4<act_t> y4 = act_out4(y) + base;
     const float* ca = coef + 12 * g;
     const float a0 = ca[0], a1 = ca[1], a2 = ca[2], a3 = ca[3], c0 = ca[4], c1 = ca[5];
     const float e0 = ca[6], e1 = ca[7], e2 = ca[8], e3 = ca[9], f0 = ca[10], f1 = ca[11];
-    float s0 = 0.f, s1 = 0.f, s2 = 0.f, s3 = 0.f;
+    ACC s0 = 0, s1 = 0, s2 = 0, s3 = 0;
     for (long r = (long)bx * rpi + r0; r < HW; r += (long)gx * rpi) {
         const float4 v = x4[r * G + g];
         float4 o;
@@ -345,8 +349,15 @@
         o.y = act_fn<ACT>(fmaf(a2, v.x, fmaf(a3, v.y, c1)));
         o.z = act_fn<ACT>(fmaf(e0, v.z, fmaf(e1, v.w, f0)));
         o.w = act_fn<ACT>(fmaf(e2, v.z, fmaf(e3, v.w, f1)));
+        if (DROP) {
+            const uint64_t e = (uint64_t)(base + r * G + g) * 4;
+            o.x *= dcs_keep_scale(seed, e, drop_p, inv_keep);
+            o.y *= dcs_keep_scale(seed, e + 1, drop_p, inv_keep);
+            o.z *= dcs_keep_scale(seed, e + 2, drop_p, inv_keep);
+            o.w *= dcs_keep_scale(seed, e + 3, drop_p, inv_keep);
+        }
         y4[r * G + g] = o;
-        s0 += stored(o.x); s1 += stored(o.y); s2 += stored(o.z); s3 += stored(o.w);
+        s0 += (ACC)stored(o.x); s1 += (ACC)stored(o.y); s2 += (ACC)stored(o.z); s3 += (ACC)stored(o.w);
     }
     red[t * 4 + 0] = s0; red[t * 4 + 1] = s1; red[t * 4 + 2] = s2; red[t * 4 + 3] = s3;
     __syncthreads();
@@ -448,12 +459,44 @@
     DCS_LAUNCH((cbn_finalize_kernel<float, float>), dim3(C), dim3(256), 0, s, pivot, part, rows, stride, weight, bias,
                running_mean, running_covar, stats_out, coef_out, P, C, eps, momentum, 1);
     DCS_CHECK_LAUNCH();
-#define DCS_CBN_AP(A) DCS_LAUNCH((cbn_apply_pool_kernel<A>), dim3(nch, B), dim3(kThreads), 0, s, x, y, (const float*)coef_out, \
-                                 (double*)pool_part, HW, C, G)
+#define DCS_CBN_AP(A) DCS_LAUNCH((cbn_apply_pool_kernel<A, false, float>), dim3(nch, B), dim3(kThreads), 0, s, x, y, \
+                                 (const float*)coef_out, (double*)pool_part, HW, C, G, 0.f, (uint64_t)0, (const uint64_t*)nullptr)
     if (act == DCS_ACT_RELU) DCS_CBN_AP(DCS_ACT_RELU);
     else if (act == DCS_ACT_LRELU) DCS_CBN_AP(DCS_ACT_LRELU);
     else DCS_CBN_AP(DCS_ACT_NONE);
 #undef DCS_CBN_AP
+    DCS_CHECK_LAUNCH();
+    return DCS_OK;
+}
+
+extern "C" int DCS_SYM(dcs_cbn_fwd_slabs_pool_drop)(const act_t* x, act_t* y, const float* weight, const float* bias,
+                                                    float* running_mean, float* running_covar, float* stats_out, float* coef_out,
+                                                    const float* part, int rows, int stride, const float* pivot, void* pool_part,
+                                                    long pool_bytes, int B, long HW, int C, float eps, float momentum, int act,
+                                                    float drop_p, unsigned long long seed, const unsigned long long* seed_dev,
+                                                    dcs_stream_t stream) {
+    int G;
+    if (!x || !y || !stats_out || !coef_out || !part || !pivot || !pool_part || B <= 0 || B > 65535 || HW <= 0 ||
+        !att::pool_geom(C, &G) || rows < 1 || stride < rows)
+        return DCS_ERR_BADARG;
+    if ((weight == nullptr) != (bias == nullptr)) return DCS_ERR_BADARG;
+    if (act != DCS_ACT_NONE && act != DCS_ACT_RELU && act != DCS_ACT_LRELU) return DCS_ERR_BADARG;
+    if (!(drop_p >= 0.f && drop_p < 1.f)) return DCS_ERR_BADARG;
+    const int nch = att::ca_chunks(HW, G);
+    if (pool_bytes < (long)B * nch * C * 2 * (long)sizeof(double)) return DCS_ERR_WORKSPACE;
+    hipStream_t s = dcs_stream(stream);
+    const long P = (long)B * HW;
+    DCS_LAUNCH((cbn_finalize_kernel<float, float>), dim3(C), dim3(256), 0, s, pivot, part, rows, stride, weight, bias,
+               running_mean, running_covar, stats_out, coef_out, P, C, eps, momentum, 1);
+    DCS_CHECK_LAUNCH();
+#define DCS_CBN_APD(A, D) DCS_LAUNCH((cbn_apply_pool_kernel<A, D, double>), dim3(nch, B), dim3(kThreads), 0, s, x, y, \
+                                     (const float*)coef_out, (double*)pool_part, HW, C, G, drop_p, (uint64_t)seed,       \
+                                     (const uint64_t*)seed_dev)
+    const bool drop = drop_p > 0.f;
+    if (act == DCS_ACT_RELU) { if (drop) DCS_CBN_APD(DCS_ACT_RELU, true); else DCS_CBN_APD(DCS_ACT_RELU, false); }
+    else if (act == DCS_ACT_LRELU) { if (drop) DCS_CBN_APD(DCS_ACT_LRELU, true); else DCS_CBN_APD(DCS_ACT_LRELU, false); }
+    else { if (drop) DCS_CBN_APD(DCS_ACT_NONE, true); else DCS_CBN_APD(DCS_ACT_NONE, false); }
+#undef DCS_CBN_APD
     DCS_CHECK_LAUNCH();
     return DCS_OK;
 }
diff --git a/dcs-net_amd/csrc/cbn_geom.h b/dcs-net_amd/csrc/cbn_geom.h
--- a/dcs-net_amd/csrc/cbn_geom.h
+++ b/dcs-net_amd/csrc/cbn_geom.h
@@ -62,6 +62,13 @@
     *G = g;
     return true;
 }
+inline bool pool_geom(int C, int* G) {
+    if (C < 2 || (C & 1)) return false;
+    const int g = C / 2;
+    if (g > 256 || (256 % g) != 0) return false;
+    *G = g;
+    return true;
+}
 inline int ca_chunks(long HW, int G) {
     const int rows_per_iter = 256 / G;
     const long it = (HW + rows_per_iter - 1) / rows_per_iter;
diff --git a/dcs-net_amd/dcsnet/_lib.py b/dcs-net_amd/dcsnet/_lib.py
--- a/dcs-net_amd/dcsnet/_lib.py
+++ b/dcs-net_amd/dcsnet/_lib.py
@@ -48,6 +48,7 @@
     'dcs_cbn_fwd_slabs': (_I, [_P] * 9 + [_I, _I, _P, _L, _I, _F, _F, _I, _F, _U64, _P, _P]),
     'dcs_ca_pool_chunks': (_I, [_L, _I]),
     'dcs_cbn_fwd_slabs_pool': (_I, [_P] * 9 + [_I, _I, _P, _P, _L, _I, _L, _I, _F, _F, _I, _P]),
+    'dcs_cbn_fwd_slabs_pool_drop': (_I, [_P] * 9 + [_I, _I, _P, _P, _L, _I, _L, _I, _F, _F, _I, _F, _U64, _P, _P]),
     'dcs_channel_attention_fc_fwd': (_I, [_P] * 6 + [_I, _L, _I, _I, _P]),
     'dcs_cbn_bwd_workspace_bytes': (_L, [_L, _I]),
     'dcs_cbn_bwd': (_I, [_P] * 9 + [_L, _L, _I, _I, _I, _F, _U64, _P, _P]),
@@ -69,6 +70,7 @@
     'dcs_attention_bwd_fc_weights': (_I, [_P, _L, _P, _P, _P, _P, _P, _P, _I, _L, _I, _I, _P]),
     'dcs_attention_fwd_batched_workspace_bytes': (_L, [_I, _P, _I]),
     'dcs_attention_fwd_batched': (_I, [_I, _P, _P, _L, _I, _P]),
+    'dcs_attention_fwd_batched_pooled': (_I, [_I, _P, _P, _P, _L, _I, _P]),
     'dcs_attention_bwd_batched_workspace_bytes': (_L, [_I, _P, _I]),
     'dcs_attention_bwd_batched': (_I, [_I, _P, _P, _L, _I, _P]),
     'dcs_lstm_layer_fwd': (_I, [_P] * 6 + [_I, _I, _I, _I, _L, _L, _L, _P]),
@@ -164,8 +166,8 @@
 
 
 for _n in ('dcs_cconv2d_fwd', 'dcs_cconv2d_fwd_affine', 'dcs_cconv2d_fwd_stats', 'dcs_cconv2d_bwd_data', 'dcs_cconv2d_bwd_weight',
-           'dcs_cconv_up2_single_fwd', 'dcs_cconv_up2_single_bwd_data', 'dcs_cconv_up2_single_bwd_weight', 'dcs_tapsum_bwd', 'dcs_cbn_fwd', 'dcs_cbn_fwd_slabs', 'dcs_cbn_fwd_slabs_pool', 'dcs_cbn_bwd', 'dcs_cbn_bwd_add',
-           'dcs_channel_attention_fwd', 'dcs_spatial_pool_fwd', 'dcs_attention_apply_fwd', 'dcs_attention_fwd_batched',
+           'dcs_cconv_up2_single_fwd', 'dcs_cconv_up2_single_bwd_data', 'dcs_cconv_up2_single_bwd_weight', 'dcs_tapsum_bwd', 'dcs_cbn_fwd', 'dcs_cbn_fwd_slabs', 'dcs_cbn_fwd_slabs_pool', 'dcs_cbn_fwd_slabs_pool_drop', 'dcs_cbn_bwd', 'dcs_cbn_bwd_add',
+           'dcs_channel_attention_fwd', 'dcs_spatial_pool_fwd', 'dcs_attention_apply_fwd', 'dcs_attention_fwd_batched', 'dcs_attention_fwd_batched_pooled',
            'dcs_attention_bwd_sa', 'dcs_attention_bwd_x', 'dcs_attention_bwd_batched'):
     SIGNATURES[_n + '_h'] = SIGNATURES[_n]
 
diff --git a/dcs-net_amd/dcsnet/functional.py b/dcs-net_amd/dcsnet/functional.py
--- a/dcs-net_amd/dcsnet/functional.py
+++ b/dcs-net_amd/dcsnet/functional.py
@@ -195,17 +195,25 @@
 
     @staticmethod
     def forward(ctx, x, weight, bias, running_mean, running_covar, eps, momentum, use_batch_stats, act, drop_p, seed, stat=None):
-        y, stats, coef = ops.cbn(x, weight, bias, running_mean, running_covar, eps, momentum, use_batch_stats,
-                                 act, drop_p, seed, stat=stat)
+        slabs = None
+        if stat is not None and use_batch_stats and weight is not None and ops.ENC_POOL and ops.cbn_pool_ok(x):
+            y, stats, coef, slabs = ops.cbn_pool(x, weight, bias, running_mean, running_covar, eps, momentum, act, drop_p,
+                                                 seed, stat)
+        else:
+            y, stats, coef = ops.cbn(x, weight, bias, running_mean, running_covar, eps, momentum, use_batch_stats,
+                                     act, drop_p, seed, stat=stat)
         ctx.cfg = (bool(use_batch_stats), act, float(drop_p), int(seed), weight is not None)
         ctx.sinks = (_sink(weight), _sink(bias))
         ctx.save_for_backward(x, weight, stats, coef)
         ctx.set_materialize_grads(False)
         y2 = torch.empty(0, dtype=y.dtype, device=y.device).set_(y.untyped_storage(), y.storage_offset(), y.shape, y.stride())
-        return y, y2
-
-    @staticmethod
-    def backward(ctx, g_a, g_b):
+        if slabs is None:
+            slabs = torch.empty(0, dtype=torch.float64, device=y.device)
+        ctx.mark_non_differentiable(slabs)
+        return y, y2, slabs
+
+    @staticmethod
+    def backward(ctx, g_a, g_b, _g_slabs=None):
         x, weight, stats, coef = ctx.saved_tensors
         use_batch, act, drop_p, seed, affine = ctx.cfg
         if g_a is None and g_b is None:
@@ -229,9 +237,11 @@
 
 def cbn_two(x, weight, bias, running_mean, running_covar, eps, momentum, use_batch_stats, act=ACT_NONE,
             drop_p=0.0, seed=0, stat=None):
-    y, y2 = _CbnTwoFn.apply(x, weight, bias, running_mean, running_covar, eps, momentum, use_batch_stats, act,
-                            drop_p, seed, stat)
+    y, y2, slabs = _CbnTwoFn.apply(x, weight, bias, running_mean, running_covar, eps, momentum, use_batch_stats, act,
+                                   drop_p, seed, stat)
     y2._dcs_adds_pool_term = True
+    if slabs.numel():
+        y2._dcs_pool_slabs = slabs
     return y, y2
 
 
@@ -332,7 +342,7 @@
 class _AttentionBlocksFn(torch.autograd.Function):
 
     @staticmethod
-    def forward(ctx, n, ksize, split, *args):
+    def forward(ctx, n, ksize, split, slabs, *args):
         xs, params = args[:n], [args[n + 6 * i:n + 6 * i + 6] for i in range(n)]
         ctx.split = tuple(split)
         w1s, w2s, wsas, biases = [], [], [], []
@@ -342,7 +352,7 @@
             wsa, zero_bias = packed_weight(c1_r, c1_i, None, None, False)
             wsas.append(wsa)
             biases.append(zero_bias)
-        outs = ops.attention_blocks_fwd(xs, w1s, w2s, wsas, biases)
+        outs = ops.attention_blocks_fwd(xs, w1s, w2s, wsas, biases, slabs)
         ctx.n, ctx.ksize = n, ksize
         ctx.sinks = [tuple(_sink(t) for t in pr) for pr in params]
         ctx.shapes = [(tuple(pr[0].shape), tuple(pr[2].shape)) for pr in params]
@@ -368,7 +378,7 @@
             sk, (s0, s2) = ctx.sinks[i], ctx.shapes[i]
             new = lambda shape: torch.empty(shape, dtype=torch.float32, device=x.device)
             fcs.append(tuple(sk[j] if sk[j] is not None else new(s0 if j < 2 else s2) for j in range(4)))
-        split = tuple(sp_ and ctx.needs_input_grad[3 + i] for i, sp_ in enumerate(ctx.split))
+        split = tuple(sp_ and ctx.needs_input_grad[4 + i] for i, sp_ in enumerate(ctx.split))
         res = ops.attention_blocks_bwd(saved, gs, wbs, fcs, split)
         if any(split):
             _POOL_ADD.clear()
@@ -389,7 +399,7 @@
         if WGRAD_SIDE is not None and ops.WGRAD_DEFER is not None:
             ops.WGRAD_DEFER.append((sps, [r[1] for r in res]))
             FLUSH_AT_NEXT_FORK = True
-        return (None, None, None, *grads_x, *grads_p)
+        return (None, None, None, None, *grads_x, *grads_p)
 
 
 SPLIT_SKIP_POOL = os.environ.get('DCS_SPLIT_SKIP_POOL', '1') != '0'
@@ -406,7 +416,8 @@
     flat = [p for pr in params for p in pr]
     split = tuple(bool(SPLIT_SKIP_POOL and getattr(x, '_dcs_adds_pool_term', False) and torch.is_grad_enabled() and x.requires_grad)
                   for x in xs)
-    return _AttentionBlocksFn.apply(len(xs), ksize, split, *xs, *flat)
+    slabs = tuple(getattr(x, '_dcs_pool_slabs', None) if ops.ENC_POOL else None for x in xs)
+    return _AttentionBlocksFn.apply(len(xs), ksize, split, slabs, *xs, *flat)
 
 
 
diff --git a/dcs-net_amd/dcsnet/ops.py b/dcs-net_amd/dcsnet/ops.py
--- a/dcs-net_amd/dcsnet/ops.py
+++ b/dcs-net_amd/dcsnet/ops.py
@@ -262,6 +262,7 @@
 import os as _os
 FUSE_APPLY_POOL = _os.environ.get('DCS_FUSE_APPLY_POOL', '1') != '0'
 STATS_EPILOGUE = _os.environ.get('DCS_STATS_EPILOGUE', '1') != '0'
+ENC_POOL = _os.environ.get('DCS_ENC_POOL', '1') != '0'
 
 
 def _conv_bytes(act, n_in, n_out, n_w):
@@ -454,6 +455,35 @@
     return y, stats, coef
 
 
+def cbn_pool_ok(x):
+    C = x.shape[3]
+    return x.dim() == 5 and 2 <= C <= 128 and (C & (C - 1)) == 0 and x.shape[0] <= 65535
+
+
+def cbn_pool(x, weight, bias, running_mean, running_covar, eps, momentum, act, drop_p, seed, stat):
+    _chk(x, 'x', 5, act=True)
+    for n, t in (('weight', weight), ('bias', bias), ('running_mean', running_mean), ('running_covar', running_covar)):
+        _chk(t, n)
+    part, rows, pivot = stat
+    _chk(part, 'stat part', 3)
+    _chk(pivot, 'stat pivot', 2)
+    B, H, W, C, _ = x.shape
+    HW = H * W
+    nch = _lib.load().dcs_ca_pool_chunks(HW, C)
+    if nch < 1 or part.shape[2] < rows or tuple(part.shape[:2]) != (C, 5) or tuple(pivot.shape) != (C, 2):
+        raise _lib.DcsHipError(f'cbn_pool: unsupported C={C} or mismatching statistics slabs {tuple(part.shape)}')
+    y = torch.empty_like(x)
+    stats = torch.empty((C, 8), dtype=torch.float32, device=x.device)
+    coef = torch.empty((C, 6), dtype=torch.float32, device=x.device)
+    slabs = torch.empty((B, nch, C, 2), dtype=torch.float64, device=x.device)
+    check(_sym('dcs_cbn_fwd_slabs_pool_drop', x, y)(ptr(x), ptr(y), ptr(weight), ptr(bias), ptr(running_mean), ptr(running_covar),
+                                                   ptr(stats), ptr(coef), ptr(part), int(rows), int(part.shape[2]), ptr(pivot),
+                                                   ptr(slabs), slabs.numel() * 8, B, HW, C, eps,
+                                                   -1.0 if momentum is None else momentum, act, float(drop_p), int(seed),
+                                                   ptr(SEED_STATE), cur_stream()), 'dcs_cbn_fwd_slabs_pool_drop')
+    return y, stats, coef, slabs
+
+
 def cbn_channel_attention(x, weight, bias, running_mean, running_covar, eps, momentum, act, stat, w1, w2):
     _chk(x, 'x', 5, act=True)
     for n, t in (('weight', weight), ('bias', bias), ('running_mean', running_mean), ('running_covar', running_covar),
@@ -606,7 +636,7 @@
     return items
 
 
-def attention_blocks_fwd(xs, w1s, w2s, wsas, biases):
+def attention_blocks_fwd(xs, w1s, w2s, wsas, biases, slabs=None):
     lib = _lib.load()
     B, dev = xs[0].shape[0], xs[0].device
     new = lambda *shape: torch.empty(shape, dtype=torch.float32, device=dev)
@@ -624,6 +654,19 @@
     nbytes = lib.dcs_attention_fwd_batched_workspace_bytes(n, items, B)
     if nbytes < 0:
         raise _lib.DcsHipError('attention_blocks_fwd: unsupported block geometry')
+    if slabs is not None and any(s_ is not None for s_ in slabs):
+        import ctypes
+        for x, s_ in zip(xs, slabs):
+            if s_ is not None:
+                _, H, W, C, _ = x.shape
+                want = (B, lib.dcs_ca_pool_chunks(H * W, C), C, 2)
+                if s_.dtype != torch.float64 or tuple(s_.shape) != want or not s_.is_contiguous() or s_.device != dev:
+                    raise _lib.DcsHipError(f'attention_blocks_fwd: pooling slabs {s_.dtype} {tuple(s_.shape)}, expected float64 {want}')
+        parts = (ctypes.c_void_p * n)(*[ptr(s_) for s_ in slabs])
+        ws = None if all(s_ is not None for s_ in slabs) else _workspace(nbytes, dev)
+        check(_sym('dcs_attention_fwd_batched_pooled', *xs)(n, items, parts, ptr(ws), 0 if ws is None else ws.numel(), B,
+                                                            cur_stream()), 'dcs_attention_fwd_batched_pooled')
+        return outs
     ws = _workspace(nbytes, dev)
     check(_sym('dcs_attention_fwd_batched', *xs)(n, items, ptr(ws), ws.numel(), B, cur_stream()), 'dcs_attention_fwd_batched')
     return outs
diff --git a/include/dcsnet_hip.h b/include/dcsnet_hip.h
--- a/include/dcsnet_hip.h
+++ b/include/dcsnet_hip.h
@@ -108,6 +108,11 @@
                            int B, long HW, int C, float eps, float momentum, int act, dcs_stream_t stream);
 int dcs_channel_attention_fc_fwd(const void* pool_part, const float* w1, const float* w2, float* ca_out, float* pooled_out,
                                  float* hidden_out, int B, long HW, int C, int Ch, dcs_stream_t stream);
+int dcs_cbn_fwd_slabs_pool_drop(const float* x, float* y, const float* weight, const float* bias,
+                                float* running_mean, float* running_covar, float* stats_out, float* coef_out,
+                                const float* part, int rows, int stride, const float* pivot, void* pool_part, long pool_bytes,
+                                int B, long HW, int C, float eps, float momentum, int act,
+                                float drop_p, unsigned long long seed, const unsigned long long* seed_dev, dcs_stream_t stream);
 
 long dcs_cbn_bwd_workspace_bytes(long P, int C);
 int  dcs_cbn_bwd(const float* x, const float* g_out, float* g_x, const float* weight,
@@ -144,6 +149,8 @@
 long dcs_attention_fwd_batched_workspace_bytes(int n, const dcs_attention_item* items, int B);
 int dcs_attention_fwd_batched(int n, const dcs_attention_item* items, void* workspace, long workspace_bytes, int B,
                               dcs_stream_t stream);
+int dcs_attention_fwd_batched_pooled(int n, const dcs_attention_item* items, const void* const* pool_parts, void* workspace,
+                                     long workspace_bytes, int B, dcs_stream_t stream);
 long dcs_attention_bwd_batched_workspace_bytes(int n, const dcs_attention_item* items, int B);
 int dcs_attention_bwd_batched(int n, const dcs_attention_item* items, void* workspace, long workspace_bytes, int B,
                               dcs_stream_t stream);
@@ -404,6 +411,11 @@
                              float* running_mean, float* running_covar, float* stats_out, float* coef_out,
                              const float* part, int rows, int stride, const float* pivot, void* pool_part, long pool_bytes,
                              int B, long HW, int C, float eps, float momentum, int act, dcs_stream_t stream);
+int dcs_cbn_fwd_slabs_pool_drop_h(const dcs_bf16_t* x, dcs_bf16_t* y, const float* weight, const float* bias,
+                                  float* running_mean, float* running_covar, float* stats_out, float* coef_out,
+                                  const float* part, int rows, int stride, const float* pivot, void* pool_part, long pool_bytes,
+                                  int B, long HW, int C, float eps, float momentum, int act,
+                                  float drop_p, unsigned long long seed, const unsigned long long* seed_dev, dcs_stream_t stream);
 int dcs_cbn_bwd_h(const dcs_bf16_t* x, const dcs_bf16_t* g_out, dcs_bf16_t* g_x, const float* weight,
                   const float* stats, const float* coef, float* g_weight, float* g_bias,
                   void* workspace, long workspace_bytes, long P, int C, int use_batch_stats, int act,
@@ -422,6 +434,8 @@
                               const unsigned long long* seed_dev, dcs_stream_t stream);
 int dcs_attention_fwd_batched_h(int n, const dcs_attention_item* items, void* workspace, long workspace_bytes, int B,
                                 dcs_stream_t stream);
+int dcs_attention_fwd_batched_pooled_h(int n, const dcs_attention_item* items, const void* const* pool_parts, void* workspace,
+                                       long workspace_bytes, int B, dcs_stream_t stream);
 int dcs_attention_bwd_sa_h(const dcs_bf16_t* x, const dcs_bf16_t* g_out, const float* ca, const float* sa, float* g_pre,
                            int B, long HW, int C, float drop_p, unsigned long long seed, const unsigned long long* seed_dev,
                            dcs_stream_t stream);
```

After: 2.591 million (median of 2 runs). No clear change (+0.3%).
